# potamides/DeTikZify

Measured on AMD Instinct MI355X. Metric: tikz_tokens_per_sec, higher is better.
Workload: dtype bf16; 1 GPU; detikzify-ds-7b (synthetic weights, seed 1234), 1 image 224x224->384x384, 243-token prefix, greedy decode of 512 tokens per rollout, batch 1 per GPU, hipGraph per token; rollouts_per_gpu=5

## Files before the change

### detikzify_amd/_lib.py

```python
from __future__ import annotations

import ctypes as C
import os
from pathlib import Path

_HERE = Path(__file__).resolve().parent
LIB_PATH = _HERE / "lib" / "libdtk_hip.so"

DTK_ABI_VERSION = 7
DTK_VIT_BATCH = 8
DTK_F32, DTK_BF16, DTK_F16 = 0, 1, 2
DTK_ARCH_PROJ_NO_BIAS = 1
DTK_PREFILL_REUSE_PREFIX, DTK_PREFILL_REUSE_IMAGE = 1, 2
DTK_MAX_INFLIGHT = 4
DTK_MAX_BATCH = 64
DTK_MAX_TOP = 8
DTK_EPI_BIAS, DTK_EPI_GELU, DTK_EPI_RESIDUAL, DTK_GEMM_NAIVE = 1, 2, 4, 256
DTK_GEMM_WT = 512
DTK_GEMM_SL = 1024
DTK_GEMM_KSLICES_SHIFT = 12


class DtkConfig(C.Structure):
    _fields_ = [
# ... 163 lines not shown
    "dtk_decode_batch_launch": (C.c_int, [_P, C.POINTER(C.c_int32)]),
    "dtk_decode_batch_wait": (C.c_int, [_P, C.POINTER(C.c_int64)]),
    "dtk_kv_fork": (C.c_int, [_P, C.c_int, C.c_int, C.c_int]),
    "dtk_get_logits_slot": (C.c_int, [_P, C.c_int, _P]),
    "dtk_context_len_slot": (C.c_int, [_P, C.c_int]),
    "dtk_slot_lcp": (C.c_int, [_P, C.c_int, _P, C.c_int, C.c_uint64, C.POINTER(C.c_int)]),
    "dtk_slot_cached_ids": (C.c_int, [_P, C.c_int, _P, C.c_int]),
    "dtk_resume_slot": (C.c_int, [_P, C.c_int, _P, C.c_int, C.c_uint64]),
    "dtk_bench_gemv": (C.c_int, [_P, C.c_int, C.c_int, C.c_int, C.POINTER(C.c_float)]),
    "dtk_set_gemv_variant": (C.c_int, [_P, C.c_int, C.c_int]),
    "dtk_set_option": (C.c_int, [_P, C.c_char_p, C.c_int]),
    "dtk_op_gemm": (C.c_int, [_P, _P, _P, _P, _P, C.c_int, C.c_int, C.c_int, C.c_int, _P]),
    "dtk_adapter_create": (C.c_int, [_P, C.POINTER(DtkAdapterConfig)]),
    "dtk_adapter_destroy": (C.c_int, [_P]),
    "dtk_has_adapter": (C.c_int, [_P]),
    "dtk_vit_encode_text": (C.c_int, [_P, _P, C.c_int, _P, C.c_int, C.c_uint64, _P, _P]),
    "dtk_prefill_text": (C.c_int, [_P, _P, C.c_int, _P, C.c_uint64, _P, C.c_int, C.c_uint64, C.c_int, _P]),
    "dtk_prefill_slot_text": (C.c_int, [_P, C.c_int, _P, C.c_int, _P, C.c_uint64, _P, C.c_int, C.c_uint64, C.c_int, _P]),
    "dtk_adapter_embed": (C.c_int, [_P, _P, C.c_int, _P]),
    "dtk_text_image_key": (C.c_uint64, [C.c_uint64, C.c_uint64]),
    "dtk_op_gemm_gated": (C.c_int, [_P, _P, _P, _P, _P, _P, C.c_int, C.c_int, C.c_int, C.c_int, _P]),
    "dtk_score": (C.c_int, [_P, _P, C.c_int, _P, C.c_uint64, C.c_uint32, C.c_int, _P, _P, _P]),
    "dtk_score_text": (C.c_int, [_P, _P, C.c_int, _P, C.c_uint64, _P, C.c_int, C.c_uint64, C.c_uint32, C.c_int, _P, _P, _P]),
    "dtk_op_score": (C.c_int, [_P, _P, _P, _P, C.c_int, C.c_int, C.c_int, C.c_int, _P, _P, _P, _P]),
    "dtk_score_packed": (C.c_int, [_P, _P, C.c_int, _P, C.c_uint64, C.c_uint32, _P, _P, C.c_int, _P, _P, _P]),
    "dtk_score_packed_text": (C.c_int, [_P, _P, C.c_int, _P, C.c_uint64, _P, C.c_int, C.c_uint64, C.c_uint32, _P, _P, C.c_int, _P, _P, _P]),
    "dtk_op_attention_seg": (C.c_int, [_P, _P, _P, _P, C.c_int, C.c_int, C.c_int, C.c_int, C.c_int, _P, _P, _P]),
    "dtk_op_attn_decode": (C.c_int, [_P, _P, _P, _P, C.c_int, C.c_int, C.c_int, C.c_int, _P, C.c_int, C.c_int, C.c_int, C.c_int, C.c_int,
                                     _P, _P, _P, _P]),
    "dtk_op_attn_decode_b": (C.c_int, [_P, _P, _P, _P, C.c_int, C.c_int, C.c_int, C.c_int, _P, _P, _P, _P,
                                       C.c_int, C.c_int, C.c_int, C.c_int, C.c_int, _P]),
    "dtk_kv8_info": (C.c_int, [_P, C.c_int, C.POINTER(C.c_int)]),
    "dtk_read_kv8": (C.c_int, [_P, C.c_int, C.c_int, C.c_int, C.c_int, C.c_int, _P, _P, _P]),
    "dtk_op_attn_decode_b8": (C.c_int, [_P, _P, _P, _P, C.c_int, C.c_int, C.c_int, C.c_int, _P, _P, _P, _P, _P, _P, _P, _P, _P,
                                        C.c_int, C.c_int, C.c_int, C.c_int, C.c_int, _P]),
    "dtk_op_gemv_b": (C.c_int, [_P, C.c_int, _P, _P, _P, C.c_int, C.c_int, _P, _P, C.c_float, _P, _P, C.c_int,
                                C.c_int, C.c_int, C.c_int, C.c_int, C.c_int, _P, _P, _P, _P, _P, _P, _P, _P, _P, _P]),
    "dtk_op_gemv_bkp": (C.c_int, [_P, _P, _P, _P, C.c_int, C.c_int, _P, _P, C.c_int, _P, C.c_float, _P, _P, _P, _P]),
    "dtk_op_gemv_role": (C.c_int, [_P, C.c_int, C.c_int, C.c_int, _P, _P, _P, _P, _P] + [C.c_int] * 9 + [C.c_float, _P, _P, _P, _P,
                                   C.c_int, _P, _P, _P, C.c_int, _P, _P, _P, _P, _P]),
    "dtk_op_rope_scatter": (C.c_int, [_P, C.c_int, _P, _P] + [C.c_int] * 8 + [_P, C.c_int, _P, _P, C.c_int, _P, _P, _P]),
    "dtk_op_rows_norm": (C.c_int, [_P, C.c_int, _P, _P, C.c_int, C.c_int, _P, _P, _P, _P, _P] + [C.c_int] * 7 + [C.c_float, C.c_int, _P, _P]),
    "dtk_op_swiglu": (C.c_int, [_P, C.c_int, _P, _P, C.c_int, C.c_int, _P, _P, C.c_int, C.c_int, C.c_int, C.c_int, C.c_int, _P]),
    "dtk_op_attention_ex": (C.c_int, [_P, _P, C.c_int64, _P, C.c_int64, _P, C.c_int64, _P, C.c_int64, _P] + [C.c_int] * 9),
    "dtk_op_rows_move": (C.c_int, [_P, C.c_int, _P, _P, _P] + [C.c_int] * 8 + [_P]),
    "dtk_op_gemv_mv_role": (C.c_int, [_P] + [C.c_int] * 4 + [_P, _P, _P] + [C.c_int] * 7 + [_P, _P, C.c_int, C.c_int, _P, _P, C.c_float,
                                      _P, _P, C.c_int, _P, _P, _P, _P, _P]),
    "dtk_w13_row_bytes": (C.c_int, [C.c_int]),
    "dtk_w13_pack_host": (C.c_int, [_P, C.c_int, C.c_int, _P, _P, _P]),
    "dtk_w13_unpack_host": (C.c_int, [_P, _P, C.c_int, C.c_int, _P]),
    "dtk_w13_op_bad_rows": (C.c_int, [_P]),
    "dtk_w13_row_bytes_host": (C.c_int, [_P, C.c_int, C.c_int, _P]),
    "dtk_w13_flagged_rows": (C.c_int, [_P, C.c_int]),
    "dtk_op_gemv": (C.c_int, [_P, _P, _P, _P, C.c_int, C.c_int, C.c_int, C.c_float, _P]),
    "dtk_op_gemv_mv": (C.c_int, [_P, _P, _P, _P, C.c_int, C.c_int, C.c_int, C.c_float, C.c_int, _P]),
    "dtk_op_gemv_q4": (C.c_int, [_P, _P, _P, _P, C.c_int, C.c_int, C.c_int, C.c_float, _P, _P]),
    "dtk_mx_layout": (C.c_int, [C.c_int, C.c_int, C.c_int, _P, _P]),
    "dtk_op_gemv_mx": (C.c_int, [_P, _P, _P, _P, C.c_int, C.c_int, C.c_int, C.c_int, C.c_int, _P, _P, _P, _P, _P]),
    "dtk_op_attention": (C.c_int, [_P, _P, _P, _P, C.c_int, C.c_int, C.c_int, C.c_int, C.c_int, C.c_int, _P]),
    "dtk_op_layernorm": (C.c_int, [_P, _P, _P, _P, C.c_int, C.c_int, C.c_float, _P]),
    "dtk_op_sample": (C.c_int, [_P, _P, C.c_int, C.c_int, C.POINTER(C.c_int64), _P]),
    "dtk_decode_wait_lp": (C.c_int, [_P, C.POINTER(C.c_int64), C.POINTER(C.c_float)]),
    "dtk_decode_batch_wait_lp": (C.c_int, [_P, C.POINTER(C.c_int64), C.POINTER(C.c_float), C.POINTER(C.c_float)]),
    "dtk_engine_read_lp": (C.c_int, [_P, C.c_int, C.POINTER(C.c_int64), C.POINTER(C.c_float), C.POINTER(C.c_float), C.c_int,
                                     C.POINTER(C.c_int32), C.POINTER(C.c_int32), C.c_int]),
    "dtk_engine_set_wait_lp_op": (C.c_int, [_P, DtkEngineOps.WAIT_LP]),
    "dtk_op_sample_lp": (C.c_int, [_P, _P, C.c_int, C.c_int, C.POINTER(C.c_int64), _P, C.POINTER(C.c_float)]),
    "dtk_score_top": (C.c_int, [_P, _P, C.c_int, _P, C.c_uint64, C.c_uint32, C.c_int, _P, _P, _P, C.c_int, _P, _P]),
    "dtk_score_top_text": (C.c_int, [_P, _P, C.c_int, _P, C.c_uint64, _P, C.c_int, C.c_uint64, C.c_uint32, C.c_int, _P, _P, _P,
                                     C.c_int, _P, _P]),
    "dtk_score_packed_top": (C.c_int, [_P, _P, C.c_int, _P, C.c_uint64, C.c_uint32, _P, _P, C.c_int, _P, _P, _P, C.c_int, _P, _P]),
    "dtk_score_packed_top_text": (C.c_int, [_P, _P, C.c_int, _P, C.c_uint64, _P, C.c_int, C.c_uint64, C.c_uint32, _P, _P, C.c_int,
                                            _P, _P, _P, C.c_int, _P, _P]),
    "dtk_op_score_top": (C.c_int, [_P, _P, _P, _P, C.c_int, C.c_int, C.c_int, C.c_int, _P, _P, _P, _P, C.c_int, _P, _P, _P]),
    "dtk_decode_wait_top": (C.c_int, [_P, C.POINTER(C.c_int64), C.POINTER(C.c_float), C.POINTER(C.c_int32), C.POINTER(C.c_float)]),
    "dtk_decode_batch_wait_top": (C.c_int, [_P, C.POINTER(C.c_int64), C.POINTER(C.c_float), C.POINTER(C.c_float),
                                            C.POINTER(C.c_int32), C.POINTER(C.c_float)]),
    "dtk_set_sampling_ext": (C.c_int, [_P, C.POINTER(DtkSamplingExt)]),
    "dtk_set_sampling_slot_ext": (C.c_int, [_P, C.c_int, C.POINTER(DtkSamplingExt)]),
    "dtk_op_sample_ext": (C.c_int, [_P, _P, C.c_int, C.c_int, C.POINTER(C.c_int64), _P, C.POINTER(C.c_float), C.POINTER(DtkSamplingExt)]),
    "dtk_engine_submit_ext": (C.c_int, [_P, C.POINTER(DtkJoin), C.POINTER(DtkSamplingExt), C.POINTER(C.c_int64), C.c_int, C.c_uint64,
                                        C.POINTER(C.c_uint64)]),
    "dtk_engine_set_sampling_ext_op": (C.c_int, [_P, DtkEngineOps.SAMPLING_EXT]),
    "dtk_set_penalties": (C.c_int, [_P, C.c_float, C.c_float, C.c_int]),
    "dtk_set_penalties_slot": (C.c_int, [_P, C.c_int, C.c_float, C.c_float, C.c_int]),
    "dtk_op_sample_pen": (C.c_int, [_P, _P, C.c_int, C.c_int, C.POINTER(C.c_int64), _P, C.POINTER(C.c_float), C.POINTER(DtkSamplingExt),
                                    C.c_float, C.c_float, C.POINTER(C.c_int64), C.c_int]),
    "dtk_token_counts": (C.c_int, [_P, C.c_int, C.POINTER(C.c_uint16), C.c_int]),
    "dtk_engine_submit_pen": (C.c_int, [_P, C.POINTER(DtkJoin), C.POINTER(DtkSamplingExt), C.c_float, C.c_float, C.c_int,
                                        C.POINTER(C.c_int64), C.c_int, C.c_uint64, C.POINTER(C.c_uint64)]),
    "dtk_engine_set_penalties_op": (C.c_int, [_P, DtkEngineOps.PENALTIES]),
    "dtk_set_dry": (C.c_int, [_P, C.POINTER(DtkDry)]),
    "dtk_set_dry_slot": (C.c_int, [_P, C.c_int, C.POINTER(DtkDry)]),
    "dtk_dry_history": (C.c_int, [_P, C.c_int, C.POINTER(C.c_int32), C.c_int]),
    "dtk_dry_state_bytes": (C.c_int64, [_P]),
    "dtk_op_dry_scan": (C.c_int, [_P, C.c_int, C.POINTER(C.c_int64), C.c_int, C.POINTER(C.c_int64), C.c_int, C.POINTER(DtkDry),
                                  C.POINTER(C.c_int32), C.POINTER(C.c_uint8), C.c_int]),
    "dtk_op_sample_dry": (C.c_int, [_P, _P, C.c_int, C.c_int, C.POINTER(C.c_int64), _P, C.POINTER(C.c_float), C.POINTER(DtkSamplingExt),
                                    C.c_float, C.c_float, C.POINTER(C.c_int64), C.c_int, C.POINTER(C.c_int64), C.c_int, C.POINTER(DtkDry)]),
    "dtk_engine_submit_dry": (C.c_int, [_P, C.POINTER(DtkJoin), C.POINTER(DtkSamplingExt), C.c_float, C.c_float, C.c_int, C.POINTER(DtkDry),
                                        C.POINTER(C.c_int64), C.c_int, C.c_uint64, C.POINTER(C.c_uint64)]),
    "dtk_engine_set_dry_op": (C.c_int, [_P, DtkEngineOps.DRY]),
    "dtk_set_length_control": (C.c_int, [_P, C.POINTER(DtkLengthCtl)]),
    "dtk_set_length_control_slot": (C.c_int, [_P, C.c_int, C.POINTER(DtkLengthCtl)]),
    "dtk_set_logit_bias": (C.c_int, [_P, C.POINTER(C.c_int32), C.POINTER(C.c_float), C.c_int]),
    "dtk_set_logit_bias_slot": (C.c_int, [_P, C.c_int, C.POINTER(C.c_int32), C.POINTER(C.c_float), C.c_int]),
# ... 85 lines not shown
```

### detikzify_amd/csrc/dtk_api.hip

```cpp
#include <hip/hip_runtime.h>

#include <cfloat>
#include <cmath>
#include <cstdarg>
#include <cstdio>
#include <cstdlib>
#include <cstring>
#include <atomic>
#include <mutex>
#include <string>
#include <unordered_map>
#include <vector>

#include "dtk_ctx.h"
#include "w13.h"
#include "mx_quant.h"

int& dtk_lds_attr_error(int device) {
  static int e[65] = {};
  return e[(device >= 0 && device < 64) ? device : 64];
}

namespace {

// ... 497 lines not shown

static void pen_args(const dtk_ctx* c, SampleArgs& sa, DryScanArgs& ds, bool batch) {
  const bool dry = (batch ? c->dry_batch : c->dry_single) && c->dry_tab;
  const bool pen = (batch ? c->pen_batch : c->pen_single) && c->pen_tab;
  const bool len = (batch ? c->len_batch : c->len_single) && c->len_dev;
  if (!(pen || dry || len) || !c->pen_dev || !c->pen_tok) return;
  const int first = batch ? 1 : 0;
  if (len) {
    sa.len = c->len_dev + first; sa.len_m = c->len_m + (size_t)first * c->len_m_stride; sa.len_m_stride = c->len_m_stride;
    sa.bias = c->bias_tab + (size_t)first * c->bias_stride; sa.bias_stride = c->bias_stride;
  }
  sa.pen = c->pen_dev + first; sa.pen_cnt = c->pen_tab ? c->pen_tab + (size_t)first * c->pen_stride : nullptr; sa.pen_stride = c->pen_stride;
  sa.pen_tok = c->pen_tok + first;
  if (!dry) return;
  sa.dry = c->dry_dev + first; sa.dry_m = c->dry_tab + (size_t)first * c->dry_stride; sa.dry_stride = c->dry_stride;
  ds.dry = sa.dry; ds.hist = c->dry_hist + (size_t)first * c->Tmax; ds.len = c->dry_len + first; ds.hist_stride = c->Tmax;
  ds.m = c->dry_tab + (size_t)first * c->dry_stride; ds.m_stride = c->dry_stride;
  ds.touched = c->dry_touched + (size_t)first * c->Tmax; ds.n_touched = c->dry_ntouched + first;
  ds.V = sa.V; ds.bs = sa.bs; ds.nslots = sa.bs ? sa.nslots : 1;
}
static void sampler_launch(dtk_ctx* c, SampleArgs& sa, bool mb, bool batch) {
  DryScanArgs ds;
  pen_args(c, sa, ds, batch);
  if (sa.dry) launch_dry_scan(ds, c->stream);
  if (mb) launch_sample_mb(sa, c->stream); else launch_sample_b(sa, c->stream);
  if (sa.pen) launch_count_token(sa, ds, c->stream);
}

static void top_logits_launch(dtk_ctx* c, const SampleArgs& sa) {
  if (!c->top_logprobs || !c->logprobs) return;
  TopArgs t;
  t.logits = sa.logits; t.V = sa.V; t.logits_stride = sa.logits_stride; t.st = sa.st; t.bs = sa.bs; t.nslots = sa.nslots;
  t.ring = sa.ring; t.k = c->top_logprobs; t.top_ring = sa.bs ? c->topb_dev : c->top_ring_dev;
  launch_top_logits(t, c->stream);
}

static inline int cfg_grid(const dtk_ctx* c) { return c->cfg_res > c->cfg_n ? c->cfg_res : c->cfg_n; }
static void guidance_launch(dtk_ctx* c, const SampleArgs& sa) {
  if (!cfg_grid(c)) return;
  CfgArgs g;
  g.logits = const_cast<float*>(sa.logits); g.V = sa.V; g.stride = sa.logits_stride; g.pairs = c->cfg_dev; g.n_pairs = cfg_grid(c); g.bs = sa.bs;
  g.part = c->cfg_part; g.lse = c->cfg_lse; g.st = sa.st; g.forced = c->cfg_forced;
  launch_cfg_mix(g, c->stream);
}
static void follow_launch(dtk_ctx* c, const SampleArgs& sa) {
  if (!cfg_grid(c)) return;
  CfgFollowArgs f;
  f.pairs = c->cfg_dev; f.n_pairs = cfg_grid(c); f.bs = sa.bs; f.forced = c->cfg_forced; f.st = sa.st; f.x = sa.x; f.d = sa.d; f.tok_ring = sa.tok_ring; f.ring = sa.ring;
  f.lp_ring = sa.lp_ring; f.lse_ring = sa.lse_ring; f.top_ring = (c->logprobs && c->top_logprobs) ? c->topb_dev : nullptr;
  launch_cfg_follow(f, c->stream);
}

static inline bool w13_on(const dtk_ctx* c) { return c->wfmt == 0 && c->w13 != 0; }

void decode_step_launches(dtk_ctx* c, bool with_probe, bool short_ctx = false) {
  hipStream_t s = c->stream;
  SampleArgs sa;
  sa.logits = c->logits; sa.V = c->V; sa.sp = c->sp; sa.st = c->st; sa.embed = c->embed;
  sa.x = c->x; sa.d = c->d; sa.tok_ring = c->tok_ring_dev; sa.ring = DTK_MAX_INFLIGHT;
  sa.probs_out = nullptr; sa.advance = 1; sa.step_override = -1; sa.bs = nullptr; sa.logits_stride = 0; sa.nslots = 1; sa.mb = c->smb;
  sa.lp_ring = c->logprobs ? c->lp_ring_dev : nullptr;
  sa.trunc = c->trunc_single ? 1 : 0;
  sa.lse_ring = (c->logprobs && c->top_logprobs) ? c->lse_ring_dev : nullptr;
  top_logits_launch(c, sa);
  sampler_launch(c, sa, c->mb_single, false);
  const float scale = 1.0f / sqrtf((float)c->hd);
  for (int l = 0; l < c->L; ++l) {
    const LayerW& w = c->layers[l];
    GemvArgs g{};
    g.eps = c->cfg.rms_eps; g.st = c->st; g.T_max = c->Tmax; g.d = c->d; g.ff = c->ff; g.H = c->H; g.KVH = c->KVH; g.hd = c->hd;
    g.rope_cos = c->rope_cos; g.rope_sin = c->rope_sin;
    g.pm = c->pm; g.pl = c->pl; g.po = c->po; g.S = c->S;
    g.W = w.wqkv; g.W8 = w.q_wqkv; g.wscale = w.s_wqkv; g.N = c->d + 2 * c->KVH * c->hd; g.K = c->d; g.x = c->x; g.norm_w = w.ln1;
    g.W4 = w.f4_wqkv; g.S4 = w.e4_wqkv;
    const bool p13 = w13_on(c) && c->w13_ready;
    g.Wp = p13 ? w.p13_wqkv : nullptr; g.Wh = w.h13_wqkv;
    g.q_out = c->q; g.kcache = kcache(c, l); g.vcache = vcache(c, l);
    launch_gemv(PRO_RMSNORM, EPI_QKV, g, s);
    AttnDecArgs ad;
    ad.q = c->q; ad.kcache = kcache(c, l); ad.vcache = vcache(c, l); ad.st = c->st;
    ad.pm = c->pm; ad.pl = c->pl; ad.po = c->po; ad.H = c->H; ad.S = c->S; ad.T_max = c->Tmax; ad.G = c->H / c->KVH;
    ad.scale = scale; ad.hd = c->hd;
    ad.threads = c->attn_threads;
    ad.combine = (!ad.threads && short_ctx && c->attn_combine == 2) ? 3 : c->attn_combine; ad.out = c->attn_out; ad.counters = c->attn_ctr;
    if (ad.threads && ad.combine == 1) ad.combine = 2;
    launch_attn_decode(ad, s);
    g.W = w.wo; g.W8 = w.q_wo; g.wscale = w.s_wo; g.N = c->d; g.K = c->d; g.y = c->x;
    g.W4 = w.f4_wo; g.S4 = w.e4_wo;
    g.Wp = p13 ? w.p13_wo : nullptr; g.Wh = w.h13_wo;
    const bool partials = ad.combine == 0 && !(ad.threads && ad.S == 1);
    if (!partials) { g.x = c->attn_out; launch_gemv(PRO_COPY, EPI_RESID, g, s); }
    else launch_gemv(PRO_ATTN, EPI_RESID, g, s);
    g.W = w.wgu; g.W8 = w.q_wgu; g.wscale = w.s_wgu; g.N = 2 * c->ff; g.K = c->d; g.x = c->x; g.norm_w = w.ln2; g.y = c->act;
    g.W4 = w.f4_wgu; g.S4 = w.e4_wgu;
    g.Wp = p13 ? w.p13_wgu : nullptr; g.Wh = w.h13_wgu;
    const bool probe_here = with_probe && (l == c->L / 2);
    if (probe_here) (void)hipEventRecord(c->probe_a, s);
    launch_gemv(PRO_RMSNORM, EPI_SWIGLU, g, s);
    if (probe_here) (void)hipEventRecord(c->probe_b, s);
    g.W = w.wdown; g.W8 = w.q_wdown; g.wscale = w.s_wdown; g.N = c->d; g.K = c->ff; g.x = c->act; g.y = c->x;
    g.W4 = w.f4_wdown; g.S4 = w.e4_wdown;
    g.Wp = p13 ? w.p13_wdown : nullptr; g.Wh = w.h13_wdown;
    launch_gemv(PRO_COPY, EPI_RESID, g, s);
  }
  GemvArgs g{};
  if (w13_on(c) && c->w13_ready) { g.Wp = c->p13_lm_head; g.Wh = c->h13_lm_head; }
  g.W = c->lm_head; g.W8 = c->q_lm_head; g.wscale = c->s_lm_head; g.N = c->V; g.K = c->d; g.x = c->x; g.norm_w = c->final_norm;
  g.eps = c->cfg.rms_eps; g.logits = c->logits;
  launch_gemv(PRO_RMSNORM, EPI_LOGITS, g, s);
}

static inline bool mx_step(const dtk_ctx* c) { return c->wfmt == 1 && c->mx_ok && c->act_fp8 != 0; }
static inline void kv8_args(const dtk_ctx* c, int l, AttnDecBArgs& ad) {
  if (!c->kv8) return;
  const size_t head_rows = (size_t)c->KVH * c->Tmax, kv_layer = 2 * head_rows * 128;
  ad.k8 = c->kv8c + (size_t)l * kv_layer; ad.v8 = ad.k8 + head_rows * 128;
  ad.k8s = c->kv8s + (size_t)l * (kv_layer / 32); ad.v8s = ad.k8s + head_rows * 4;
  ad.kv8_slot_stride = c->kv_slot_stride;
}

void batch_step_launches_mx(dtk_ctx* c) {
  hipStream_t s = c->stream;
  const int d = c->d, ff = c->ff, nslots = 16 * c->nt_step;
  SampleArgs sa;
  sa.logits = c->logits_b; sa.V = c->V; sa.sp = c->sp_b; sa.st = c->st_b; sa.embed = c->embed;
  sa.x = c->xb; sa.d = d; sa.tok_ring = c->tokb_dev; sa.ring = DTK_MAX_INFLIGHT;
  sa.probs_out = nullptr; sa.advance = 1; sa.step_override = -1; sa.bs = c->bs_dev; sa.logits_stride = c->V; sa.nslots = nslots; sa.mb = c->smb_b;
  sa.lp_ring = c->logprobs ? c->lpb_dev : nullptr;
  sa.trunc = c->trunc_batch ? 1 : 0;
  sa.lse_ring = (c->logprobs && c->top_logprobs) ? c->lseb_dev : nullptr;
  guidance_launch(c, sa);
  top_logits_launch(c, sa);
  sampler_launch(c, sa, c->mb_batch, true);
  follow_launch(c, sa);
  const float scale = 1.0f / sqrtf(128.f);
  const size_t kv_layer = (size_t)2 * c->KVH * c->Tmax * 128;
  for (int l = 0; l < c->L; ++l) {
    const LayerW& w = c->layers[l];
    bf16_t* kc = c->kvb + (size_t)l * kv_layer;
    bf16_t* vc = kc + (size_t)c->KVH * c->Tmax * 128;
    GemvBArgs g{};
    g.bs = c->bs_dev; g.st = c->st_b; g.T_max = c->Tmax; g.d = d; g.ff = ff; g.H = c->H; g.KVH = c->KVH; g.nt = c->nt_step;
    g.rope_cos = c->rope_cos; g.rope_sin = c->rope_sin; g.kv_slot_stride = c->kv_slot_stride; g.kpart = c->kpart; g.err = batch_err_word(c);
    if (l == 0) launch_rmsnorm_b(c->xb, d, w.ln1, c->xnb, d, d, c->cfg.rms_eps, c->bs_dev, nslots, s, c->xn8, c->xns);
    g.Wm = w.m_wqkv; g.wscale = w.s_wqkv; g.N = d + 2 * c->KVH * 128; g.K = d; g.X8 = c->xn8; g.XS = c->xns; g.q_out = c->qb; g.kcache = kc; g.vcache = vc;
    launch_gemv_mxu(EPI_QKV, g, s);
    AttnDecBArgs ad;
    ad.q = c->qb; ad.kcache = kc; ad.vcache = vc; ad.kv_slot_stride = c->kv_slot_stride; ad.st = c->st_b; ad.bs = c->bs_dev;
    ad.out = c->aob; ad.H = c->H; ad.T_max = c->Tmax; ad.d = d; ad.G = c->H / c->KVH; ad.nslots = nslots;
    ad.scale = scale;
    ad.use_prefix = c->prefix_mfma; ad.pfx_splits = c->pfx_splits; ad.tail_threads = c->tail_threads; ad.gqa_fused = c->gqa_fused; ad.nt_private = c->attn_nt;
    ad.pfx_m = c->pfx_m; ad.pfx_l = c->pfx_l; ad.pfx_o = c->pfx_o;
    ad.out8 = c->ao8; ad.outs = c->aos;
    kv8_args(c, l, ad);
    launch_attn_decode_b(ad, s);
    g.Wm = w.m_wo; g.wscale = w.s_wo; g.N = d; g.K = d; g.X8 = c->ao8; g.XS = c->aos;
    if (!launch_gemv_mxk(g, 32, s)) c->launch_refused = true;
    launch_resid_norm_b(c->kpart, c->xb, d, w.ln2, c->xnb, d, c->cfg.rms_eps, c->bs_dev, nslots, s, c->xn8, c->xns);
    g.Wm = w.m_wgu; g.wscale = w.s_wgu; g.N = 2 * ff; g.K = d; g.X8 = c->xn8; g.XS = c->xns; g.Y8 = c->act8; g.YS = c->acts;
    launch_gemv_mxu(EPI_SWIGLU, g, s);
    g.Wm = w.m_wdown; g.wscale = w.s_wdown; g.N = d; g.K = ff; g.X8 = c->act8; g.XS = c->acts;
// ... 138 lines not shown
  }
  g.W = c->lm_head; g.W8 = c->q_lm_head; g.wscale = c->s_lm_head; g.N = c->V; g.K = d; g.X = c->xb; g.ldx = d; g.norm_w = c->final_norm;
  g.logits = c->logits_b;
  launch_gemv_mv(PRO_RMSNORM, EPI_LOGITS, NB, g, s);
}

void ensure_fp8_weights(dtk_ctx* c) {
  if (c->wfmt == 0 || c->fp8_ready) return;
  for (int l = 0; l < c->L && c->wfmt == 2; ++l) {
    LayerW& w = c->layers[l];
    launch_quant_mxfp4_rows(w.wqkv, w.f4_wqkv, w.e4_wqkv, c->d + 2 * c->KVH * c->hd, c->d, c->stream);
    launch_quant_mxfp4_rows(w.wo, w.f4_wo, w.e4_wo, c->d, c->d, c->stream);
    launch_quant_mxfp4_rows(w.wgu, w.f4_wgu, w.e4_wgu, 2 * c->ff, c->d, c->stream);
    launch_quant_mxfp4_rows(w.wdown, w.f4_wdown, w.e4_wdown, c->d, c->ff, c->stream);
  }
  for (int l = 0; l < c->L && c->wfmt == 1; ++l) {
    LayerW& w = c->layers[l];
    launch_quant_fp8_rows(w.wqkv, w.q_wqkv, w.s_wqkv, c->d + 2 * c->KVH * c->hd, c->d, c->stream);
    launch_quant_fp8_rows(w.wo, w.q_wo, w.s_wo, c->d, c->d, c->stream);
    launch_quant_fp8_rows(w.wgu, w.q_wgu, w.s_wgu, 2 * c->ff, c->d, c->stream);
    launch_quant_fp8_rows(w.wdown, w.q_wdown, w.s_wdown, c->d, c->ff, c->stream);
  }
  launch_quant_fp8_rows(c->lm_head, c->q_lm_head, c->s_lm_head, c->V, c->d, c->stream);
  c->fp8_ready = true;
  c->tiled_ready = false;
  c->ptiled_ready = false;
}

static void set_weight_bytes(dtk_ctx* c) {
  const uint64_t kvd = (uint64_t)c->KVH * c->hd;
  const uint64_t attn_lin = (uint64_t)2 * c->d * c->d + 2 * kvd * c->d;
  const uint64_t per_layer = attn_lin + (uint64_t)3 * c->d * c->ff + 2 * (uint64_t)c->d;
  c->stats.weight_bytes_per_token = 2 * (per_layer * c->L + (uint64_t)c->d + (uint64_t)c->V * c->d);
  if (c->wfmt == 1) {
    const uint64_t lin = attn_lin + (uint64_t)3 * c->d * c->ff;
    const uint64_t rows = (uint64_t)3 * c->d + 2 * kvd + (uint64_t)2 * c->ff;
    c->stats.weight_bytes_per_token = (lin + 4 * rows + 4 * (uint64_t)c->d) * c->L + 2 * (uint64_t)c->d + (uint64_t)c->V * c->d + 4 * (uint64_t)c->V;
  }
  if (c->wfmt == 2) {
    const uint64_t bd = mxfp4_row_scales(c->d), bf = mxfp4_row_scales(c->ff);
    const uint64_t blocks = ((uint64_t)2 * c->d + 2 * kvd + (uint64_t)2 * c->ff) * bd + (uint64_t)c->d * bf;
    c->stats.weight_bytes_per_token = (17 * blocks + 4 * (uint64_t)c->d) * c->L + 2 * (uint64_t)c->d + (uint64_t)c->V * c->d + 4 * (uint64_t)c->V;
  }
  c->stats.probe_kernel_bytes = (uint64_t)2 * c->ff * c->d * (c->wfmt == 1 ? 1 : 2);
  if (c->wfmt == 2) c->stats.probe_kernel_bytes = (uint64_t)2 * c->ff * 17 * mxfp4_row_scales(c->d);
  if (w13_on(c) && c->w13_ready) {
    auto mat = [](const uint8_t* planes, uint64_t N, int K) { return planes ? N * (w13_row_bytes(K) + 1) : 2 * N * (uint64_t)K; };
    uint64_t W = 2 * ((uint64_t)2 * c->d * c->L + (uint64_t)c->d) + mat(c->p13_lm_head, (uint64_t)c->V, c->d);
    for (int l = 0; l < c->L; ++l) {
      const LayerW& w = c->layers[l];
      W += mat(w.p13_wqkv, (uint64_t)c->d + 2 * kvd, c->d) + mat(w.p13_wo, (uint64_t)c->d, c->d) + mat(w.p13_wgu, (uint64_t)2 * c->ff, c->d) +
           mat(w.p13_wdown, (uint64_t)c->d, c->ff);
    }
    c->stats.weight_bytes_per_token = W;
    c->stats.probe_kernel_bytes = mat(c->layers[c->L / 2].p13_wgu, (uint64_t)2 * c->ff, c->d);
  }
}
static void w13_set_stats(dtk_ctx* c) {
  const uint32_t rows = c->w13_bad_rows > 4095u ? 4095u : c->w13_bad_rows;
  c->stats.w13_counts = (c->w13_packed & 1023u) | ((c->w13_unpacked & 1023u) << 10) | (rows << 20);
}
static int w13_pack_one(dtk_ctx* c, int role, int pro, int epi, const bf16_t* W, int N, int K, uint8_t** planes, uint8_t** hb) {
  GemvArgs g{};
  g.N = N; g.K = K; g.d = c->d; g.ff = c->ff; g.hd = c->hd;
  if (!gemv_w13_takes(pro, epi, g)) {
    if (*planes) { (void)hipFree(*planes); *planes = nullptr; }
    if (*hb) { (void)hipFree(*hb); *hb = nullptr; }
    return DTK_OK;
  }
  if (!*planes) HIPCHK(c, hipMalloc((void**)planes, (size_t)N * w13_row_bytes(K)));
  if (!*hb) HIPCHK(c, hipMalloc((void**)hb, (size_t)N));
  HIPCHK(c, hipMemsetAsync(c->w13_bad, 0, sizeof(unsigned), c->stream));
  launch_pack_w13_rows(W, *planes, *hb, c->w13_bad, N, K, !c->w13_nz, c->stream);
  unsigned bad = 0;
  HIPCHK(c, hipMemcpyAsync(&bad, c->w13_bad, sizeof(unsigned), hipMemcpyDeviceToHost, c->stream));
  HIPCHK(c, hipStreamSynchronize(c->stream));
  if (bad) {
    (void)hipFree(*planes); *planes = nullptr;
    (void)hipFree(*hb); *hb = nullptr;
    c->w13_unpacked++; c->w13_bad_rows += bad;
  } else {
    c->w13_packed++;
    std::vector<uint8_t> bytes((size_t)N);
    HIPCHK(c, hipMemcpy(bytes.data(), *hb, (size_t)N, hipMemcpyDeviceToHost));
    for (uint8_t b : bytes) c->w13_zrows[role] += (b & W13_ZROW) ? 1u : 0u;
  }
  return DTK_OK;
}
static void w13_free(dtk_ctx* c);
int ensure_w13(dtk_ctx* c) {
  if (!w13_on(c) || c->w13_ready) return DTK_OK;
  if (!c->w13_bad) HIPCHK(c, hipMalloc((void**)&c->w13_bad, sizeof(unsigned)));
  c->w13_packed = c->w13_unpacked = c->w13_bad_rows = 0;
  for (uint32_t& z : c->w13_zrows) z = 0;
  const int qkvn = c->d + 2 * c->KVH * c->hd;
  for (int l = 0; l < c->L; ++l) {
    LayerW& w = c->layers[l];
    int rc = w13_pack_one(c, 0, PRO_RMSNORM, EPI_QKV, w.wqkv, qkvn, c->d, &w.p13_wqkv, &w.h13_wqkv);
    if (!rc) rc = w13_pack_one(c, 1, PRO_ATTN, EPI_RESID, w.wo, c->d, c->d, &w.p13_wo, &w.h13_wo);
    if (!rc) rc = w13_pack_one(c, 2, PRO_RMSNORM, EPI_SWIGLU, w.wgu, 2 * c->ff, c->d, &w.p13_wgu, &w.h13_wgu);
    if (!rc) rc = w13_pack_one(c, 3, PRO_COPY, EPI_RESID, w.wdown, c->d, c->ff, &w.p13_wdown, &w.h13_wdown);
    if (rc) { w13_free(c); return rc; }
  }
  int rc = w13_pack_one(c, 4, PRO_RMSNORM, EPI_LOGITS, c->lm_head, c->V, c->d, &c->p13_lm_head, &c->h13_lm_head);
  if (rc) { w13_free(c); return rc; }
  c->w13_ready = true;
  w13_set_stats(c);
  set_weight_bytes(c);
  return DTK_OK;
}
static void w13_free(dtk_ctx* c) {
  for (auto& w : c->layers) {
    uint8_t** ps[8] = {&w.p13_wqkv, &w.h13_wqkv, &w.p13_wo, &w.h13_wo, &w.p13_wgu, &w.h13_wgu, &w.p13_wdown, &w.h13_wdown};
    for (uint8_t** p : ps) if (*p) { (void)hipFree(*p); *p = nullptr; }
  }
  if (c->p13_lm_head) { (void)hipFree(c->p13_lm_head); c->p13_lm_head = nullptr; }
  if (c->h13_lm_head) { (void)hipFree(c->h13_lm_head); c->h13_lm_head = nullptr; }
  c->w13_ready = false;
  c->w13_packed = c->w13_unpacked = c->w13_bad_rows = 0;
  for (uint32_t& z : c->w13_zrows) z = 0;
}

void ensure_tiled_weights(dtk_ctx* c);
void ensure_prefill_tiles(dtk_ctx* c) {
  ensure_fp8_weights(c);
  if (c->ptiled_ready) return;
  for (int l = 0; l < c->L; ++l)
    if (c->layers[l].p_wgui) launch_retile_pairs(c->layers[l].wgu, c->layers[l].p_wgui, c->ff, c->d, c->stream);
  if (c->nb > 0 && c->wfmt != 1) { ensure_tiled_weights(c); c->ptiled_ready = true; return; }
  for (int l = 0; l < c->L; ++l) {
    LayerW& w = c->layers[l];
    launch_retile(w.wqkv, w.p_wqkv, c->d + 2 * c->KVH * c->hd, c->d, c->stream);
    launch_retile(w.wo, w.p_wo, c->d, c->d, c->stream);
    launch_retile(w.wgu, w.p_wgu, 2 * c->ff, c->d, c->stream);
    launch_retile(w.wdown, w.p_wdown, c->d, c->ff, c->stream);
  }
  c->ptiled_ready = true;
}

void ensure_tiled_weights(dtk_ctx* c) {
  ensure_fp8_weights(c);
  if (c->tiled_ready || c->nb <= 0) return;
  if (c->wfmt == 1) {
    const int qkvn = c->d + 2 * c->KVH * 128;
    for (int l = 0; l < c->L; ++l) {
      LayerW& w = c->layers[l];
      launch_retile_f8(w.q_wqkv, w.t8_wqkv, qkvn, c->d, c->stream);
      launch_retile_f8(w.q_wo, w.t8_wo, c->d, c->d, c->stream);
      launch_retile_f8(w.q_wgu, w.t8_wgu, 2 * c->ff, c->d, c->stream);
      launch_retile_f8(w.q_wdown, w.t8_wdown, c->d, c->ff, c->stream);
    }
    launch_retile_f8(c->q_lm_head, c->t8_lm_head, c->V, c->d, c->stream);
    if (c->mx_ok) {
      for (int l = 0; l < c->L; ++l) {
        LayerW& w = c->layers[l];
        launch_retile_mx(w.q_wqkv, w.m_wqkv, qkvn, c->d, 32, c->stream);
        launch_retile_mx(w.q_wo, w.m_wo, c->d, c->d, 32, c->stream);
        launch_retile_mx(w.q_wgu, w.m_wgu, 2 * c->ff, c->d, 32, c->stream);
        launch_retile_mx(w.q_wdown, w.m_wdown, c->d, c->ff, 16, c->stream);
      }
      launch_retile_mx(c->q_lm_head, c->m_lm_head, c->V, c->d, 32, c->stream);
    }
    c->tiled_ready = true;
    return;
  }
  for (int l = 0; l < c->L; ++l) {
    LayerW& w = c->layers[l];
    launch_retile(w.wqkv, w.t_wqkv, c->d + 2 * c->KVH * 128, c->d, c->stream);
    launch_retile(w.wo, w.t_wo, c->d, c->d, c->stream);
    launch_retile(w.wgu, w.t_wgu, 2 * c->ff, c->d, c->stream);
    launch_retile(w.wdown, w.t_wdown, c->d, c->ff, c->stream);
  }
  launch_retile(c->lm_head, c->t_lm_head, c->V, c->d, c->stream);
// ... 2162 lines not shown
  return dtk_decode_wait(c, token_out);
}

int dtk_get_logits(dtk_ctx* c, float* out) {
  if (!c || !out) return fail(c, DTK_ERR_ARG, "dtk_get_logits: null argument");
  if (!c->seq0.have_logits) return fail(c, DTK_ERR_STATE, "no logits yet");
  HIPCHK(c, hipSetDevice(c->device));
  HIPCHK(c, hipStreamSynchronize(c->stream));
  HIPCHK(c, hipMemcpy(out, c->logits, (size_t)c->V * 4, hipMemcpyDeviceToHost));
  return DTK_OK;
}

int dtk_context_len(const dtk_ctx* c) { return c ? c->seq0.host_next_pos : -1; }

int dtk_synchronize(dtk_ctx* c) {
  if (!c) return DTK_ERR_ARG;
  HIPCHK(c, hipSetDevice(c->device));
  HIPCHK(c, hipStreamSynchronize(c->stream));
  HIPCHK(c, hipGetLastError());
  return DTK_OK;
}

int dtk_get_stats(dtk_ctx* c, dtk_stats* out) {
  if (!c || !out) return DTK_ERR_ARG;
  *out = c->stats;
  return DTK_OK;
}

int dtk_bench_gemv(dtk_ctx* c, int role, int variant, int reps, float* avg_us) {
  if (!c || !avg_us || reps < 1) return fail(c, DTK_ERR_ARG, "dtk_bench_gemv: bad argument");
  HIPCHK(c, hipSetDevice(c->device));
  hipStream_t s = c->stream;
  if (role < 0 || role > 4) return fail(c, DTK_ERR_ARG, "dtk_bench_gemv: role %d (0 qkv, 1 o_proj, 2 gate/up, 3 down, 4 lm_head)", role);
  const bool same_layer = (variant & 0x100) != 0;
  const int plain = (variant >> 9) & 3;
  const bool fmt = (variant & 0x800) != 0;
  const bool b13 = (variant & 0x1000) != 0, raw16 = (variant & 0x2000) != 0;
  if (b13 && (fmt || raw16 || plain || same_layer || c->wfmt != 0 || !c->w13 || (variant & 0xff) == 0xff))
    return fail(c, DTK_ERR_ARG, "dtk_bench_gemv: 0x1000 | shape (13-bit planes) needs a bf16 context with w13 = 1, a shape number and no other flag");
  if (raw16 && ((variant & 0xff) != 0xff || plain || fmt)) return fail(c, DTK_ERR_ARG, "dtk_bench_gemv: 0x2000 (bf16 rows) goes with variant 0xff only");
  const bool step13 = w13_on(c) && !raw16 && !plain && (variant & 0xff) == 0xff;
  struct Tmp13 { std::vector<uint8_t*> p, h; ~Tmp13() { for (auto x : p) if (x) (void)hipFree(x); for (auto x : h) if (x) (void)hipFree(x); } } tmp13;
  if (b13 || step13) { if (int rc = ensure_w13(c)) return rc; }
  if (b13) {
    for (int l = 0; l < c->L && role != 4; ++l) {
      const LayerW& w = c->layers[l];
      const uint8_t* p = role == 0 ? w.p13_wqkv : (role == 1 ? w.p13_wo : (role == 2 ? w.p13_wgu : w.p13_wdown));
      if (p) continue;
      if (role != 1) return fail(c, DTK_ERR_STATE, "dtk_bench_gemv: role %d has no 13-bit planes in layer %d (an unpackable row, or a bf16 fold no 13-bit shape has)", role, l);
      if (!c->w13_bad) HIPCHK(c, hipMalloc((void**)&c->w13_bad, sizeof(unsigned)));
      uint8_t *pp = nullptr, *hh = nullptr;
      HIPCHK(c, hipMalloc((void**)&pp, (size_t)c->d * w13_row_bytes(c->d)));
      tmp13.p.push_back(pp);
      HIPCHK(c, hipMalloc((void**)&hh, (size_t)c->d));
      tmp13.h.push_back(hh);
      unsigned bad = 0;
      HIPCHK(c, hipMemsetAsync(c->w13_bad, 0, sizeof(unsigned), s));
      launch_pack_w13_rows(w.wo, pp, hh, c->w13_bad, c->d, c->d, !c->w13_nz, s);
      HIPCHK(c, hipMemcpyAsync(&bad, c->w13_bad, sizeof(unsigned), hipMemcpyDeviceToHost, s));
      HIPCHK(c, hipStreamSynchronize(s));
      if (bad) return fail(c, DTK_ERR_STATE, "dtk_bench_gemv: o_proj of layer %d has %u unpackable row(s)", l, bad);
    }
    if (role == 4 && !c->p13_lm_head) return fail(c, DTK_ERR_STATE, "dtk_bench_gemv: lm_head has no 13-bit planes");
  }
  if (fmt && ((variant & 0xff) != 0xff || plain))
    return fail(c, DTK_ERR_ARG, "dtk_bench_gemv: 0x800 (the context's weight format) goes with variant 0xff only");
  if (fmt) ensure_fp8_weights(c);
  variant &= 0xff;
  const bool shipped = variant == 0xff;
  if (b13) {
    const int pro = (role == 1 || role == 3) ? PRO_COPY : PRO_RMSNORM;
    const int epi = role == 0 ? EPI_QKV : (role == 2 ? EPI_SWIGLU : (role == 4 ? EPI_LOGITS : EPI_RESID));
    if (!gemv_w13_has(pro, epi, variant)) return fail(c, DTK_ERR_ARG, "dtk_bench_gemv: no 13-bit shape %d for role %d", variant, role);
  }
  auto launch = [&](int pro, int epi, const GemvArgs& g) {
    if (b13) launch_gemv_w13_variant(pro, epi, variant, g, s);
    else if (shipped) launch_gemv(pro, epi, g, s);
    else launch_gemv_variant(pro, epi, variant, g, s);
  };
  auto one_pass = [&]() {
    for (int l = 0; l < c->L; ++l) {
      const LayerW& w = c->layers[same_layer ? 0 : l];
      GemvArgs g{};
      if (plain) {
        g.eps = c->cfg.rms_eps; g.y = c->GU;
        if (role == 0) { g.W = w.wqkv; g.N = c->d + 2 * c->KVH * c->hd; g.K = c->d; g.x = c->x; g.norm_w = w.ln1; }
        else if (role == 1) { g.W = w.wo; g.N = c->d; g.K = c->d; g.x = c->attn_out; g.norm_w = w.ln1; }
        else if (role == 2) { g.W = w.wgu; g.N = 2 * c->ff; g.K = c->d; g.x = c->x; g.norm_w = w.ln2; }
        else if (role == 3) { g.W = w.wdown; g.N = c->d; g.K = c->ff; g.x = c->act; g.norm_w = w.ln2; }
        else { g.W = c->lm_head; g.N = c->V; g.K = c->d; g.x = c->x; g.norm_w = c->final_norm; }
        launch_gemv_variant(plain == 2 ? PRO_RMSNORM : PRO_COPY, EPI_STORE, variant, g, s);
        continue;
      }
      g.eps = c->cfg.rms_eps; g.st = c->st; g.T_max = c->Tmax; g.d = c->d; g.ff = c->ff; g.H = c->H; g.KVH = c->KVH; g.hd = c->hd;
      g.rope_cos = c->rope_cos; g.rope_sin = c->rope_sin; g.pm = c->pm; g.pl = c->pl; g.po = c->po; g.S = c->S;
      if (fmt) {
        if (role == 0) { g.W8 = w.q_wqkv; g.wscale = w.s_wqkv; g.W4 = w.f4_wqkv; g.S4 = w.e4_wqkv; }
        else if (role == 1) { g.W8 = w.q_wo; g.wscale = w.s_wo; g.W4 = w.f4_wo; g.S4 = w.e4_wo; }
        else if (role == 2) { g.W8 = w.q_wgu; g.wscale = w.s_wgu; g.W4 = w.f4_wgu; g.S4 = w.e4_wgu; }
        else if (role == 3) { g.W8 = w.q_wdown; g.wscale = w.s_wdown; g.W4 = w.f4_wdown; g.S4 = w.e4_wdown; }
        else { g.W8 = c->q_lm_head; g.wscale = c->s_lm_head; }
      }
      if (b13 || step13) {
        if (role == 0) { g.Wp = w.p13_wqkv; g.Wh = w.h13_wqkv; }
        else if (role == 1) { g.Wp = w.p13_wo; g.Wh = w.h13_wo; if (!g.Wp && b13) { g.Wp = tmp13.p[(size_t)l]; g.Wh = tmp13.h[(size_t)l]; } }
        else if (role == 2) { g.Wp = w.p13_wgu; g.Wh = w.h13_wgu; }
        else if (role == 3) { g.Wp = w.p13_wdown; g.Wh = w.h13_wdown; }
        else { g.Wp = c->p13_lm_head; g.Wh = c->h13_lm_head; }
      }
      if (role == 0) { g.W = w.wqkv; g.N = c->d + 2 * c->KVH * c->hd; g.K = c->d; g.x = c->x; g.norm_w = w.ln1; g.q_out = c->q; g.kcache = kcache(c, l); g.vcache = vcache(c, l); launch(PRO_RMSNORM, EPI_QKV, g); }
      else if (role == 1) { g.W = w.wo; g.N = c->d; g.K = c->d; g.x = c->attn_out; g.y = c->q; launch(PRO_COPY, EPI_RESID, g); }
      else if (role == 2) { g.W = w.wgu; g.N = 2 * c->ff; g.K = c->d; g.x = c->x; g.norm_w = w.ln2; g.y = c->act; launch(PRO_RMSNORM, EPI_SWIGLU, g); }
      else if (role == 3) { g.W = w.wdown; g.N = c->d; g.K = c->ff; g.x = c->act; g.y = c->q; launch(PRO_COPY, EPI_RESID, g); }
      else { g.W = c->lm_head; g.N = c->V; g.K = c->d; g.x = c->x; g.norm_w = c->final_norm; g.logits = c->logits; launch(PRO_RMSNORM, EPI_LOGITS, g); }
    }
  };
  one_pass();
  HIPCHK(c, hipEventRecord(c->ev_a, s));
  for (int r = 0; r < reps; ++r) one_pass();
  HIPCHK(c, hipEventRecord(c->ev_b, s));
  HIPCHK(c, hipStreamSynchronize(s));
  HIPCHK(c, hipGetLastError());
  float ms = 0.f;
  HIPCHK(c, hipEventElapsedTime(&ms, c->ev_a, c->ev_b));
  *avg_us = ms * 1e3f / (float)(reps * c->L);
  c->seq0.have_logits = false;
  return DTK_OK;
}
// ... 4 lines not shown
  if (c->blaunched != c->bwaited) return fail(c, DTK_ERR_STATE, "dtk_bench_cfg: a batch step is in flight");
  HIPCHK(c, hipSetDevice(c->device));
  SampleArgs sa;
  sa.logits = c->logits_b; sa.V = c->V; sa.logits_stride = c->V; sa.bs = c->bs_dev; sa.st = c->st_b; sa.x = c->xb; sa.d = c->d;
  sa.tok_ring = c->tokb_dev; sa.ring = DTK_MAX_INFLIGHT;
  sa.lp_ring = c->logprobs ? c->lpb_dev : nullptr; sa.lse_ring = (c->logprobs && c->top_logprobs) ? c->lseb_dev : nullptr;
  for (int which = 0; which < 2; ++which) {
    for (int i = 0; i < 3; ++i) { if (which) follow_launch(c, sa); else guidance_launch(c, sa); }
    HIPCHK(c, hipEventRecord(c->probe_a, c->stream));
    for (int i = 0; i < reps; ++i) { if (which) follow_launch(c, sa); else guidance_launch(c, sa); }
    HIPCHK(c, hipEventRecord(c->probe_b, c->stream));
    HIPCHK(c, hipEventSynchronize(c->probe_b));
    float ms = 0.f;
    HIPCHK(c, hipEventElapsedTime(&ms, c->probe_a, c->probe_b));
    avg_us[which] = ms * 1000.f / (float)reps;
  }
  return DTK_OK;
}

int dtk_bench_spec(dtk_ctx* c, int reps, float* avg_us) {
  if (!c || !avg_us || reps < 1 || reps > 64) return fail(c, DTK_ERR_ARG, "dtk_bench_spec: bad argument (1 <= reps <= 64)");
  if (!c->spec_on) return fail(c, DTK_ERR_STATE, "dtk_bench_spec: slot 0 is not speculating (dtk_spec_begin)");
  if (c->blaunched != c->bwaited) return fail(c, DTK_ERR_STATE, "dtk_bench_spec: a step is in flight");
  HIPCHK(c, hipSetDevice(c->device));
  SpecArgs sv;
  sv.sd = c->spec_sd; sv.hist = c->spec_hist; sv.table = c->spec_table; sv.K = 0; sv.max_ngram = 0; sv.NV = 0; sv.T_max = c->Tmax; sv.V = c->V;
  sv.st_true = c->st_b; sv.st_vec = c->spec_st; sv.bs = c->spec_bs; sv.tok_ring = c->tokb_dev; sv.ring = DTK_MAX_INFLIGHT;
  sv.embed = c->embed; sv.x = c->xb; sv.d = c->d;
  for (int i = 0; i < 3; ++i) { launch_spec_accept(sv, c->stream); launch_spec_draft(sv, c->stream); }
  HIPCHK(c, hipEventRecord(c->probe_a, c->stream));
  for (int i = 0; i < reps; ++i) { launch_spec_accept(sv, c->stream); launch_spec_draft(sv, c->stream); }
  HIPCHK(c, hipEventRecord(c->probe_b, c->stream));
  HIPCHK(c, hipEventSynchronize(c->probe_b));
  float ms = 0.f;
  HIPCHK(c, hipEventElapsedTime(&ms, c->probe_a, c->probe_b));
  *avg_us = ms * 1000.f / (float)reps;
  const uint32_t ring_was = (uint32_t)(c->blaunched % DTK_MAX_INFLIGHT);
  HIPCHK(c, hipMemcpy(&c->spec_bs->step, &ring_was, sizeof ring_was, hipMemcpyHostToDevice));
  return DTK_OK;
}

int dtk_set_option(dtk_ctx* c, const char* name, int value) {
  if (!c || !name) return DTK_ERR_ARG;
  HIPCHK(c, hipSetDevice(c->device));
  HIPCHK(c, hipStreamSynchronize(c->stream));
  if (!strcmp(name, "attn_full_max")) c->attn_full_max = value;
  else if (!strcmp(name, "w13")) {
    if (value != 0 && value != 1) return fail(c, DTK_ERR_ARG, "w13 must be 0 or 1");
    if (value != c->w13) {
      if (c->launched != c->waited) return fail(c, DTK_ERR_STATE, "w13: %d single-sequence decode step(s) are unread", (int)(c->launched - c->waited));
      c->w13 = value; drop_graph(c);
      if (!value) { w13_free(c); w13_set_stats(c); }
      set_weight_bytes(c);
    }
  }
  else if (!strcmp(name, "w13_nz")) {
    if (value != 0 && value != 1) return fail(c, DTK_ERR_ARG, "w13_nz must be 0 or 1");
    if (value != c->w13_nz) {
      if (c->launched != c->waited) return fail(c, DTK_ERR_STATE, "w13_nz: %d single-sequence decode step(s) are unread", (int)(c->launched - c->waited));
      c->w13_nz = value;
      if (c->w13_ready) { c->w13_ready = false; drop_graph(c); }
    }
  }
  else if (!strcmp(name, "logprobs")) {
    if (value != 0 && value != 1) return fail(c, DTK_ERR_ARG, "logprobs must be 0 or 1");
    if (value == 0 && c->top_logprobs) return fail(c, DTK_ERR_STATE, "logprobs: top_logprobs = %d needs it (set \"top_logprobs\" to 0 first)", c->top_logprobs);
    if ((value != 0) != (c->logprobs != 0)) {
      if (c->blaunched != c->bwaited) return fail(c, DTK_ERR_STATE, "logprobs: a batch step is in flight");
      if (c->engine_holds.load() > 0) return fail(c, DTK_ERR_STATE, "logprobs: an engine holds %d sequence(s) in this context's slots", c->engine_holds.load());
      if (c->launched != c->waited) return fail(c, DTK_ERR_STATE, "logprobs: %d single-sequence decode step(s) are unread", (int)(c->launched - c->waited));
      c->logprobs = value; drop_graph(c); drop_batch_graphs(c);
    }
  }
  else if (!strcmp(name, "top_logprobs")) {
    if (value < 0 || value > DTK_MAX_TOP) return fail(c, DTK_ERR_ARG, "top_logprobs must be 0 .. %d", DTK_MAX_TOP);
    if (value > c->V) return fail(c, DTK_ERR_ARG, "top_logprobs = %d exceeds the vocabulary (%d)", value, c->V);
    if (value != 0 && !c->logprobs) return fail(c, DTK_ERR_STATE, "top_logprobs needs logprobs = 1 (dtk_set_option \"logprobs\", 1 first)");
    if (value != c->top_logprobs) {
      if (c->blaunched != c->bwaited) return fail(c, DTK_ERR_STATE, "top_logprobs: a batch step is in flight");
      if (c->engine_holds.load() > 0) return fail(c, DTK_ERR_STATE, "top_logprobs: an engine holds %d sequence(s) in this context's slots", c->engine_holds.load());
      if (c->launched != c->waited) return fail(c, DTK_ERR_STATE, "top_logprobs: %d single-sequence decode step(s) are unread", (int)(c->launched - c->waited));
      if (value) {
        const size_t n1 = DTK_MAX_INFLIGHT, nb = c->nb > 0 ? (size_t)DTK_MAX_INFLIGHT * DTK_MAX_BATCH : 0;
        if (!c->top_ring_dev) { HIPCHK(c, hipMalloc(&c->top_ring_dev, sizeof(TopRec) * n1)); HIPCHK(c, hipMemset(c->top_ring_dev, 0, sizeof(TopRec) * n1)); }
        if (!c->lse_ring_dev) { HIPCHK(c, hipMalloc(&c->lse_ring_dev, sizeof(float) * n1)); HIPCHK(c, hipMemset(c->lse_ring_dev, 0, sizeof(float) * n1)); }
        if (!c->top_ring_host) HIPCHK(c, hipHostMalloc((void**)&c->top_ring_host, sizeof(TopRec) * n1, hipHostMallocDefault));
        if (!c->lse_ring_host) HIPCHK(c, hipHostMalloc((void**)&c->lse_ring_host, sizeof(float) * n1, hipHostMallocDefault));
        if (nb && !c->topb_dev) { HIPCHK(c, hipMalloc(&c->topb_dev, sizeof(TopRec) * nb)); HIPCHK(c, hipMemset(c->topb_dev, 0, sizeof(TopRec) * nb)); }
        if (nb && !c->lseb_dev) { HIPCHK(c, hipMalloc(&c->lseb_dev, sizeof(float) * nb)); HIPCHK(c, hipMemset(c->lseb_dev, 0, sizeof(float) * nb)); }
        if (nb && !c->topb_host) HIPCHK(c, hipHostMalloc((void**)&c->topb_host, sizeof(TopRec) * nb, hipHostMallocDefault));
        if (nb && !c->lseb_host) HIPCHK(c, hipHostMalloc((void**)&c->lseb_host, sizeof(float) * nb, hipHostMallocDefault));
      }
      c->top_logprobs = value; drop_graph(c); drop_batch_graphs(c);
    }
  }
  else if (!strcmp(name, "gemm_tile")) {
    if (value < 0 || value > 5) return fail(c, DTK_ERR_ARG, "gemm_tile must be 0..5");
    set_gemm_tile(value);
  }
  else if (!strcmp(name, "share_prefix_reads")) c->share_reads = value != 0;
  else if (!strcmp(name, "prefix_mfma") || !strcmp(name, "pfx_splits") || !strcmp(name, "gemv_b_wide") ||
           !strcmp(name, "tail_threads")) {
    if (!strcmp(name, "prefix_mfma")) c->prefix_mfma = value != 0;
    else if (!strcmp(name, "tail_threads")) { if (value != 64 && value != 128 && value != 256 && value != 512) return fail(c, DTK_ERR_ARG, "tail_threads must be 64, 128, 256 or 512"); c->tail_threads = value; }
    else if (!strcmp(name, "pfx_splits")) { if (value < 1 || value > 4) return fail(c, DTK_ERR_ARG, "pfx_splits must be 1..4"); c->pfx_splits = value; }
    else { if (value < 0 || value > 6) return fail(c, DTK_ERR_ARG, "gemv_b_wide must be 0..6"); set_gemv_b_wide(value); }
// ... 383 lines not shown
```

### detikzify_amd/csrc/dtk_ctx.h

```cpp
#pragma once
#include <hip/hip_runtime.h>

#include <atomic>
#include <cstddef>
#include <cstdint>
#include <mutex>
#include <string>
#include <unordered_map>
#include <vector>

#include "../../include/dtk.h"
#include "kernels.h"
#ifndef W13_DEFAULT
#define W13_DEFAULT 1
#endif

struct TensorEntry {
  std::string name;
  bf16_t* ptr = nullptr;
  int64_t rows = 1;
  int64_t cols = 0;
  int64_t stride = 0;
  float synth_scale = 0.02f;
  float synth_offset = 0.f;
// ... 75 lines not shown

  bf16_t *X, *Xn, *QKV, *Qh, *AO, *GU, *ACT;
  int sk_sl_min_rows = SK_SL_MIN_ROWS;
  float* skpart = nullptr;
  size_t skpart_floats = 0;
  int swiglu_fused = 1;
  int qkv_rope_fused = 1;
  int prefill_sk = 1;
  int32_t* ids_dev = nullptr;
  float* score_rec = nullptr;
  float* score_out = nullptr;
  float* score_top = nullptr;
  int32_t* packed_rows = nullptr;
  bf16_t *x, *q, *act;
  float *logits, *pm, *pl, *po;
  bf16_t* attn_out = nullptr;
  unsigned* attn_ctr = nullptr;
  int attn_combine = 0;
  DecState* st = nullptr;
  SamplingDev* sp = nullptr;
  int64_t* tok_ring_dev = nullptr;
  int64_t* tok_ring_host = nullptr;
  float* probs_dev = nullptr;
  int logprobs = 0;
  std::atomic<int> engine_holds{0};
  float2* lp_ring_dev = nullptr;
  float2* lp_ring_host = nullptr;
  float2* lpb_dev = nullptr;
  float2* lpb_host = nullptr;
  int top_logprobs = 0;
  TopRec* top_ring_dev = nullptr;
  TopRec* top_ring_host = nullptr;
  float* lse_ring_dev = nullptr;
  float* lse_ring_host = nullptr;
  TopRec* topb_dev = nullptr;
  TopRec* topb_host = nullptr;
  float* lseb_dev = nullptr;
  float* lseb_host = nullptr;
  float* pixels_dev = nullptr;
  bf16_t *patches, *VX, *VN, *VQKV, *VAO, *VH, *feats, *last_hidden;
  bf16_t *pq, *pkv, *pao, *px, *pn, *ph, *pooled;
  bf16_t* IMG;
  Adapter* ad = nullptr;
  unsigned char* scratch = nullptr;
  size_t scratch_bytes = 0;

  SeqHost seq0;
  int wfmt = 0;
  bool fp8_ready = false;
  uint8_t* q_lm_head = nullptr;
  float* s_lm_head = nullptr;
  int w13 = W13_DEFAULT;
  int w13_nz = 1;
  bool w13_ready = false;
  uint8_t *p13_lm_head = nullptr, *h13_lm_head = nullptr;
  unsigned* w13_bad = nullptr;
  int w13_op_bad_rows = -1;
  uint32_t w13_packed = 0, w13_unpacked = 0, w13_bad_rows = 0;
  uint32_t w13_zrows[5] = {0, 0, 0, 0, 0};
  uint64_t cached_image_key = 0;
  bool have_image = false;
  int KVH = 0;
  int hd = 128;
  bool proj_bias = true;
  int nb = 0;
  bool share_reads = true;
  int nt = 1;
  std::vector<SeqHost> bseq;
  bf16_t* kvb = nullptr;
  size_t kv_slot_stride = 0;
  int kv8 = 0; int kv8_slots = 0;
  uint8_t* kv8c = nullptr; uint8_t* kv8s = nullptr;
  bf16_t *xb = nullptr, *xnb = nullptr, *qb = nullptr, *aob = nullptr, *actb = nullptr;
  float* logits_b = nullptr;
  float* kpart = nullptr; unsigned* kctr = nullptr;
  int attn_nt = 1;
  bool resid_kparts = true;
  float *pfx_m = nullptr, *pfx_l = nullptr, *pfx_o = nullptr;
  int prefix_mfma = 0;
  int pfx_splits = 4;
  int gqa_fused = 1;
  int tail_threads = 256;
  DecState* st_b = nullptr;
  SamplingDev* sp_b = nullptr;
  BatchState* bs_dev = nullptr;
  bf16_t* t_lm_head = nullptr;
  uint8_t* t8_lm_head = nullptr;
  uint8_t* m_lm_head = nullptr;
  uint8_t *xn8 = nullptr, *xns = nullptr, *ao8 = nullptr, *aos = nullptr, *act8 = nullptr, *acts = nullptr;
  bool mx_ok = false;
  int act_fp8 = 0;
  bool launch_refused = false;
  bool tiled_ready = false;
  bool ptiled_ready = false;
  BatchState* bs_host = nullptr;
  SamplingDev* sp_stage = nullptr; uint32_t* draw_stage = nullptr;
  DecState* st_stage = nullptr;
  int64_t* tokb_dev = nullptr;
  int64_t* tokb_host = nullptr;
  uint64_t blaunched = 0, bwaited = 0;
  hipEvent_t bstep_done[DTK_MAX_INFLIGHT] = {};
  bool bgraph_ready[6] = {false, false, false, false, false, false};
  hipGraph_t bgraph[6] = {nullptr, nullptr, nullptr, nullptr, nullptr, nullptr};
  hipGraphExec_t bgraph_exec[6] = {nullptr, nullptr, nullptr, nullptr, nullptr, nullptr};
  int nt_step = 1;
  int mv_slots = 4;
  int mv_step = 0;
  int mv_tail_threads = 512;
  dtk_sampling sampling{};
  SampleMB* smb = nullptr;
  SampleMB* smb_b = nullptr;
  bool mb_single = false;
// ... 120 lines not shown
```

### detikzify_amd/csrc/dtk_ops.hip

```cpp
#include <hip/hip_runtime.h>

#include <cmath>
#include <cstdio>
#include <cstdlib>
#include <cstring>
#include <optional>
#include <vector>

#include "dtk_ctx.h"
#include "w13.h"
#include "mx_quant.h"

#pragma GCC visibility push(default)
extern "C" {

extern "C++" {
namespace {
struct OpRun {
  static constexpr size_t GUARD = 256;
  dtk_ctx* c; const char* who; int fill; size_t off = 0, need = 0; bool full = false;
  struct In { void* dev; const void* host; size_t bytes; };
  struct Res { void* dev; void* host; size_t bytes; const char* name; bool up; };
  std::vector<In> ins; std::vector<Res> res;
  OpRun(dtk_ctx* c_, const char* who_, int fill_ = -1) : c(c_), who(who_), fill(fill_) {}
// ... 480 lines not shown
int dtk_op_gemv_role(dtk_ctx* c, int pro, int epi, int variant, const uint16_t* W, const uint8_t* W8, const float* wscale,
                     const uint8_t* W4, const uint8_t* S4, int N, int K, int d, int ff, int H, int KVH, int hd, int T_max, int pos, float eps,
                     const uint16_t* x, const uint16_t* norm_w, const uint16_t* rope_cos, const uint16_t* rope_sin,
                     int S, const float* pm, const float* pl, const float* po, int scratch_fill,
                     uint16_t* q_io, uint16_t* k_io, uint16_t* v_io, uint16_t* y_io, float* logits_io) {
  if (!c) return DTK_ERR_ARG;
  if ((W != nullptr) + (W8 != nullptr) + (W4 != nullptr) != 1 || (W8 && !wscale) || (!W8 && wscale) || (!W4 != !S4))
    return fail(c, DTK_ERR_ARG, "dtk_op_gemv_role: exactly one of W | W8 + wscale | W4 + S4");
  const int fmt = W4 ? 2 : (W8 ? 1 : 0);
  const bool f13 = variant >= 0x1000;
  const int v13 = variant - 0x1000;
  if (f13) {
    if (fmt != 0) return fail(c, DTK_ERR_ARG, "dtk_op_gemv_role: the 13-bit planes are packed from bf16 operands (W)");
    if (v13 != 0xff && !gemv_w13_has(pro, epi, v13)) return fail(c, DTK_ERR_ARG, "dtk_op_gemv_role: no 13-bit kernel for prologue %d, epilogue %d, shape %d", pro, epi, v13);
    if (v13 == 0xff && !gemv_w13_has(pro, epi, 0)) return fail(c, DTK_ERR_ARG, "dtk_op_gemv_role: no 13-bit kernel for prologue %d, epilogue %d", pro, epi);
    variant = -1;
  }
  if (N < 1 || K < 8 || (K & 7) || (fmt == 1 && (K & 15))) return fail(c, DTK_ERR_ARG, "dtk_op_gemv_role: N >= 1, K a multiple of 8 (16 for fp8 weights)");
  if (pro < PRO_COPY || pro > PRO_ATTN || epi < EPI_STORE || epi > EPI_LOGITS) return fail(c, DTK_ERR_ARG, "dtk_op_gemv_role: unknown prologue %d or epilogue %d", pro, epi);
  if (!gemv_role_variant_ok(fmt, pro, epi, variant))
    return fail(c, DTK_ERR_ARG, "dtk_op_gemv_role: no %s kernel for prologue %d, epilogue %d, variant %d", fmt == 2 ? "MXFP4" : (fmt == 1 ? "fp8" : "bf16"), pro, epi, variant);
  if (hd != 128 && hd != 64) return fail(c, DTK_ERR_ARG, "dtk_op_gemv_role: head dim %d (128 or 64)", hd);
  if (scratch_fill < 0 || scratch_fill > 255 || d < 0) return fail(c, DTK_ERR_ARG, "dtk_op_gemv_role: scratch_fill is a byte, d >= 0");
  if (pro == PRO_ATTN) {
    if (S < 1 || S > 16) return fail(c, DTK_ERR_ARG, "dtk_op_gemv_role: S must be 1..16");
    if (H < 1 || K != H * hd || !pm || !pl || !po) return fail(c, DTK_ERR_ARG, "dtk_op_gemv_role: PRO_ATTN needs K = H * hd and the partials pm / pl / po");
  } else if (!x || (pro == PRO_RMSNORM && !norm_w)) return fail(c, DTK_ERR_ARG, "dtk_op_gemv_role: x (and norm_w for PRO_RMSNORM) required");
  if (epi == EPI_QKV) {
    if (H < 1 || KVH < 1 || H % KVH) return fail(c, DTK_ERR_ARG, "dtk_op_gemv_role: H %d query heads over KVH %d key / value heads", H, KVH);
    if (N != (H + 2 * KVH) * hd || d != H * hd) return fail(c, DTK_ERR_ARG, "dtk_op_gemv_role: QKV needs N = (H + 2 KVH) * hd and d = H * hd");
    if (T_max < 1 || pos < 0 || pos >= T_max) return fail(c, DTK_ERR_ARG, "dtk_op_gemv_role: position %d of %d rows", pos, T_max);
    if (!rope_cos || !rope_sin || !q_io || !k_io || !v_io) return fail(c, DTK_ERR_ARG, "dtk_op_gemv_role: QKV needs the rope tables and q / k / v buffers");
  } else if (epi == EPI_SWIGLU) {
    if (ff < 8 || (ff & 7) || N != 2 * ff || !y_io) return fail(c, DTK_ERR_ARG, "dtk_op_gemv_role: SWIGLU needs ff a multiple of 8 (as dtk_create), N = 2 ff and y");
  } else if (epi == EPI_LOGITS) {
    if (!logits_io) return fail(c, DTK_ERR_ARG, "dtk_op_gemv_role: LOGITS needs the logits buffer");
  } else if (!y_io) return fail(c, DTK_ERR_ARG, "dtk_op_gemv_role: RESID / STORE need y");
  HIPCHK(c, hipSetDevice(c->device));
  hipStream_t s = c->stream;
  const int KC4 = (K + 31) >> 5, hd2 = hd / 2;
  const size_t w_bytes = fmt == 2 ? (size_t)N * KC4 * 16 : (fmt == 1 ? (size_t)N * K : (size_t)N * K * 2);
  const size_t kv = epi == EPI_QKV ? (size_t)KVH * T_max * hd : 0, qn = epi == EPI_QKV ? (size_t)H * hd : 0, rope = epi == EPI_QKV ? (size_t)T_max * hd2 : 0;
  const size_t ny = epi == EPI_SWIGLU ? (size_t)ff : ((epi == EPI_STORE || epi == EPI_RESID) ? (size_t)N : 0), nl = epi == EPI_LOGITS ? (size_t)N : 0;
  const size_t hs = pro == PRO_ATTN ? (size_t)H * S : 0;
  DecState hst; memset(&hst, 0, sizeof hst);
  hst.pos = pos; hst.next_pos = pos + 1;
  OpRun r(c, "dtk_op_gemv_role", scratch_fill);
  GemvArgs g{};
  const uint8_t* dW = r.in<uint8_t>(fmt == 2 ? (const void*)W4 : (fmt == 1 ? (const void*)W8 : (const void*)W), w_bytes);
  const float* dws = r.in<float>(wscale, fmt == 1 ? N : 0); const uint8_t* dS4 = r.in<uint8_t>(S4, fmt == 2 ? (size_t)N * KC4 : 0);
  if (fmt == 0) g.W = reinterpret_cast<const bf16_t*>(dW);
  else if (fmt == 1) { g.W8 = dW; g.wscale = dws; }
  else { g.W4 = dW; g.S4 = dS4; }
  uint8_t* dWp = (uint8_t*)r.take(f13 ? (size_t)N * w13_row_bytes(K) : 0); uint8_t* dWh = (uint8_t*)r.take(f13 ? (size_t)N : 0);
  unsigned* dbad = (unsigned*)r.take(f13 ? sizeof(unsigned) : 0);
  g.x = r.in<bf16_t>(pro != PRO_ATTN ? x : nullptr, K); g.norm_w = r.in<bf16_t>(pro == PRO_RMSNORM ? norm_w : nullptr, K);
  g.rope_cos = r.in<bf16_t>(rope_cos, rope); g.rope_sin = r.in<bf16_t>(rope_sin, rope); g.st = r.in<DecState>(&hst, 1);
  g.pm = r.in<float>(pm, hs); g.pl = r.in<float>(pl, hs); g.po = r.in<float>(po, hs * hd);
  g.q_out = r.io<bf16_t>(qn ? q_io : nullptr, qn, "q"); g.kcache = r.io<bf16_t>(kv ? k_io : nullptr, kv, "k"); g.vcache = r.io<bf16_t>(kv ? v_io : nullptr, kv, "v");
  g.y = r.io<bf16_t>(ny ? y_io : nullptr, ny, "y"); g.logits = r.io<float>(nl ? logits_io : nullptr, nl, "logits");
  g.N = N; g.K = K; g.eps = eps; g.S = S; g.T_max = T_max; g.d = d; g.ff = ff; g.H = H; g.KVH = KVH; g.hd = hd;
  if (const int rc = r.upload(s)) return rc;
  if (f13) {
    unsigned bad = 0;
    HIPCHK(c, hipMemsetAsync(dbad, 0, sizeof(unsigned), s));
    launch_pack_w13_rows(g.W, dWp, dWh, dbad, N, K, !c->w13_nz, s);
    HIPCHK(c, hipMemcpyAsync(&bad, dbad, sizeof(unsigned), hipMemcpyDeviceToHost, s));
    HIPCHK(c, hipStreamSynchronize(s));
    HIPCHK(c, hipMemsetAsync(dbad, scratch_fill, sizeof(unsigned), s));
    c->w13_op_bad_rows = (int)bad;
    if (!bad) { g.Wp = dWp; g.Wh = dWh; }
  }
  if (f13 && g.Wp && v13 != 0xff) launch_gemv_w13_variant(pro, epi, v13, g, s);
  else if (variant < 0) launch_gemv(pro, epi, g, s);
  else if (fmt == 1) launch_gemv_f8_variant(pro, epi, variant, g, s);
  else launch_gemv_variant(pro, epi, variant, g, s);
  return r.finish(s);
}


int dtk_op_rope_scatter(dtk_ctx* c, int form, const uint16_t* QKV, const float* part, int S, int part_rows, int T, int H, int KVH, int hd,
                        int T_max, int start_pos, const int32_t* rows, int max_pos, const uint16_t* rope_cos, const uint16_t* rope_sin,
                        int scratch_fill, uint16_t* q_io, uint16_t* k_io, uint16_t* v_io) {
  const char* who = "dtk_op_rope_scatter";
  if (!c || !rope_cos || !rope_sin || !q_io || !k_io || !v_io) return fail(c, DTK_ERR_ARG, "%s: null argument", who);
  if (form != 0 && form != 1) return fail(c, DTK_ERR_ARG, "%s: form %d (0 bf16 rows, 1 fp32 K-slice partials)", who, form);
  if (hd != 128 && hd != 64) return fail(c, DTK_ERR_ARG, "%s: head dim %d (128 or 64)", who, hd);
  if (T < 1 || H < 1 || KVH < 1 || H % KVH || T_max < 1 || max_pos < 1) return fail(c, DTK_ERR_ARG, "%s: T %d, H %d query heads over KVH %d key / value heads, T_max %d", who, T, H, KVH, T_max);
  if (scratch_fill < 0 || scratch_fill > 255) return fail(c, DTK_ERR_ARG, "%s: scratch_fill is a byte", who);
  if (form == 0 && !QKV) return fail(c, DTK_ERR_ARG, "%s: form 0 needs QKV", who);
  if (form == 1 && (!part || S < 1 || S > 8 || part_rows < T)) return fail(c, DTK_ERR_ARG, "%s: form 1 needs partials of S = 1..8 slices and part_rows >= T", who);
  for (int t = 0; t < T; ++t) {
    const int pos = rows ? rows[2 * t] : start_pos + t, row = rows ? rows[2 * t + 1] : start_pos + t;
    if (pos < 0 || pos >= max_pos || row < 0 || row >= T_max)
      return fail(c, DTK_ERR_ARG, "%s: row %d: position %d of %d, cache row %d of %d", who, t, pos, max_pos, row, T_max);
  }
  HIPCHK(c, hipSetDevice(c->device));
  hipStream_t s = c->stream;
  const size_t qkvn = (size_t)(H + 2 * KVH) * hd, kv = (size_t)KVH * T_max * hd;
  OpRun r(c, who, scratch_fill);
  const bf16_t* dQKV = r.in<bf16_t>(form == 0 ? QKV : nullptr, form == 0 ? (size_t)T * qkvn : 0);
  const float* dP = r.in<float>(form == 1 ? part : nullptr, form == 1 ? (size_t)S * part_rows * qkvn : 0);
  const bf16_t* dcos = r.in<bf16_t>(rope_cos, (size_t)max_pos * (hd / 2));
  const bf16_t* dsin = r.in<bf16_t>(rope_sin, (size_t)max_pos * (hd / 2));
  const int2* dR = r.in<int2>(rows, rows ? (size_t)T : 0);
  bf16_t* dq = r.io<bf16_t>(q_io, (size_t)H * T * hd, "q"); bf16_t* dk = r.io<bf16_t>(k_io, kv, "k"); bf16_t* dv = r.io<bf16_t>(v_io, kv, "v");
  if (const int rc = r.upload(s)) return rc;
  const long ps = (long)part_rows * (long)qkvn;
  if (form == 0 && rows) launch_rope_scatter_rows(dQKV, dq, dk, dv, dcos, dsin, T, dR, H, KVH, T_max, s, hd);
  else if (form == 0) launch_rope_scatter(dQKV, dq, dk, dv, dcos, dsin, T, start_pos, H, KVH, T_max, s, hd);
  else if (rows) launch_sk_rope_scatter_rows(dP, ps, S, dq, dk, dv, dcos, dsin, T, dR, H, KVH, T_max, s, hd);
  else launch_sk_rope_scatter(dP, ps, S, dq, dk, dv, dcos, dsin, T, start_pos, H, KVH, T_max, s, hd);
  return r.finish(s);
}

int dtk_op_rows_norm(dtk_ctx* c, int form, const uint16_t* X, const float* part, int S, int part_rows, const uint16_t* norm_w,
                     const uint16_t* ln_b, const uint16_t* bias, const uint16_t* residual, const uint16_t* gate, int flags, int M, int N,
                     int ldx, int ldc, int ldr, int ldy, float eps, int scratch_fill, uint16_t* c_io, uint16_t* y_io) {
  const char* who = "dtk_op_rows_norm";
  if (!c) return DTK_ERR_ARG;
  if (form < 0 || form > 3) return fail(c, DTK_ERR_ARG, "%s: form %d (0 rmsnorm_rows, 1 rmsnorm_rows_sk, 2 sk_reduce, 3 layernorm_rows)", who, form);
  if (M < 1 || N < 1 || scratch_fill < 0 || scratch_fill > 255) return fail(c, DTK_ERR_ARG, "%s: M, N >= 1, scratch_fill a byte", who);
  const bool in_place = form == 3 && !X;
  if (form != 2) {
// ... 199 lines not shown
  } else if (epi == EPI_SWIGLU) {
    if (ff < 8 || (ff & 7) || N != 2 * ff || !y_io) return fail(c, DTK_ERR_ARG, "%s: SWIGLU needs ff a multiple of 8 (as dtk_create), N = 2 ff and y", who);
  } else if (epi == EPI_LOGITS) {
    if (!logits_io) return fail(c, DTK_ERR_ARG, "%s: LOGITS needs the logits buffer", who);
  } else if (!y_io) return fail(c, DTK_ERR_ARG, "%s: RESID / STORE need y", who);
  HIPCHK(c, hipSetDevice(c->device));
  hipStream_t s = c->stream;
  const bool qkv = epi == EPI_QKV;
  const size_t kv_slot = qkv ? (size_t)KVH * T_max * 128 : 0;
  const size_t ny = epi == EPI_SWIGLU ? (size_t)((ff + 31) >> 5) * 512 : ((epi == EPI_STORE || epi == EPI_RESID) ? (size_t)nb * N : 0);
  BatchState hbs; memset(&hbs, 0, sizeof hbs);
  DecState hst[4]; memset(hst, 0, sizeof hst);
  for (int j = 0; j < DTK_MAX_BATCH; ++j) hbs.share_src[j] = -1;
  for (int b = 0; b < nb; ++b) { hbs.active[b] = active[b] ? 1 : 0; hst[b].pos = pos[b]; hst[b].next_pos = pos[b] + 1; }
  OpRun r(c, who, scratch_fill);
  GemvMvArgs g{};
  if (W8) { g.W8 = r.in<uint8_t>(W8, (size_t)N * K); g.wscale = r.in<float>(wscale, N); }
  else g.W = r.in<bf16_t>(W, (size_t)N * K);
  g.X = r.in<bf16_t>(X, x_layout ? (size_t)((K + 31) >> 5) * 512 : (size_t)nb * K);
  g.norm_w = r.in<bf16_t>(pro == PRO_RMSNORM ? norm_w : nullptr, pro == PRO_RMSNORM ? K : 0);
  g.rope_cos = r.in<bf16_t>(qkv ? rope_cos : nullptr, qkv ? (size_t)T_max * 64 : 0);
  g.rope_sin = r.in<bf16_t>(qkv ? rope_sin : nullptr, qkv ? (size_t)T_max * 64 : 0);
  g.st = r.in<DecState>(hst, 4);
  const BatchState* dbs = r.in<BatchState>(&hbs, 1);
  g.bs = bs_null ? nullptr : dbs;
  g.q_out = r.io<bf16_t>(qkv ? q_io : nullptr, qkv ? (size_t)nb * d : 0, "q");
  g.kcache = r.io<bf16_t>(qkv ? k_io : nullptr, (size_t)nb * kv_slot, "k");
  g.vcache = r.io<bf16_t>(qkv ? v_io : nullptr, (size_t)nb * kv_slot, "v");
  g.Y = r.io<bf16_t>(ny ? y_io : nullptr, ny, "y");
  g.logits = r.io<float>(epi == EPI_LOGITS ? logits_io : nullptr, epi == EPI_LOGITS ? (size_t)nb * N : 0, "logits");
  g.N = N; g.K = K; g.ldx = K; g.x_rowmajor = x_layout == 0; g.eps = eps; g.ldy = N; g.kv_slot_stride = kv_slot;
  g.T_max = T_max; g.d = d; g.ff = ff; g.H = H; g.KVH = KVH;
  if (const int rc = r.upload(s)) return rc;
  {
    MvShapeScope scope(epi, shape);
    launch_gemv_mv(pro, epi, nb, g, s);
  }
  return r.finish(s);
}

int dtk_w13_row_bytes(int K) { return (K < 8 || (K & 7)) ? -1 : (int)w13_row_bytes(K); }
int dtk_w13_pack_host(const uint16_t* W, int N, int K, uint8_t* planes, uint8_t* hb, int32_t* bad) {
  if (!W || !planes || !hb || !bad || N < 1 || K < 8 || (K & 7)) return DTK_ERR_ARG;
  for (int r = 0; r < N; ++r) bad[r] = w13_pack_row(W + (size_t)r * K, K, planes + (size_t)r * w13_row_bytes(K), hb + r);
  return DTK_OK;
}
int dtk_w13_unpack_host(const uint8_t* planes, const uint8_t* hb, int N, int K, uint16_t* W) {
  if (!W || !planes || !hb || N < 1 || K < 8 || (K & 7)) return DTK_ERR_ARG;
  for (int r = 0; r < N; ++r) w13_unpack_row(planes + (size_t)r * w13_row_bytes(K), hb[r], K, W + (size_t)r * K);
  return DTK_OK;
}
int dtk_w13_op_bad_rows(dtk_ctx* c) { return c ? c->w13_op_bad_rows : -1; }
int dtk_w13_flagged_rows(dtk_ctx* c, int role) { return (c && role >= 0 && role < 5 && c->w13_ready) ? (int)c->w13_zrows[role] : -1; }
int dtk_w13_row_bytes_host(const uint16_t* W, int N, int K, uint8_t* bytes) {
  if (!W || !bytes || N < 0 || K < 8 || (K & 7)) return DTK_ERR_ARG;
  for (int r = 0; r < N; ++r) bytes[r] = (uint8_t)w13_row_byte(W + (size_t)r * K, K);
  return DTK_OK;
}

extern "C++" {
namespace {
inline int op_nt_of(int nslots) { const int hi = nslots - 1; return hi < 16 ? 1 : (hi < 32 ? 2 : 4); }
const void* op_tiled_weights(OpRun& r, const uint16_t* W, const uint8_t* W8, const float* wscale, int N, int K, GemvBArgs& g) {
  g.N = N; g.K = K;
  if (W8) {
    const uint8_t* dW = r.in<uint8_t>(W8, (size_t)N * K);
    g.W8 = (uint8_t*)r.take(tiled_bytes_f8(N, K)); g.wscale = r.in<float>(wscale, N);
    return dW;
  }
  const bf16_t* dW = r.in<bf16_t>(W, (size_t)N * K);
  g.W = (bf16_t*)r.take(tiled_elems(N, K) * sizeof(bf16_t));
  return dW;
}
void op_retile(const void* rows, const GemvBArgs& g, hipStream_t s) {
  if (g.W8) launch_retile_f8((const uint8_t*)rows, const_cast<uint8_t*>(g.W8), g.N, g.K, s);
  else launch_retile((const bf16_t*)rows, const_cast<bf16_t*>(g.W), g.N, g.K, s);
}
struct OpBatchState {
  BatchState hbs; DecState hst[DTK_MAX_BATCH];
  OpBatchState(OpRun& r, const int32_t* active, const int32_t* pos, int nslots, GemvBArgs& g) {
    memset(&hbs, 0, sizeof hbs); memset(hst, 0, sizeof hst);
    for (int j = 0; j < DTK_MAX_BATCH; ++j) hbs.share_src[j] = -1;
    for (int j = 0; j < nslots; ++j) {
      hbs.active[j] = active[j] ? 1 : 0;
      if (pos) { hst[j].pos = pos[j]; hst[j].next_pos = pos[j] + 1; }
    }
    g.bs = r.in<BatchState>(&hbs, 1); g.st = r.in<DecState>(hst, DTK_MAX_BATCH); g.nt = op_nt_of(nslots);
  }
  OpBatchState(const OpBatchState&) = delete;
};
std::vector<bf16_t> op_x_fragments(const uint16_t* X, int nslots, int K) {
  const int nsteps = (K + 31) >> 5;
  std::vector<bf16_t> h((size_t)4 * nsteps * 512, (bf16_t)0);
  for (int j = 0; j < nslots; ++j)
    for (int k = 0; k < K; ++k) h[host_xtile_off(j, k, nsteps)] = X[(size_t)j * K + k];
  return h;
}
void op_x_rows(const bf16_t* frag, int nslots, int K, uint16_t* X) {
  const int nsteps = (K + 31) >> 5;
  for (int j = 0; j < nslots; ++j)
    for (int k = 0; k < K; ++k) X[(size_t)j * K + k] = frag[host_xtile_off(j, k, nsteps)];
}
}
}

int dtk_op_gemv_b(dtk_ctx* c, int epi, const uint16_t* W, const uint8_t* W8, const float* wscale, int N, int K,
// ... 364 lines not shown
```

### detikzify_amd/csrc/gemv_inl.h

```cpp
#pragma once
#include "common.h"
#include "w13.h"

template <int NR, int U>
__device__ __forceinline__ void gemv_load(u32x4 (&w)[NR][U], const u32x4* (&rows)[NR],
                                          int g, int lane, int K8) {
  if (64 * (g * U + U) <= K8) {
#pragma unroll
    for (int u = 0; u < U; ++u) {
      const int c = lane + 64 * (g * U + u);
#pragma unroll
      for (int r = 0; r < NR; ++r) w[r][u] = ld_nt(rows[r] + c);
    }
    return;
  }
#pragma unroll
  for (int u = 0; u < U; ++u) {
    const int c = lane + 64 * (g * U + u);
    const bool ok = c < K8;
#pragma unroll
    for (int r = 0; r < NR; ++r) {
      u32x4 z = {0u, 0u, 0u, 0u};
      w[r][u] = ok ? ld_nt(rows[r] + c) : z;
    }
// ... 55 lines not shown
#undef F4_WORD
  return c;
}

template <int NR, int U>
__device__ __forceinline__ void gemv_load_f4(u32x4 (&w)[NR][U], unsigned (&sc)[NR][U], const u32x4* (&rows)[NR], const uint8_t* (&srows)[NR],
                                             int g, int lane, int KC) {
  gemv_load<NR, U>(w, rows, g, lane, KC);
  const bool full = 64 * (g * U + U) <= KC;
#pragma unroll
  for (int u = 0; u < U; ++u) {
    const int c = lane + 64 * (g * U + u);
#pragma unroll
    for (int r = 0; r < NR; ++r) sc[r][u] = (full || c < KC) ? (unsigned)srows[r][c] : 127u;
  }
}

template <int NR, int U>
__device__ __forceinline__ void gemv_fma_f4(float (&acc)[NR], const u32x4 (&w)[NR][U], const unsigned (&sc)[NR][U],
                                            const u32x4* xs, int g, int lane, int KC) {
#pragma unroll
  for (int u = 0; u < U; ++u) {
    const int c = lane + 64 * (g * U + u);
    u32x4 x0 = {0u, 0u, 0u, 0u}, x1 = x0, x2 = x0, x3 = x0;
    if (64 * (g * U + U) <= KC || c < KC) {
      const int b = ((c >> 4) << 6) | (c & 15);
      x0 = xs[b]; x1 = xs[(b + 16) ^ 2]; x2 = xs[(b + 32) ^ 4]; x3 = xs[(b + 48) ^ 6];
    }
#pragma unroll
    for (int r = 0; r < NR; ++r) acc[r] = dot32_f4(w[r][u], f4_scale(sc[r][u]), x0, x1, x2, x3, acc[r]);
  }
}

typedef __attribute__((ext_vector_type(2))) unsigned short u16x2_t;

__device__ __forceinline__ uint32_t w13_high4(uint32_t codes, uint32_t lo2) {
  const uint32_t nz = ((codes + 0x0f0f0f0fu) >> 4) & 0x01010101u;
  const u16x2_t r = __builtin_bit_cast(u16x2_t, nz) * __builtin_bit_cast(u16x2_t, lo2) + __builtin_bit_cast(u16x2_t, codes);
  return __builtin_bit_cast(uint32_t, r);
}

template <bool NZ>
__device__ __forceinline__ float dot8_w13(uint32_t la, uint32_t lb, uint32_t n, uint32_t s, int i, uint32_t lo4, const u32x4& x, float c) {
  const uint32_t ce = n & 0x0f0f0f0fu, co = (n >> 4) & 0x0f0f0f0fu;
  const uint32_t he = (NZ ? ce + lo4 : w13_high4(ce, lo4 & 0x00ff00ffu)) | ((s << (7 - 2 * i)) & 0x80808080u);
  const uint32_t ho = (NZ ? co + lo4 : w13_high4(co, lo4 & 0x00ff00ffu)) | ((s << (6 - 2 * i)) & 0x80808080u);
  c = dot2(__builtin_amdgcn_perm(he, la, 0x05010400u), x[0], c);
  c = dot2(__builtin_amdgcn_perm(he, la, 0x07030602u), x[1], c);
  c = dot2(__builtin_amdgcn_perm(ho, lb, 0x05010400u), x[2], c);
  c = dot2(__builtin_amdgcn_perm(ho, lb, 0x07030602u), x[3], c);
  return c;
}

template <int NR, int U>
__device__ __forceinline__ void gemv_load_w13(u32x4 (&wl)[NR][U / 2], u32x2 (&wn)[NR][U / 2], uint32_t (&ws)[NR][U / 4],
                                              const u32x4* (&rows)[NR], int g, int lane, int J2, int n_off, int s_off) {
  static_assert(U % 4 == 0, "a stage is whole sign blocks");
  if (2 * (g * (U / 4) + U / 4) <= J2) {
#pragma unroll
    for (int ub = 0; ub < U / 4; ++ub) {
      const int b = g * (U / 4) + ub;
#pragma unroll
      for (int r = 0; r < NR; ++r) {
        const unsigned char* p = reinterpret_cast<const unsigned char*>(rows[r]);
#pragma unroll
        for (int h = 0; h < 2; ++h) {
          wl[r][2 * ub + h] = ld_nt(rows[r] + ((2 * b + h) * 64 + lane));
          wn[r][2 * ub + h] = __builtin_nontemporal_load(reinterpret_cast<const u32x2*>(p + n_off) + ((2 * b + h) * 64 + lane));
        }
        ws[r][ub] = __builtin_nontemporal_load(reinterpret_cast<const uint32_t*>(p + s_off) + (b * 64 + lane));
      }
    }
    return;
  }
#pragma unroll
  for (int ub = 0; ub < U / 4; ++ub) {
    const int b = g * (U / 4) + ub;
#pragma unroll
    for (int r = 0; r < NR; ++r) {
      const unsigned char* p = reinterpret_cast<const unsigned char*>(rows[r]);
#pragma unroll
      for (int h = 0; h < 2; ++h) {
        const bool ok = 2 * b + h < J2;
        const u32x4 zl = {0u, 0u, 0u, 0u};
        const u32x2 zn = {0u, 0u};
        wl[r][2 * ub + h] = ok ? ld_nt(rows[r] + ((2 * b + h) * 64 + lane)) : zl;
        wn[r][2 * ub + h] = ok ? __builtin_nontemporal_load(reinterpret_cast<const u32x2*>(p + n_off) + ((2 * b + h) * 64 + lane)) : zn;
      }
      ws[r][ub] = (2 * b < J2) ? __builtin_nontemporal_load(reinterpret_cast<const uint32_t*>(p + s_off) + (b * 64 + lane)) : 0u;
    }
  }
}

template <int NR, int U, bool NZ>
__device__ __forceinline__ void gemv_fma_w13(float (&acc)[NR], const u32x4 (&wl)[NR][U / 2], const u32x2 (&wn)[NR][U / 2],
                                             const uint32_t (&ws)[NR][U / 4], const uint32_t (&lo4)[NR],
                                             const u32x4* xs, int g, int lane, int K8) {
  const bool full = 64 * (g * U + U) <= K8;
#pragma unroll
  for (int u = 0; u < U; ++u) {
    const int c = lane + 64 * (g * U + u);
    u32x4 xv = {0u, 0u, 0u, 0u};
    if (full || c < K8) xv = xs[c];
#pragma unroll
    for (int r = 0; r < NR; ++r) {
      const u32x4& l = wl[r][u >> 1];
      acc[r] = dot8_w13<NZ>((u & 1) ? l[2] : l[0], (u & 1) ? l[3] : l[1], wn[r][u >> 1][u & 1], ws[r][u >> 2], u & 3, lo4[r], xv, acc[r]);
    }
  }
}
```

### detikzify_amd/csrc/kernels.h

```cpp
#pragma once
#include "common.h"
#include <stdlib.h>
#include <string.h>

enum { PRO_COPY = 0, PRO_RMSNORM = 1, PRO_ATTN = 2 };
enum { EPI_STORE = 0, EPI_RESID = 1, EPI_QKV = 2, EPI_SWIGLU = 3, EPI_LOGITS = 4 };

struct GemvArgs {
  const bf16_t* W;
  const uint8_t* W8;
  const float* wscale;
  int N;
  int K;
  const bf16_t* x;
  const bf16_t* norm_w;
  float eps;
  const float* pm;
  const float* pl;
  const float* po;
  int S;
  bf16_t* y;
  float* logits;
  bf16_t* q_out;
  bf16_t* kcache;
  bf16_t* vcache;
  const bf16_t* rope_cos;
  const bf16_t* rope_sin;
  const DecState* st;
  int T_max;
  int d;
  int ff;
  int H;
  int KVH;
  int hd = 128;
  const uint8_t* W4 = nullptr;
  const uint8_t* S4 = nullptr;
  const uint8_t* Wp = nullptr;
  const uint8_t* Wh = nullptr;
};

void launch_gemv(int pro, int epi, const GemvArgs& a, hipStream_t s);
void launch_gemv_q4(int pro, int epi, const GemvArgs& a, hipStream_t s);
void launch_gemv_variant(int pro, int epi, int variant, const GemvArgs& a, hipStream_t s);
void launch_gemv_w13_variant(int pro, int epi, int variant, const GemvArgs& a, hipStream_t s);
bool gemv_w13_has(int pro, int epi, int variant);
bool gemv_w13_takes(int pro, int epi, const GemvArgs& a);
void launch_pack_w13_rows(const bf16_t* W, uint8_t* Wp, uint8_t* Wh, unsigned* bad_rows, int N, int K, bool zflag_all, hipStream_t s);
void launch_gemv_f8(int pro, int epi, const GemvArgs& a, hipStream_t s);
void launch_gemv_f8_variant(int pro, int epi, int variant, const GemvArgs& a, hipStream_t s);
void set_gemv_default_variant(int epi, int variant);

struct AttnDecArgs {
  const bf16_t* q;
  const bf16_t* kcache;
  const bf16_t* vcache;
  const DecState* st;
  float* pm; float* pl; float* po;
  int H; int S; int T_max; float scale;
  int combine;
  bf16_t* out;
  unsigned* counters;
  int G;
  int threads;
  int hd = 128;
};
void launch_attn_decode(const AttnDecArgs& a, hipStream_t s);

struct SampleArgs {
  const float* logits; int V;
  const SamplingDev* sp;
  DecState* st;
  const bf16_t* embed;
  bf16_t* x;
  int d;
  int64_t* tok_ring;
  int ring;
  float* probs_out;
  int advance;
  int step_override;
  const BatchState* bs;
  int logits_stride;
  int nslots;
  SampleMB* mb;
  float2* lp_ring = nullptr;
  int trunc = 0;
  float* lse_ring = nullptr;
  const PenDev* pen = nullptr;
  const uint16_t* pen_cnt = nullptr;
  int pen_stride = 0;
  int32_t* pen_tok = nullptr;
  const DryDev* dry = nullptr;
  const uint8_t* dry_m = nullptr;
  int dry_stride = 0;
  const LenDev* len = nullptr;
  const float* len_m = nullptr;
  int len_m_stride = 0;
  const float* bias = nullptr;
  int bias_stride = 0;
  int len_cur = -1;
};
// ... 287 lines not shown
```

### detikzify_amd/csrc/kernels_decode.hip

```cpp
#include <cstdlib>
#include <cstring>
#include "kernels.h"
#include "gemv_inl.h"

template <int EPI, bool F8, int HD = 128>
__device__ __forceinline__ void gemv_epilogue(const GemvArgs& a, int u, float a0, float a1, float pre0, float pre1, int pos) {
    constexpr int HD2 = HD / 2, HSH = HD == 128 ? 6 : 5;
    static_assert(HD == 128 || HD == 64, "head dim 128 or 64");
    if (F8) {
      if (EPI == EPI_QKV) {
        const int r0 = (u >> HSH) * HD + (u & (HD2 - 1));
        a0 *= a.wscale[r0];
        a1 *= a.wscale[r0 + HD2];
      } else if (EPI == EPI_SWIGLU) {
        a0 *= a.wscale[u];
        a1 *= a.wscale[a.ff + u];
      } else {
        a0 *= a.wscale[u];
      }
    }
    if (EPI == EPI_STORE) {
      a.y[u] = f2bf(a0);
    } else if (EPI == EPI_RESID) {
      a.y[u] = f2bf(pre0 + rbf(a0));
// ... 18 lines not shown
        const float c = pre0, s = pre1;
        const float o1 = rbf(rbf(x1 * c) + rbf(-x2 * s));
        const float o2 = rbf(rbf(x2 * c) + rbf(x1 * s));
        bf16_t* dst = (sec == 0) ? (a.q_out + head * HD)
                                 : (a.kcache + ((size_t)head * a.T_max + pos) * HD);
        dst[i] = f2bf(o1);
        dst[i + HD2] = f2bf(o2);
      }
    }
}

template <int PRO, int EPI, int R, int U, int WAVES, bool PERSIST, bool F8 = false, int KS = 1, int HD = 128, bool F4 = false, bool W13 = false, int FW = WAVES>
__global__ __launch_bounds__(WAVES * 64) void k_gemv(GemvArgs a) {
  static_assert(!(F4 && F8) && !(W13 && (F4 || F8)), "one weight format");
  static_assert(FW >= 1 && FW <= WAVES, "the folding threads are the block's first");
  constexpr int FT = FW * 64;
  constexpr bool FALL = FW == WAVES;
  constexpr bool PAIRED = (EPI == EPI_QKV) || (EPI == EPI_SWIGLU);
  constexpr int NR = PAIRED ? 2 * R : R;
  constexpr int THREADS = WAVES * 64;
  constexpr int RW = WAVES / KS;
  constexpr int HD2 = HD / 2, HC = HD / 8;
  constexpr int HSH = HD == 128 ? 6 : 5, CSH = HSH - 2;
  static_assert(HD == 128 || HD == 64, "head dim 128 or 64");
  static_assert(WAVES % KS == 0 && (KS == 1 || !PERSIST), "split-K variants are not persistent");
  extern __shared__ __attribute__((aligned(16))) unsigned char smem[];
  u32x4* xs = reinterpret_cast<u32x4*>(smem);
  const int K8 = a.K >> 3;
  const int KC = F4 ? ((a.K + 31) >> 5) : (F8 ? (a.K >> 4) : K8);
  const size_t row_bytes = W13 ? w13_row_bytes(a.K) : (F4 ? (size_t)KC * 16 : (F8 ? (size_t)a.K : (size_t)a.K * 2));
  const unsigned char* Wb = reinterpret_cast<const unsigned char*>(W13 ? (const void*)a.Wp : (F4 ? (const void*)a.W4 : (F8 ? (const void*)a.W8 : (const void*)a.W)));
  const int J2 = W13 ? w13_units(a.K) : 0, n13 = W13 ? (int)w13_n_off(a.K) : 0, s13 = W13 ? (int)w13_s_off(a.K) : 0;
  float* red = reinterpret_cast<float*>(smem + (size_t)(F4 ? f4_xrows(KC) : K8) * 16);
#define XI(c) (F4 ? f4_xswz(c) : (c))

  const int tid = threadIdx.x;
  const int lane = tid & 63;
  const int wave = tid >> 6;
  const int rw = KS > 1 ? wave / KS : wave;
  const int ks = KS > 1 ? wave % KS : 0;

  int n_units;
  if (EPI == EPI_QKV) n_units = (a.N >> 1);
  else if (EPI == EPI_SWIGLU) n_units = a.ff;
  else n_units = a.N;
  const int chunk_stride = PERSIST ? (int)gridDim.x * WAVES : 0;
  int chunk = PERSIST ? (int)blockIdx.x + (int)gridDim.x * wave : (int)blockIdx.x * RW + rw;
  int unit0 = chunk * R;

  const u32x4* rows[NR];
  const uint8_t* srows[NR];
  uint32_t lo4[NR];
  bool zrow = false;
  auto set_rows = [&](int u0) {
    unsigned zb = 0;
#pragma unroll
    for (int j = 0; j < R; ++j) {
      int u = u0 + j;
      if (u >= n_units) u = n_units - 1;
      int r0, r1 = 0;
      if (EPI == EPI_QKV) {
        r0 = (u >> HSH) * HD + (u & (HD2 - 1));
        r1 = r0 + HD2;
      } else if (EPI == EPI_SWIGLU) {
        r0 = u;
        r1 = a.ff + u;
      } else {
        r0 = u;
      }
      if (PAIRED) {
        rows[2 * j] = reinterpret_cast<const u32x4*>(Wb + (size_t)r0 * row_bytes);
        rows[2 * j + 1] = reinterpret_cast<const u32x4*>(Wb + (size_t)r1 * row_bytes);
      } else {
        rows[j] = reinterpret_cast<const u32x4*>(Wb + (size_t)r0 * row_bytes);
      }
      if (F4) {
        if (PAIRED) { srows[2 * j] = a.S4 + (size_t)r0 * KC; srows[2 * j + 1] = a.S4 + (size_t)r1 * KC; }
        else srows[j] = a.S4 + (size_t)r0 * KC;
      }
      if (W13) {
        const unsigned b0 = a.Wh[r0], b1 = PAIRED ? a.Wh[r1] : 0u;
        if (PAIRED) { lo4[2 * j] = (uint32_t)w13_lo(b0) * 0x01010101u; lo4[2 * j + 1] = (uint32_t)w13_lo(b1) * 0x01010101u; }
        else lo4[j] = (uint32_t)w13_lo(b0) * 0x01010101u;
        zb |= b0 | b1;
      }
    }
    if (W13 && PRO == PRO_RMSNORM) zrow = (__builtin_amdgcn_readfirstlane((int)zb) & W13_ZROW) != 0;
  };
  set_rows(unit0);

  const int iters = (KC + 63) >> 6;
  const int Gall = (iters + U - 1) / U;
  const int G = KS > 1 ? (Gall - ks + KS - 1) / KS : Gall;
#define GIDX(g) (KS > 1 ? ks + KS * (g) : (g))
  u32x4 wa[NR][U], wb[NR][U];
  unsigned sa[NR][U], sb[NR][U];
  constexpr int UW = W13 ? U : 4;
  u32x4 lwa[NR][UW / 2], lwb[NR][UW / 2];
  u32x2 nwa[NR][UW / 2], nwb[NR][UW / 2];
  uint32_t zwa[NR][UW / 4], zwb[NR][UW / 4];
  float acc[NR];
#define GLOAD(w, sc, g) do { if (W13) gemv_load_w13<NR, UW>(l##w, n##w, z##w, rows, (g), lane, J2, n13, s13); else if (F4) gemv_load_f4<NR, U>(w, sc, rows, srows, (g), lane, KC); else gemv_load<NR, U>(w, rows, (g), lane, KC); } while (0)
#define GFMA(w, sc, g) do { if (W13) gemv_fma_w13<NR, UW, NZ>(acc, l##w, n##w, z##w, lo4, xs, (g), lane, K8); else if (F4) gemv_fma_f4<NR, U>(acc, w, sc, xs, (g), lane, KC); else if (F8) gemv_fma_f8<NR, U>(acc, w, xs, (g), lane, KC); else gemv_fma<NR, U>(acc, w, xs, (g), lane, KC); } while (0)

  if (G > 0) GLOAD(wa, sa, GIDX(0));

  float pre0[R], pre1[R];
  int pos = 0;
  if (EPI == EPI_QKV) pos = a.st->pos;
  auto prefetch_epilogue = [&](int u0) {
#pragma unroll
    for (int j = 0; j < R; ++j) {
      pre0[j] = 0.f; pre1[j] = 0.f;
      if (lane == 0 && ks == 0) {
        int u = u0 + j;
        if (u >= n_units) u = n_units - 1;
        if (EPI == EPI_RESID) pre0[j] = bf2f(a.y[u]);
        if (EPI == EPI_QKV) {
          pre0[j] = bf2f(a.rope_cos[(size_t)pos * HD2 + (u & (HD2 - 1))]);
          pre1[j] = bf2f(a.rope_sin[(size_t)pos * HD2 + (u & (HD2 - 1))]);
        }
      }
    }
  };
  if (EPI == EPI_RESID || EPI == EPI_QKV) prefetch_epilogue(unit0);

  if (PRO == PRO_COPY) {
    const u32x4* x4 = reinterpret_cast<const u32x4*>(a.x);
    for (int c = tid; c < K8; c += THREADS) xs[XI(c)] = x4[c];
  } else if (PRO == PRO_RMSNORM) {
    const u32x4* x4 = reinterpret_cast<const u32x4*>(a.x);
    const u32x4* w4 = reinterpret_cast<const u32x4*>(a.norm_w);
    if (K8 <= 2 * FT) {
      const int c0 = tid, c1 = tid + FT;
      const bool h0 = (FALL || tid < FT) && c0 < K8, h1 = (FALL || tid < FT) && c1 < K8;
      const u32x4 zz = {0u, 0u, 0u, 0u};
      const u32x4 v0 = h0 ? x4[c0] : zz, v1 = h1 ? x4[c1] : zz;
      const u32x4 g0 = h0 ? w4[c0] : zz, g1 = h1 ? w4[c1] : zz;
      float ss = 0.f;
#pragma unroll
      for (int e = 0; e < 4; ++e) {
        const float lo = pk_lo(v0[e]), hi = pk_hi(v0[e]);
        ss += lo * lo;
        ss += hi * hi;
      }
#pragma unroll
      for (int e = 0; e < 4; ++e) {
        const float lo = pk_lo(v1[e]), hi = pk_hi(v1[e]);
        ss += lo * lo;
        ss += hi * hi;
      }
      ss = wave_sum(ss);
      if (lane == 0) red[wave] = ss;
      __syncthreads();
      float tot = 0.f;
#pragma unroll
      for (int w = 0; w < FW; ++w) tot += red[w];
      const float inv = rsqrtf(tot / (float)a.K + a.eps);
// ... 47 lines not shown
        float m4[4];
#pragma unroll
        for (int j = 0; j < 4; ++j) m4[j] = (s0 + j < S) ? pmh[s0 + j] : -1e30f;
#pragma unroll
        for (int j = 0; j < 4; ++j) M = fmaxf(M, m4[j]);
      }
      float L = 0.f;
      float o[8];
#pragma unroll
      for (int e = 0; e < 8; ++e) o[e] = 0.f;
      for (int s0 = 0; s0 < S; s0 += 4) {
        float m4[4], l4[4];
        f32x4 p0[4], p1[4];
#pragma unroll
        for (int j = 0; j < 4; ++j) {
          const bool ok = s0 + j < S;
          const int sj = ok ? s0 + j : s0;
          m4[j] = ok ? pmh[sj] : -1e30f;
          l4[j] = ok ? plh[sj] : 0.f;
          const f32x4* po4 = reinterpret_cast<const f32x4*>(a.po + ((size_t)(head * S + sj)) * HD + d0);
          p0[j] = po4[0];
          p1[j] = po4[1];
        }
#pragma unroll
        for (int j = 0; j < 4; ++j) {
          if (s0 + j < S) {
            const float w = __expf(m4[j] - M);
            L += w * l4[j];
#pragma unroll
            for (int e = 0; e < 4; ++e) {
              o[e] += w * p0[j][e];
              o[4 + e] += w * p1[j][e];
            }
          }
        }
      }
      const float invL = 1.f / L;
      u32x4 ov;
#pragma unroll
      for (int e = 0; e < 4; ++e) ov[e] = pack2(o[2 * e] * invL, o[2 * e + 1] * invL);
      xs[XI(c)] = ov;
    }
  }
  if (F4) {
    const u32x4 zz = {0u, 0u, 0u, 0u};
    for (int c = K8 + tid; c < 4 * KC; c += THREADS) xs[XI(c)] = zz;
  }
  __syncthreads();

  for (;;) {
    const bool active = unit0 < n_units;
#pragma unroll
    for (int r = 0; r < NR; ++r) acc[r] = 0.f;
#define MAIN_LOOP(NZV) do {                                   \
      constexpr bool NZ = NZV;                                 \
      for (int g = 0; g < G; g += 2) {                         \
        if (g + 1 < G) GLOAD(wb, sb, GIDX(g + 1));             \
        GFMA(wa, sa, GIDX(g));                                 \
        if (g + 1 < G) {                                       \
          if (g + 2 < G) GLOAD(wa, sa, GIDX(g + 2));           \
          GFMA(wb, sb, GIDX(g + 1));                           \
        }                                                      \
      }                                                        \
    } while (0)
    if constexpr (W13 && PRO == PRO_RMSNORM) {
      if (zrow) MAIN_LOOP(false);
      else MAIN_LOOP(true);
    } else {
      MAIN_LOOP(false);
    }
#undef MAIN_LOOP
    const int cur = unit0;
    float q0[R], q1[R];
#pragma unroll
    for (int j = 0; j < R; ++j) { q0[j] = pre0[j]; q1[j] = pre1[j]; }
    if (PERSIST) {
      chunk += chunk_stride;
      unit0 = chunk * R;
      if (unit0 < n_units) {
        set_rows(unit0);
        GLOAD(wa, sa, 0);
        if (EPI == EPI_RESID || EPI == EPI_QKV) prefetch_epilogue(unit0);
      }
    }
#pragma unroll
    for (int r = 0; r < NR; ++r) acc[r] = wave_sum(acc[r]);
    if (KS > 1) {
      float* part = red + WAVES;
      if (lane == 0) {
#pragma unroll
        for (int r = 0; r < NR; ++r) part[(rw * NR + r) * KS + ks] = acc[r];
      }
      __syncthreads();
      if (ks == 0 && lane == 0) {
#pragma unroll
        for (int r = 0; r < NR; ++r) {
          float t = part[(rw * NR + r) * KS];
#pragma unroll
          for (int k = 1; k < KS; ++k) t += part[(rw * NR + r) * KS + k];
          acc[r] = t;
        }
      }
    }

    if (active && lane == 0 && ks == 0) {
#pragma unroll
      for (int j = 0; j < R; ++j) {
        const int u = cur + j;
        if (u >= n_units) break;
        gemv_epilogue<EPI, F8, HD>(a, u, PAIRED ? acc[2 * j] : acc[j], PAIRED ? acc[2 * j + 1] : 0.f, q0[j], q1[j], pos);
      }
    }
    if (!PERSIST || unit0 >= n_units) break;
  }
#undef GIDX
#undef GLOAD
#undef GFMA
#undef XI
}

static int num_cus() {
  static int n = 0;
  if (!n) {
    int dev = 0;
    hipDeviceProp_t p;
    if (hipGetDevice(&dev) == hipSuccess && hipGetDeviceProperties(&p, dev) == hipSuccess) n = p.multiProcessorCount;
    if (n <= 0) n = 256;
  }
  return n;
}

template <int PRO, int EPI, int R, int U, int WAVES, bool PERSIST, int KS = 1>
static void launch_gemv_t(const GemvArgs& a, hipStream_t s, int blocks_per_cu) {
  int n_units = (EPI == EPI_QKV) ? (a.N >> 1) : (EPI == EPI_SWIGLU ? a.ff : a.N);
  const int per_block = (WAVES / KS) * R;
  int grid = (n_units + per_block - 1) / per_block;
  if (PERSIST) {
    const int cap = num_cus() * (blocks_per_cu > 0 ? blocks_per_cu : 2);
    if (grid > cap) grid = cap;
  }
  const size_t lds = (size_t)(a.K >> 3) * 16 + 64 + 1024;
  if constexpr (EPI == EPI_QKV || PRO == PRO_ATTN) {
    if (a.hd == 64) { hipLaunchKernelGGL((k_gemv<PRO, EPI, R, U, WAVES, PERSIST, false, KS, 64>), dim3(grid), dim3(WAVES * 64), lds, s, a); return; }
  }
  hipLaunchKernelGGL((k_gemv<PRO, EPI, R, U, WAVES, PERSIST, false, KS>), dim3(grid), dim3(WAVES * 64), lds, s, a);
}

struct GemvShape { int R, U, waves, ks; bool persist; };
#define GV(PRO, EPI, R, U, W, P, BPC) do { if (q) { *q = GemvShape{R, U, W, 1, P}; return; } return launch_gemv_t<PRO, EPI, R, U, W, P>(a, s, BPC); } while (0)
#define GVK(PRO, EPI, R, U, W, KS) do { if (q) { *q = GemvShape{R, U, W, KS, false}; return; } return launch_gemv_t<PRO, EPI, R, U, W, false, KS>(a, s, 0); } while (0)
static void gemv_variant_row(int pro, int epi, int variant, const GemvArgs& a, hipStream_t s, GemvShape* q) {
  if (pro == PRO_RMSNORM && epi == EPI_QKV) {
    switch (variant) {
      default: GV(PRO_RMSNORM, EPI_QKV, 1, 2, 4, false, 0);
      case 8: GV(PRO_RMSNORM, EPI_QKV, 2, 2, 4, false, 0);
      case 9: GV(PRO_RMSNORM, EPI_QKV, 1, 1, 4, false, 0);
      case 10: GV(PRO_RMSNORM, EPI_QKV, 1, 2, 8, false, 0);
      case 11: GV(PRO_RMSNORM, EPI_QKV, 1, 2, 2, false, 0);
      case 1: GV(PRO_RMSNORM, EPI_QKV, 1, 4, 4, false, 0);
      case 2: GV(PRO_RMSNORM, EPI_QKV, 2, 2, 8, false, 0);
      case 3: GV(PRO_RMSNORM, EPI_QKV, 2, 2, 4, true, 4);
      case 4: GV(PRO_RMSNORM, EPI_QKV, 2, 2, 8, true, 2);
      case 5: GV(PRO_RMSNORM, EPI_QKV, 1, 4, 8, true, 2);
      case 6: GV(PRO_RMSNORM, EPI_QKV, 4, 1, 4, false, 0);
      case 7: GV(PRO_RMSNORM, EPI_QKV, 1, 2, 4, false, 0);
    }
  }
  if (pro == PRO_RMSNORM && epi == EPI_SWIGLU) {
    switch (variant) {
// ... 117 lines not shown
                 case 2: F8(PRO_RMSNORM, EPI_LOGITS, 4, 4, 4); case 3: F8(PRO_RMSNORM, EPI_LOGITS, 8, 2, 4); }
  }
  if (pro == PRO_ATTN && epi == EPI_RESID) F8(PRO_ATTN, EPI_RESID, 2, 2, 4);
  switch (v) { default: F8(PRO_COPY, EPI_RESID, 2, 4, 4); case 0: F8(PRO_COPY, EPI_RESID, 1, 4, 4);
               case 2: F8(PRO_COPY, EPI_RESID, 2, 8, 4); case 3: F8(PRO_COPY, EPI_RESID, 4, 4, 4);
               case 4: F8(PRO_COPY, EPI_RESID, 2, 4, 8); case 5: F8(PRO_COPY, EPI_RESID, 1, 8, 4);
               case 6: F8P(PRO_COPY, EPI_RESID, 1, 4, 4, 4); case 7: F8P(PRO_COPY, EPI_RESID, 2, 4, 4, 4);
               case 8: F8P(PRO_COPY, EPI_RESID, 1, 4, 8, 2); case 9: F8P(PRO_COPY, EPI_RESID, 1, 8, 4, 4); }
}
#undef F8
#undef F8P

template <int PRO, int EPI, int R, int U, int WAVES, bool PERSIST = false, int BPC = 2>
static void launch_gemv_q4_t(const GemvArgs& a, hipStream_t s) {
  int n_units = (EPI == EPI_QKV) ? (a.N >> 1) : (EPI == EPI_SWIGLU ? a.ff : a.N);
  const int per_block = WAVES * R;
  int grid = (n_units + per_block - 1) / per_block;
  if (PERSIST && grid > num_cus() * BPC) grid = num_cus() * BPC;
  const int KC = (a.K + 31) >> 5;
  const size_t lds = (size_t)((4 * KC + 63) & ~63) * 16 + 64 + 1024;
  if constexpr (EPI == EPI_QKV || PRO == PRO_ATTN) {
    if (a.hd == 64) { hipLaunchKernelGGL((k_gemv<PRO, EPI, R, U, WAVES, PERSIST, false, 1, 64, true>), dim3(grid), dim3(WAVES * 64), lds, s, a); return; }
  }
  hipLaunchKernelGGL((k_gemv<PRO, EPI, R, U, WAVES, PERSIST, false, 1, 128, true>), dim3(grid), dim3(WAVES * 64), lds, s, a);
}
#define Q4(PRO, EPI, R, U, W) return launch_gemv_q4_t<PRO, EPI, R, U, W>(a, s)
#define Q4P(PRO, EPI, R, U, W, BPC) return launch_gemv_q4_t<PRO, EPI, R, U, W, true, BPC>(a, s)
void launch_gemv_q4(int pro, int epi, const GemvArgs& a, hipStream_t s) {
  if (pro == PRO_RMSNORM && epi == EPI_QKV) Q4P(PRO_RMSNORM, EPI_QKV, 1, 2, 8, 2);
  if (pro == PRO_RMSNORM && epi == EPI_SWIGLU) Q4P(PRO_RMSNORM, EPI_SWIGLU, 1, 2, 8, 2);
  if (pro == PRO_ATTN && epi == EPI_RESID) Q4(PRO_ATTN, EPI_RESID, 2, 2, 4);
  if (pro == PRO_COPY && epi == EPI_RESID) Q4(PRO_COPY, EPI_RESID, 2, 2, 4);
  if (pro == PRO_RMSNORM && epi == EPI_STORE) Q4(PRO_RMSNORM, EPI_STORE, 2, 2, 4);
  if (pro == PRO_COPY && epi == EPI_STORE) Q4(PRO_COPY, EPI_STORE, 2, 2, 4);
  fprintf(stderr, "launch_gemv_q4: no MXFP4 kernel for prologue %d, epilogue %d\n", pro, epi);
  abort();
}
#undef Q4
#undef Q4P

template <int PRO, int EPI, int R, int U, int WAVES, bool PERSIST = false, int KS = 1, int BPC = 2, int FW0 = 0>
static void launch_gemv_w13_t(const GemvArgs& a, hipStream_t s) {
  int n_units = (EPI == EPI_QKV) ? (a.N >> 1) : (EPI == EPI_SWIGLU ? a.ff : a.N);
  const int per_block = (WAVES / KS) * R;
  int grid = (n_units + per_block - 1) / per_block;
  if (PERSIST && grid > num_cus() * BPC) grid = num_cus() * BPC;
  const size_t lds = (size_t)(a.K >> 3) * 16 + 64 + 1024;
  constexpr int FW = FW0 ? FW0 : WAVES;
  if constexpr (EPI == EPI_QKV || PRO == PRO_ATTN) {
    if (a.hd == 64) { hipLaunchKernelGGL((k_gemv<PRO, EPI, R, U, WAVES, PERSIST, false, KS, 64, false, true, FW>), dim3(grid), dim3(WAVES * 64), lds, s, a); return; }
  }
  hipLaunchKernelGGL((k_gemv<PRO, EPI, R, U, WAVES, PERSIST, false, KS, 128, false, true, FW>), dim3(grid), dim3(WAVES * 64), lds, s, a);
}
#define WV(PRO, EPI, R, U, W) return launch_gemv_w13_t<PRO, EPI, R, U, W>(a, s)
#define WVP(PRO, EPI, R, U, W, BPC) return launch_gemv_w13_t<PRO, EPI, R, U, W, true, 1, BPC>(a, s)
#define WVK(PRO, EPI, R, U, W, KS) return launch_gemv_w13_t<PRO, EPI, R, U, W, false, KS>(a, s)
#define WVF(PRO, EPI, R, U, W, BPC, FW) return launch_gemv_w13_t<PRO, EPI, R, U, W, true, 1, BPC, FW>(a, s)
bool gemv_w13_has(int pro, int epi, int v) {
  if (pro == PRO_RMSNORM && (epi == EPI_QKV || epi == EPI_SWIGLU)) return v >= 0 && v <= 7;
  if (pro == PRO_COPY && epi == EPI_RESID) return v >= 0 && v <= 6;
  if (pro == PRO_ATTN && epi == EPI_RESID) return v >= 0 && v <= 2;
  if (pro == PRO_RMSNORM && epi == EPI_LOGITS) return v >= 0 && v <= 7;
  if (pro == PRO_RMSNORM && epi == EPI_STORE) return v >= 0 && v <= 1;
  if (pro == PRO_COPY && epi == EPI_STORE) return v == 0;
  return false;
}
void launch_gemv_w13_variant(int pro, int epi, int v, const GemvArgs& a, hipStream_t s) {
  if (pro == PRO_RMSNORM && epi == EPI_QKV) {
    switch (v) { default: WV(PRO_RMSNORM, EPI_QKV, 1, 4, 4); case 1: WV(PRO_RMSNORM, EPI_QKV, 2, 4, 4); case 2: WV(PRO_RMSNORM, EPI_QKV, 1, 4, 8);
                 case 3: WVP(PRO_RMSNORM, EPI_QKV, 1, 4, 8, 2); case 4: WV(PRO_RMSNORM, EPI_QKV, 1, 8, 4);
                 case 5: WVP(PRO_RMSNORM, EPI_QKV, 1, 4, 4, 4);
                 case 6: WVF(PRO_RMSNORM, EPI_QKV, 1, 4, 8, 2, 4); case 7: WVF(PRO_RMSNORM, EPI_QKV, 1, 4, 16, 1, 4); }
  }
  if (pro == PRO_RMSNORM && epi == EPI_SWIGLU) {
    switch (v) { default: WV(PRO_RMSNORM, EPI_SWIGLU, 1, 4, 4); case 1: WV(PRO_RMSNORM, EPI_SWIGLU, 2, 4, 4); case 2: WV(PRO_RMSNORM, EPI_SWIGLU, 1, 4, 8);
                 case 3: WVP(PRO_RMSNORM, EPI_SWIGLU, 1, 4, 8, 2); case 4: WV(PRO_RMSNORM, EPI_SWIGLU, 1, 8, 4);
                 case 5: WVP(PRO_RMSNORM, EPI_SWIGLU, 1, 4, 4, 4);
                 case 6: WVF(PRO_RMSNORM, EPI_SWIGLU, 1, 4, 8, 2, 4); case 7: WVF(PRO_RMSNORM, EPI_SWIGLU, 1, 4, 16, 1, 4); }
  }
  if (pro == PRO_COPY && epi == EPI_RESID) {
    switch (v) { default: WV(PRO_COPY, EPI_RESID, 1, 8, 8); case 1: WV(PRO_COPY, EPI_RESID, 1, 4, 8); case 2: WV(PRO_COPY, EPI_RESID, 2, 4, 4);
                 case 3: WVK(PRO_COPY, EPI_RESID, 1, 4, 8, 2); case 4: WVK(PRO_COPY, EPI_RESID, 2, 4, 8, 2);
                 case 5: WV(PRO_COPY, EPI_RESID, 1, 4, 4); case 6: WV(PRO_COPY, EPI_RESID, 1, 4, 16); }
  }
  if (pro == PRO_ATTN && epi == EPI_RESID) {
    switch (v) { default: WVK(PRO_ATTN, EPI_RESID, 2, 4, 16, 2); case 1: WV(PRO_ATTN, EPI_RESID, 2, 4, 8); case 2: WV(PRO_ATTN, EPI_RESID, 2, 4, 4); }
  }
  if (pro == PRO_RMSNORM && epi == EPI_LOGITS) {
    switch (v) { default: WV(PRO_RMSNORM, EPI_LOGITS, 1, 4, 4); case 1: WV(PRO_RMSNORM, EPI_LOGITS, 2, 4, 4); case 2: WVP(PRO_RMSNORM, EPI_LOGITS, 1, 4, 8, 2);
                 case 3: WVP(PRO_RMSNORM, EPI_LOGITS, 2, 4, 8, 2); case 4: WV(PRO_RMSNORM, EPI_LOGITS, 2, 4, 8);
                 case 5: WVF(PRO_RMSNORM, EPI_LOGITS, 2, 4, 8, 2, 4); case 6: WVF(PRO_RMSNORM, EPI_LOGITS, 1, 4, 8, 2, 4);
                 case 7: WVF(PRO_RMSNORM, EPI_LOGITS, 2, 4, 16, 1, 4); }
  }
  if (pro == PRO_RMSNORM && epi == EPI_STORE) { if (v == 1) WVF(PRO_RMSNORM, EPI_STORE, 2, 4, 8, 2, 4); WV(PRO_RMSNORM, EPI_STORE, 2, 4, 4); }
  if (pro == PRO_COPY && epi == EPI_STORE) WV(PRO_COPY, EPI_STORE, 2, 4, 4);
  fprintf(stderr, "launch_gemv_w13: no 13-bit kernel for prologue %d, epilogue %d\n", pro, epi);
  abort();
}
#undef WV
#undef WVP
#undef WVK
#undef WVF
static int w13_shape_for(int pro, int epi, int v, const GemvArgs& a) {
  const GemvShape sh = gemv_variant_shape(pro, epi, v);
  if (pro == PRO_ATTN) return -1;
  if (pro == PRO_COPY && epi == EPI_RESID) {
    if (a.K == a.d) return -1;
    if (sh.ks == 1) return 1;
    return (sh.ks == 2 && sh.U == 4) ? 3 : -1;
  }
  const bool big = a.K >= 4096;
  if (pro == PRO_RMSNORM && epi == EPI_QKV) return sh.waves == 4 ? (big ? 6 : 5) : (sh.waves == 8 ? 3 : -1);
  if (pro == PRO_RMSNORM && epi == EPI_SWIGLU) return sh.waves == 4 ? 5 : (sh.waves == 8 ? 3 : -1);
  if (pro == PRO_RMSNORM && epi == EPI_LOGITS) return sh.waves == 4 ? (big ? 5 : 1) : (sh.waves == 8 ? 4 : -1);
  if (pro == PRO_RMSNORM && epi == EPI_STORE) return sh.waves == 4 ? 0 : -1;
  if (pro == PRO_COPY && epi == EPI_STORE) return 0;
  return -1;
}

__global__ __launch_bounds__(256) void k_pack_w13_rows(const bf16_t* W, uint8_t* Wp, uint8_t* Wh, unsigned* bad_rows, int N, int K, int zflag_all) {
  const int row = blockIdx.x, tid = threadIdx.x;
  const u32x4* w4 = reinterpret_cast<const u32x4*>(W + (size_t)row * K);
  unsigned char* out = Wp + (size_t)row * w13_row_bytes(K);
  __shared__ int red[4], redq[4];
  __shared__ int any_bad;
  const int K8 = K >> 3, J2 = w13_units(K), J4 = w13_blocks(K);
  int hb = 0, qmin = 127;
  for (int c = tid; c < K8; c += 256) {
    const u32x4 v = w4[c];
#pragma unroll
    for (int e = 0; e < 4; ++e) {
      const int q0 = (int)((v[e] >> 8) & 0x7fu), q1 = (int)((v[e] >> 24) & 0x7fu);
      hb = max(hb, max(q0, q1));
      qmin = min(qmin, min(q0, q1));
    }
  }
#pragma unroll
  for (int off = 32; off >= 1; off >>= 1) { hb = max(hb, __shfl_xor(hb, off)); qmin = min(qmin, __shfl_xor(qmin, off)); }
  if ((tid & 63) == 0) { red[tid >> 6] = hb; redq[tid >> 6] = qmin; }
  if (tid == 0) any_bad = 0;
  __syncthreads();
  hb = max(max(red[0], red[1]), max(red[2], red[3]));
  qmin = min(min(redq[0], redq[1]), min(redq[2], redq[3]));
  if (tid == 0) Wh[row] = (uint8_t)(hb | ((qmin == 0 || zflag_all) ? W13_ZROW : 0));
  const int lo = w13_lo(hb);
  int bad = 0;
  for (int t = tid; t < J4 * 64; t += 256) {
    const int b = t >> 6, l = t & 63;
    uint32_t sg = 0;
#pragma unroll
    for (int h = 0; h < 2; ++h) {
      const int j = 2 * b + h;
      if (j >= J2) break;
      u32x4 lv;
      u32x2 nv;
#pragma unroll
      for (int i2 = 0; i2 < 2; ++i2) {
        const int i = 2 * h + i2, c = 256 * b + 64 * i + l;
        u32x4 v = {0u, 0u, 0u, 0u};
        if (c < K8) v = w4[c];
        uint32_t la = 0, lb = 0, n = 0;
#pragma unroll
        for (int k = 0; k < 8; ++k) {
          unsigned wk = (v[k >> 1] >> (16 * (k & 1))) & 0xffffu;
          int code = w13_code(wk, lo);
          if (code < 0) { ++bad; code = 0; wk = 0; }
          const int kb = 8 * (k & 3);
          if (k < 4) la |= (wk & 0xffu) << kb; else lb |= (wk & 0xffu) << kb;
          n |= (uint32_t)code << (kb + 4 * (k >> 2));
          sg |= (wk >> 15) << (kb + 2 * i + (k >> 2));
        }
        lv[2 * i2] = la; lv[2 * i2 + 1] = lb; nv[i2] = n;
      }
      reinterpret_cast<u32x4*>(out)[j * 64 + l] = lv;
      reinterpret_cast<u32x2*>(out + w13_n_off(K))[j * 64 + l] = nv;
    }
    reinterpret_cast<uint32_t*>(out + w13_s_off(K))[b * 64 + l] = sg;
  }
  if (bad) atomicOr(&any_bad, 1);
  __syncthreads();
  if (tid == 0 && any_bad) atomicAdd(bad_rows, 1u);
}
void launch_pack_w13_rows(const bf16_t* W, uint8_t* Wp, uint8_t* Wh, unsigned* bad_rows, int N, int K, bool zflag_all, hipStream_t s) {
  hipLaunchKernelGGL(k_pack_w13_rows, dim3(N), dim3(256), 0, s, W, Wp, Wh, bad_rows, N, K, zflag_all ? 1 : 0);
}

static int g_variant[8] = {0, 0, 0, 0, 0, -1, 0, 0};
void set_gemv_default_variant(int epi, int variant) { if (epi >= 0 && epi < 8) g_variant[epi] = variant; }

static int gemv_chosen_variant(int pro, int epi, const GemvArgs& a) {
  if (pro == PRO_ATTN) return g_variant[6] ? g_variant[6] : (a.d > 2048 ? 8 : 1);
  int v = g_variant[epi & 7];
  const bool o_proj = epi == EPI_RESID && a.K == a.d;
  if (o_proj && g_variant[5] >= 0) v = g_variant[5];
  if (v == 0 && a.d > 0 && a.d <= 2048) {
    if (epi == EPI_SWIGLU) v = 5;
    else if (epi == EPI_RESID) v = o_proj ? 1 : 15;
    else if (epi == EPI_LOGITS) v = 3;
  } else if (v == 0 && a.d > 2048) {
    if (epi == EPI_RESID) v = 10;
    else if (epi == EPI_LOGITS) v = 3;
  }
  return v;
}

void launch_gemv(int pro, int epi, const GemvArgs& a, hipStream_t s) {
  if (a.W4) return launch_gemv_q4(pro, epi, a, s);
  if (a.W8) return launch_gemv_f8(pro, epi, a, s);
  const int v = gemv_chosen_variant(pro, epi, a);
  const int v13 = a.Wp ? w13_shape_for(pro, epi, v, a) : -1;
  if (v13 >= 0) return launch_gemv_w13_variant(pro, epi, v13, a, s);
  launch_gemv_variant(pro, epi, v, a, s);
}
bool gemv_w13_takes(int pro, int epi, const GemvArgs& a) { return w13_shape_for(pro, epi, gemv_chosen_variant(pro, epi, a), a) >= 0; }

__global__ __launch_bounds__(256) void k_attn_decode(AttnDecArgs a) {
  const int h = blockIdx.x, sp = blockIdx.y;
  const int tid = threadIdx.x, lane = tid & 63, wave = tid >> 6;
  const int sub = lane & 15;
  const int grp = lane >> 4;
  const int n = a.st->pos + 1;
  int chunk = (n + a.S - 1) / a.S;
  chunk = (chunk + 15) & ~15;
  const int j_begin = sp * chunk;
  const int j_end = min(n, j_begin + chunk);

  const u32x4 qv = reinterpret_cast<const u32x4*>(a.q + h * 128)[sub];
  const int kvh = h / a.G;
  const bf16_t* kbase = a.kcache + (size_t)kvh * a.T_max * 128;
  const bf16_t* vbase = a.vcache + (size_t)kvh * a.T_max * 128;

  float m = -1e30f, l = 0.f;
  float o[8];
#pragma unroll
  for (int e = 0; e < 8; ++e) o[e] = 0.f;

  for (int j0 = j_begin; j0 < j_end; j0 += 64) {
    u32x4 kv[4], vv[4];
    bool ok[4];
#pragma unroll
    for (int i = 0; i < 4; ++i) {
      const int j = j0 + i * 16 + wave * 4 + grp;
      ok[i] = j < j_end;
      const int jj = ok[i] ? j : j_begin;
      kv[i] = reinterpret_cast<const u32x4*>(kbase + (size_t)jj * 128)[sub];
      vv[i] = reinterpret_cast<const u32x4*>(vbase + (size_t)jj * 128)[sub];
    }
#pragma unroll
    for (int i = 0; i < 4; ++i) {
      float s = dot8(qv, kv[i], 0.f);
      s += __shfl_xor(s, 1, 64);
      s += __shfl_xor(s, 2, 64);
      s += __shfl_xor(s, 4, 64);
      s += __shfl_xor(s, 8, 64);
      s *= a.scale;
      if (ok[i]) {
        const float mn = fmaxf(m, s);
        const float corr = __expf(m - mn);
        const float p = __expf(s - mn);
        l = l * corr + p;
#pragma unroll
        for (int e = 0; e < 4; ++e) {
          o[2 * e] = o[2 * e] * corr + p * pk_lo(vv[i][e]);
          o[2 * e + 1] = o[2 * e + 1] * corr + p * pk_hi(vv[i][e]);
        }
        m = mn;
      }
// ... 1244 lines not shown
```

### detikzify_amd/csrc/w13.h

```cpp
#pragma once
#include <stddef.h>
#include <stdint.h>

#if defined(__HIPCC__) || defined(__CUDACC__)
#define W13_HD __host__ __device__
#else
#define W13_HD
#endif

W13_HD static inline int w13_units(int K) { return ((K >> 3) + 127) >> 7; }
W13_HD static inline int w13_blocks(int K) { return (w13_units(K) + 1) >> 1; }
W13_HD static inline size_t w13_n_off(int K) { return (size_t)w13_units(K) * 1024; }
W13_HD static inline size_t w13_s_off(int K) { return (size_t)w13_units(K) * 1536; }
W13_HD static inline size_t w13_row_bytes(int K) { return (size_t)w13_units(K) * 1536 + (size_t)w13_blocks(K) * 256; }
#define W13_ZROW 0x80
W13_HD static inline int w13_lo(int hb) { hb &= 0x7f; return hb > 15 ? hb - 15 : 0; }
W13_HD static inline int w13_high(int code, int lo) { return code ? lo + code : 0; }
W13_HD static inline int w13_high_nz(int code, int lo) { return lo + code; }

struct W13Pos { size_t l, n, s; int nshift, sbit; };
W13_HD static inline W13Pos w13_pos(int K, int k) {
  const int c = k >> 3, e = k & 7, lane = c & 63;
  W13Pos p;
  p.l = (size_t)((c >> 7) * 64 + lane) * 16 + (size_t)(((c >> 6) & 1) * 8 + e);
  p.n = w13_n_off(K) + (size_t)((c >> 7) * 64 + lane) * 8 + (size_t)(((c >> 6) & 1) * 4 + (e & 3));
  p.nshift = (e >> 2) * 4;
  p.s = w13_s_off(K) + (size_t)((c >> 8) * 64 + lane) * 4 + (size_t)(e & 3);
  p.sbit = 2 * ((c >> 6) & 3) + (e >> 2);
  return p;
}

static inline int w13_row_hb(const uint16_t* w, int K) {
  int hb = 0;
  for (int k = 0; k < K; ++k) { const int q = (w[k] >> 8) & 0x7f; if (q > hb) hb = q; }
  return hb;
}
static inline int w13_row_byte(const uint16_t* w, int K) {
  int z = 0;
  for (int k = 0; k < K; ++k) if (((w[k] >> 8) & 0x7f) == 0) z = W13_ZROW;
  return w13_row_hb(w, K) | z;
}
W13_HD static inline int w13_code(unsigned w, int lo) {
  const int q = (int)((w >> 8) & 0x7fu);
  if (q == 0) return 0;
  return q > lo ? q - lo : -1;
}
static inline int w13_pack_row(const uint16_t* w, int K, uint8_t* row, uint8_t* hb_out) {
  const int hb = w13_row_hb(w, K), lo = w13_lo(hb);
  int bad = 0;
  const size_t nb = w13_row_bytes(K);
  for (size_t i = 0; i < nb; ++i) row[i] = 0;
  for (int k = 0; k < K; ++k) {
    const int code = w13_code(w[k], lo);
    if (code < 0) { ++bad; continue; }
    const W13Pos p = w13_pos(K, k);
    row[p.l] = (uint8_t)(w[k] & 0xff);
    row[p.n] = (uint8_t)(row[p.n] | (code << p.nshift));
    row[p.s] = (uint8_t)(row[p.s] | (((w[k] >> 15) & 1) << p.sbit));
  }
  *hb_out = (uint8_t)hb;
  return bad;
}
static inline void w13_unpack_row(const uint8_t* row, int hb, int K, uint16_t* w) {
  const int lo = w13_lo(hb);
  for (int k = 0; k < K; ++k) {
    const W13Pos p = w13_pos(K, k);
    const int code = (row[p.n] >> p.nshift) & 15, sign = (row[p.s] >> p.sbit) & 1;
    w[k] = (uint16_t)((sign << 15) | (w13_high(code, lo) << 8) | row[p.l]);
  }
}
static inline void w13_unpack_row_nz(const uint8_t* row, int hb, int K, uint16_t* w) {
  const int lo = w13_lo(hb);
  for (int k = 0; k < K; ++k) {
    const W13Pos p = w13_pos(K, k);
    const int code = (row[p.n] >> p.nshift) & 15, sign = (row[p.s] >> p.sbit) & 1;
    w[k] = (uint16_t)((sign << 15) | (w13_high_nz(code, lo) << 8) | row[p.l]);
  }
}
```

### include/dtk.h

```cpp
#ifndef DTK_H
#define DTK_H

#include <stdint.h>

#ifdef __cplusplus
extern "C" {
#endif

#define DTK_ABI_VERSION 7

typedef struct dtk_ctx dtk_ctx;

enum { DTK_F32 = 0, DTK_BF16 = 1, DTK_F16 = 2 };

enum {
  DTK_OK = 0,
  DTK_ERR_ARG = -1,
  DTK_ERR_HIP = -2,
  DTK_ERR_STATE = -3,
  DTK_ERR_RANGE = -4
};

typedef struct dtk_config {
  int32_t hidden;
// ... 258 lines not shown
                    float* Y, uint8_t* x8_out, uint8_t* xs_out, uint8_t* y8_out, uint8_t* ys_out);
int  dtk_op_attention(dtk_ctx* ctx, const uint16_t* Q, const uint16_t* K, const uint16_t* V,
                      int H, int Tq, int Tk, int hd, int causal, int q_offset, uint16_t* O);
int  dtk_op_attention_seg(dtk_ctx* ctx, const uint16_t* Q, const uint16_t* K, const uint16_t* V,
                          int H, int Tq, int Tk, int hd, int shared_len, const int32_t* seg_begin, const int32_t* kv_row, uint16_t* O);
int  dtk_op_attn_decode(dtk_ctx* ctx, const uint16_t* q, const uint16_t* K, const uint16_t* V, int H, int KVH, int hd, int T_max,
                        const int32_t* pos, int npos, int threads, int splits, int mode, int variant, uint16_t* out,
                        float* pm_out, float* pl_out, float* po_out);
int  dtk_op_attn_decode_b(dtk_ctx* ctx, const uint16_t* q, const uint16_t* K, const uint16_t* V, int nslots, int H, int KVH, int T_max,
                          const int32_t* pos, const int32_t* active, const int32_t* share_src, const int32_t* share_len,
                          int use_prefix, int pfx_splits, int tail_threads, int gqa_fused, int attn_nt, uint16_t* out);
int  dtk_op_attn_decode_b8(dtk_ctx* ctx, const uint16_t* q, const uint16_t* K, const uint16_t* V, int nslots, int H, int KVH, int T_max,
                           const int32_t* pos, const int32_t* active, const int32_t* share_src, const int32_t* share_len,
                           const int32_t* kv8_from, uint8_t* k8_codes, uint8_t* k8_scales, uint8_t* v8_codes, uint8_t* v8_scales,
                           int use_prefix, int pfx_splits, int tail_threads, int gqa_fused, int attn_nt, uint16_t* out);
int  dtk_op_gemv_b(dtk_ctx* ctx, int epi, const uint16_t* W, const uint8_t* W8, const float* wscale, int N, int K,
                   const uint16_t* X, const uint16_t* norm_w, float eps, const int32_t* active, const int32_t* pos, int nslots,
                   int d, int ff, int H, int KVH, int T_max, const uint16_t* rope_cos, const uint16_t* rope_sin,
                   uint16_t* q_io, uint16_t* k_io, uint16_t* v_io, uint16_t* y_io, uint16_t* frag_io, float* logits_io,
                   uint16_t* xn_out, uint32_t* err_out);
int  dtk_op_gemv_bkp(dtk_ctx* ctx, const uint16_t* W, const uint8_t* W8, const float* wscale, int N, int K, const uint16_t* X,
                     const int32_t* active, int nslots, const uint16_t* norm_w, float eps, uint16_t* resid_io, uint16_t* xn_io,
                     float* part_out, uint32_t* err_out);
int  dtk_op_gemv_role(dtk_ctx* ctx, int pro, int epi, int variant, const uint16_t* W, const uint8_t* W8, const float* wscale,
                      const uint8_t* W4, const uint8_t* S4, int N, int K, int d, int ff, int H, int KVH, int hd, int T_max, int pos, float eps,
                      const uint16_t* x, const uint16_t* norm_w, const uint16_t* rope_cos, const uint16_t* rope_sin,
                      int S, const float* pm, const float* pl, const float* po, int scratch_fill,
                      uint16_t* q_io, uint16_t* k_io, uint16_t* v_io, uint16_t* y_io, float* logits_io);
#define DTK_EPI_GATED_RESIDUAL 8
int  dtk_op_rope_scatter(dtk_ctx* ctx, int form, const uint16_t* QKV, const float* part, int S, int part_rows, int T, int H, int KVH, int hd,
                         int T_max, int start_pos, const int32_t* rows, int max_pos, const uint16_t* rope_cos, const uint16_t* rope_sin,
                         int scratch_fill, uint16_t* q_io, uint16_t* k_io, uint16_t* v_io);
int  dtk_op_rows_norm(dtk_ctx* ctx, int form, const uint16_t* X, const float* part, int S, int part_rows, const uint16_t* norm_w,
                      const uint16_t* ln_b, const uint16_t* bias, const uint16_t* residual, const uint16_t* gate, int flags, int M, int N,
                      int ldx, int ldc, int ldr, int ldy, float eps, int scratch_fill, uint16_t* c_io, uint16_t* y_io);
int  dtk_op_swiglu(dtk_ctx* ctx, int form, const uint16_t* GU, const float* part, int S, int part_rows, const uint16_t* A, const uint16_t* W,
                   int M, int ff, int K, int ldact, int scratch_fill, uint16_t* act_io);
int  dtk_op_attention_ex(dtk_ctx* ctx, const uint16_t* Q, int64_t nq, const uint16_t* K, int64_t nk, const uint16_t* V, int64_t nv,
                         uint16_t* o_io, int64_t no, const int64_t* strides, int H, int kv_group, int Tq, int Tk, int hd, int causal,
                         int q_offset, int nbatch, int scratch_fill);
int  dtk_op_rows_move(dtk_ctx* ctx, int form, const int32_t* ids, const uint16_t* src, const float* pixels, int M, int D, int V, int lds,
                      int ldd, int image, int patch, int scratch_fill, uint16_t* dst_io);
int  dtk_op_gemv_mv_role(dtk_ctx* ctx, int pro, int epi, int nb, int shape, const uint16_t* W, const uint8_t* W8, const float* wscale,
                         int N, int K, int d, int ff, int H, int KVH, int T_max, const int32_t* pos, const int32_t* active, int bs_null,
                         int x_layout, const uint16_t* X, const uint16_t* norm_w, float eps, const uint16_t* rope_cos,
                         const uint16_t* rope_sin, int scratch_fill, uint16_t* q_io, uint16_t* k_io, uint16_t* v_io, uint16_t* y_io,
                         float* logits_io);
int  dtk_w13_row_bytes(int K);
int  dtk_w13_pack_host(const uint16_t* W, int N, int K, uint8_t* planes, uint8_t* hb, int32_t* bad);
int  dtk_w13_unpack_host(const uint8_t* planes, const uint8_t* hb, int N, int K, uint16_t* W);
int  dtk_w13_op_bad_rows(dtk_ctx* ctx);
int  dtk_w13_row_bytes_host(const uint16_t* W, int N, int K, uint8_t* bytes);
int  dtk_w13_flagged_rows(dtk_ctx* ctx, int role);
int  dtk_op_layernorm(dtk_ctx* ctx, const uint16_t* X, const uint16_t* w, const uint16_t* b,
                      int M, int D, float eps, uint16_t* Y);
int  dtk_op_sample(dtk_ctx* ctx, const float* logits, int V, int step, int64_t* token_out,
                   float* filtered_probs_out);

int  dtk_decode_wait_lp(dtk_ctx* ctx, int64_t* token_out, float* lp_out );
int  dtk_decode_batch_wait_lp(dtk_ctx* ctx, int64_t* tokens_out , float* logprob_out ,
                              float* sample_logprob_out );
int  dtk_engine_read_lp(dtk_engine* e, int slot, int64_t* tokens_out, float* logprob_out, float* sample_logprob_out, int cap,
                        int32_t* n_out, int32_t* state_out, int timeout_ms);
int  dtk_engine_set_wait_lp_op(dtk_engine* e, int (*wait_lp)(void* dev, int64_t* tokens_out, float* logprob_out, float* sample_logprob_out));
int  dtk_op_sample_lp(dtk_ctx* ctx, const float* logits, int V, int step, int64_t* token_out, float* filtered_probs_out,
                      float* lp_out );

#define DTK_MAX_TOP 8
int  dtk_score_top(dtk_ctx* ctx, const int64_t* ids, int T, const float* pixels, uint64_t image_key, uint32_t flags, int first,
                   float* logprob_out, int32_t* argmax_out, float* lse_out, int k, int32_t* top_ids_out, float* top_logprob_out);
int  dtk_score_top_text(dtk_ctx* ctx, const int64_t* ids, int T, const float* pixels, uint64_t image_key, const int64_t* text_ids, int T_text,
                        uint64_t text_key, uint32_t flags, int first, float* logprob_out, int32_t* argmax_out, float* lse_out,
                        int k, int32_t* top_ids_out, float* top_logprob_out);
int  dtk_score_packed_top(dtk_ctx* ctx, const int64_t* prefix_ids, int P, const float* pixels, uint64_t image_key, uint32_t flags,
                          const int64_t* cand_ids, const int32_t* cand_len, int N, float* logprob_out, int32_t* argmax_out, float* lse_out,
                          int k, int32_t* top_ids_out, float* top_logprob_out);
int  dtk_score_packed_top_text(dtk_ctx* ctx, const int64_t* prefix_ids, int P, const float* pixels, uint64_t image_key, const int64_t* text_ids,
                               int T_text, uint64_t text_key, uint32_t flags, const int64_t* cand_ids, const int32_t* cand_len, int N,
                               float* logprob_out, int32_t* argmax_out, float* lse_out, int k, int32_t* top_ids_out, float* top_logprob_out);
int  dtk_op_score_top(dtk_ctx* ctx, const uint16_t* Xn, const uint16_t* W, const int32_t* targets, int M, int N, int K, int flags,
                      float* logprob_out, float* lse_out, int32_t* argmax_out, float* zmax_out, int k, int32_t* top_ids_out,
                      float* top_logprob_out, float* top_z_out);
int  dtk_decode_wait_top(dtk_ctx* ctx, int64_t* token_out, float* lp_out , int32_t* top_ids_out ,
                         float* top_logprob_out );
int  dtk_decode_batch_wait_top(dtk_ctx* ctx, int64_t* tokens_out , float* logprob_out ,
                               float* sample_logprob_out , int32_t* top_ids_out ,
                               float* top_logprob_out );

int  dtk_set_sampling_ext(dtk_ctx* ctx, const dtk_sampling_ext* x);
int  dtk_set_sampling_slot_ext(dtk_ctx* ctx, int slot, const dtk_sampling_ext* x);
int  dtk_op_sample_ext(dtk_ctx* ctx, const float* logits, int V, int step, int64_t* token_out, float* filtered_probs_out,
                       float* lp_out , const dtk_sampling_ext* x);
int  dtk_engine_submit_ext(dtk_engine* e, dtk_join* j, const dtk_sampling_ext* x, const int64_t* text_ids, int n_text, uint64_t text_key,
                           uint64_t* ticket_out);
int  dtk_engine_set_sampling_ext_op(dtk_engine* e, int (*set_sampling_slot_ext)(void* dev, int slot, const dtk_sampling_ext* x));

int  dtk_set_penalties(dtk_ctx* ctx, float presence, float frequency, int start);
int  dtk_set_penalties_slot(dtk_ctx* ctx, int slot, float presence, float frequency, int start);
int  dtk_op_sample_pen(dtk_ctx* ctx, const float* logits, int V, int step, int64_t* token_out, float* filtered_probs_out,
                       float* lp_out , const dtk_sampling_ext* x , float presence, float frequency,
                       const int64_t* counted_ids, int n_counted);
int  dtk_token_counts(dtk_ctx* ctx, int slot, uint16_t* out, int V);
int  dtk_engine_submit_pen(dtk_engine* e, dtk_join* j, const dtk_sampling_ext* x , float presence, float frequency, int start,
                           const int64_t* text_ids, int n_text, uint64_t text_key, uint64_t* ticket_out);
int  dtk_engine_set_penalties_op(dtk_engine* e, int (*set_penalties_slot)(void* dev, int slot, float presence, float frequency, int start));

// ... 84 lines not shown
```

Before: 416.5 tokens/s.

## Add narrow 12-bit w13 row encoding that skips the sign plane for eligible row groups

Rows whose exponent codes all stay at least 8 above the row's low exponent are flagged as narrow at pack time. For those rows the sign bit is folded into the 4-bit nibble, so the GEMV kernels can skip loading the separate sign plane. Flags are computed per kernel row-group so a whole group shares one load path, with a per-row flag byte stored after the high-byte array. The aim is fewer weight bytes streamed per decode token. The cost is extra pack-time work, a flag read per row, and new kernel template paths.

```diff
diff --git a/detikzify_amd/_lib.py b/detikzify_amd/_lib.py
--- a/detikzify_amd/_lib.py
+++ b/detikzify_amd/_lib.py
@@ -239,6 +239,10 @@
     "dtk_w13_op_bad_rows": (C.c_int, [_P]),
     "dtk_w13_row_bytes_host": (C.c_int, [_P, C.c_int, C.c_int, _P]),
     "dtk_w13_flagged_rows": (C.c_int, [_P, C.c_int]),
+    "dtk_w13_narrow_rows": (C.c_int, [_P, C.c_int]),
+    "dtk_w13_op_narrow_rows": (C.c_int, [_P]),
+    "dtk_w13_pack_narrow_host": (C.c_int, [_P, C.c_int, C.c_int, _P, _P, _P, _P]),
+    "dtk_w13_unpack_narrow_host": (C.c_int, [_P, _P, _P, C.c_int, C.c_int, _P]),
     "dtk_op_gemv": (C.c_int, [_P, _P, _P, _P, C.c_int, C.c_int, C.c_int, C.c_float, _P]),
     "dtk_op_gemv_mv": (C.c_int, [_P, _P, _P, _P, C.c_int, C.c_int, C.c_int, C.c_float, C.c_int, _P]),
     "dtk_op_gemv_q4": (C.c_int, [_P, _P, _P, _P, C.c_int, C.c_int, C.c_int, C.c_float, _P, _P]),
diff --git a/detikzify_amd/csrc/dtk_api.hip b/detikzify_amd/csrc/dtk_api.hip
--- a/detikzify_amd/csrc/dtk_api.hip
+++ b/detikzify_amd/csrc/dtk_api.hip
@@ -573,6 +573,9 @@
 }
 
 static inline bool w13_on(const dtk_ctx* c) { return c->wfmt == 0 && c->w13 != 0; }
+static const uint8_t* w13_flags(const dtk_ctx* c, int pro, int epi, const GemvArgs& g, int v13 = -1) {
+  return (g.Wp && g.Wh && c->w13_narrow && gemv_w13_group(pro, epi, v13, g, c->w13_narrow == 2).mode) ? g.Wh + g.N : nullptr;
+}
 
 void decode_step_launches(dtk_ctx* c, bool with_probe, bool short_ctx = false) {
   hipStream_t s = c->stream;
@@ -617,17 +620,20 @@
     g.Wp = p13 ? w.p13_wgu : nullptr; g.Wh = w.h13_wgu;
     const bool probe_here = with_probe && (l == c->L / 2);
     if (probe_here) (void)hipEventRecord(c->probe_a, s);
+    if (g.Wp) g.Wn = w13_flags(c, PRO_RMSNORM, EPI_SWIGLU, g);
     launch_gemv(PRO_RMSNORM, EPI_SWIGLU, g, s);
     if (probe_here) (void)hipEventRecord(c->probe_b, s);
     g.W = w.wdown; g.W8 = w.q_wdown; g.wscale = w.s_wdown; g.N = c->d; g.K = c->ff; g.x = c->act; g.y = c->x;
     g.W4 = w.f4_wdown; g.S4 = w.e4_wdown;
     g.Wp = p13 ? w.p13_wdown : nullptr; g.Wh = w.h13_wdown;
+    if (g.Wp) g.Wn = w13_flags(c, PRO_COPY, EPI_RESID, g);
     launch_gemv(PRO_COPY, EPI_RESID, g, s);
   }
   GemvArgs g{};
   if (w13_on(c) && c->w13_ready) { g.Wp = c->p13_lm_head; g.Wh = c->h13_lm_head; }
   g.W = c->lm_head; g.W8 = c->q_lm_head; g.wscale = c->s_lm_head; g.N = c->V; g.K = c->d; g.x = c->x; g.norm_w = c->final_norm;
-  g.eps = c->cfg.rms_eps; g.logits = c->logits;
+  g.eps = c->cfg.rms_eps; g.logits = c->logits; g.d = c->d; g.ff = c->ff; g.hd = c->hd;
+  if (g.Wp) g.Wn = w13_flags(c, PRO_RMSNORM, EPI_LOGITS, g);
   launch_gemv(PRO_RMSNORM, EPI_LOGITS, g, s);
 }
 
@@ -872,26 +878,29 @@
       W += mat(w.p13_wqkv, (uint64_t)c->d + 2 * kvd, c->d) + mat(w.p13_wo, (uint64_t)c->d, c->d) + mat(w.p13_wgu, (uint64_t)2 * c->ff, c->d) +
            mat(w.p13_wdown, (uint64_t)c->d, c->ff);
     }
+    for (uint64_t sk : c->w13_sskip) W -= sk;
+    W += c->w13_flag_bytes;
     c->stats.weight_bytes_per_token = W;
-    c->stats.probe_kernel_bytes = mat(c->layers[c->L / 2].p13_wgu, (uint64_t)2 * c->ff, c->d);
+    c->stats.probe_kernel_bytes = mat(c->layers[c->L / 2].p13_wgu, (uint64_t)2 * c->ff, c->d) + c->w13_flag_bytes_probe - c->w13_sskip_probe;
   }
 }
 static void w13_set_stats(dtk_ctx* c) {
   const uint32_t rows = c->w13_bad_rows > 4095u ? 4095u : c->w13_bad_rows;
   c->stats.w13_counts = (c->w13_packed & 1023u) | ((c->w13_unpacked & 1023u) << 10) | (rows << 20);
 }
-static int w13_pack_one(dtk_ctx* c, int role, int pro, int epi, const bf16_t* W, int N, int K, uint8_t** planes, uint8_t** hb) {
+static int w13_pack_one(dtk_ctx* c, int role, int pro, int epi, const bf16_t* W, int N, int K, uint8_t** planes, uint8_t** hb, bool probe = false) {
   GemvArgs g{};
-  g.N = N; g.K = K; g.d = c->d; g.ff = c->ff; g.hd = c->hd;
+  g.N = N; g.K = K; g.d = c->d; g.ff = c->ff; g.hd = c->hd; g.H = c->H; g.KVH = c->KVH;
   if (!gemv_w13_takes(pro, epi, g)) {
     if (*planes) { (void)hipFree(*planes); *planes = nullptr; }
     if (*hb) { (void)hipFree(*hb); *hb = nullptr; }
     return DTK_OK;
   }
   if (!*planes) HIPCHK(c, hipMalloc((void**)planes, (size_t)N * w13_row_bytes(K)));
-  if (!*hb) HIPCHK(c, hipMalloc((void**)hb, (size_t)N));
+  if (!*hb) HIPCHK(c, hipMalloc((void**)hb, (size_t)2 * N));
   HIPCHK(c, hipMemsetAsync(c->w13_bad, 0, sizeof(unsigned), c->stream));
-  launch_pack_w13_rows(W, *planes, *hb, c->w13_bad, N, K, !c->w13_nz, c->stream);
+  const W13Group grp = c->w13_narrow ? gemv_w13_group(pro, epi, -1, g, c->w13_narrow == 2) : W13Group{};
+  launch_pack_w13_rows(W, *planes, *hb, c->w13_bad, N, K, !c->w13_nz, grp, c->stream);
   unsigned bad = 0;
   HIPCHK(c, hipMemcpyAsync(&bad, c->w13_bad, sizeof(unsigned), hipMemcpyDeviceToHost, c->stream));
   HIPCHK(c, hipStreamSynchronize(c->stream));
@@ -901,9 +910,14 @@
     c->w13_unpacked++; c->w13_bad_rows += bad;
   } else {
     c->w13_packed++;
-    std::vector<uint8_t> bytes((size_t)N);
-    HIPCHK(c, hipMemcpy(bytes.data(), *hb, (size_t)N, hipMemcpyDeviceToHost));
-    for (uint8_t b : bytes) c->w13_zrows[role] += (b & W13_ZROW) ? 1u : 0u;
+    std::vector<uint8_t> bytes((size_t)2 * N);
+    HIPCHK(c, hipMemcpy(bytes.data(), *hb, (size_t)2 * N, hipMemcpyDeviceToHost));
+    for (int r = 0; r < N; ++r) { c->w13_zrows[role] += (bytes[(size_t)r] & W13_ZROW) ? 1u : 0u; c->w13_nrows[role] += bytes[(size_t)N + r] ? 1u : 0u; }
+    uint64_t skip = 0;
+    for (int r = 0; r < N; ++r) if (bytes[(size_t)N + r]) skip += w13_row_bytes(K) - w13_row_bytes_streamed(K, 1);
+    c->w13_sskip[role] += skip;
+    if (grp.mode) c->w13_flag_bytes += (uint64_t)N;
+    if (probe) { c->w13_sskip_probe = skip; c->w13_flag_bytes_probe = grp.mode ? (uint64_t)N : 0; }
   }
   return DTK_OK;
 }
@@ -913,12 +927,15 @@
   if (!c->w13_bad) HIPCHK(c, hipMalloc((void**)&c->w13_bad, sizeof(unsigned)));
   c->w13_packed = c->w13_unpacked = c->w13_bad_rows = 0;
   for (uint32_t& z : c->w13_zrows) z = 0;
+  for (uint32_t& z : c->w13_nrows) z = 0;
+  for (uint64_t& z : c->w13_sskip) z = 0;
+  c->w13_sskip_probe = 0; c->w13_flag_bytes = c->w13_flag_bytes_probe = 0;
   const int qkvn = c->d + 2 * c->KVH * c->hd;
   for (int l = 0; l < c->L; ++l) {
     LayerW& w = c->layers[l];
     int rc = w13_pack_one(c, 0, PRO_RMSNORM, EPI_QKV, w.wqkv, qkvn, c->d, &w.p13_wqkv, &w.h13_wqkv);
     if (!rc) rc = w13_pack_one(c, 1, PRO_ATTN, EPI_RESID, w.wo, c->d, c->d, &w.p13_wo, &w.h13_wo);
-    if (!rc) rc = w13_pack_one(c, 2, PRO_RMSNORM, EPI_SWIGLU, w.wgu, 2 * c->ff, c->d, &w.p13_wgu, &w.h13_wgu);
+    if (!rc) rc = w13_pack_one(c, 2, PRO_RMSNORM, EPI_SWIGLU, w.wgu, 2 * c->ff, c->d, &w.p13_wgu, &w.h13_wgu, l == c->L / 2);
     if (!rc) rc = w13_pack_one(c, 3, PRO_COPY, EPI_RESID, w.wdown, c->d, c->ff, &w.p13_wdown, &w.h13_wdown);
     if (rc) { w13_free(c); return rc; }
   }
@@ -939,6 +956,9 @@
   c->w13_ready = false;
   c->w13_packed = c->w13_unpacked = c->w13_bad_rows = 0;
   for (uint32_t& z : c->w13_zrows) z = 0;
+  for (uint32_t& z : c->w13_nrows) z = 0;
+  for (uint64_t& z : c->w13_sskip) z = 0;
+  c->w13_sskip_probe = 0; c->w13_flag_bytes = c->w13_flag_bytes_probe = 0;
 }
 
 void ensure_tiled_weights(dtk_ctx* c);
@@ -3207,11 +3227,13 @@
       uint8_t *pp = nullptr, *hh = nullptr;
       HIPCHK(c, hipMalloc((void**)&pp, (size_t)c->d * w13_row_bytes(c->d)));
       tmp13.p.push_back(pp);
-      HIPCHK(c, hipMalloc((void**)&hh, (size_t)c->d));
+      HIPCHK(c, hipMalloc((void**)&hh, (size_t)2 * c->d));
       tmp13.h.push_back(hh);
       unsigned bad = 0;
       HIPCHK(c, hipMemsetAsync(c->w13_bad, 0, sizeof(unsigned), s));
-      launch_pack_w13_rows(w.wo, pp, hh, c->w13_bad, c->d, c->d, !c->w13_nz, s);
+      GemvArgs go{};
+      go.N = c->d; go.K = c->d; go.d = c->d; go.ff = c->ff; go.hd = c->hd;
+      launch_pack_w13_rows(w.wo, pp, hh, c->w13_bad, c->d, c->d, !c->w13_nz, c->w13_narrow ? gemv_w13_group(PRO_COPY, EPI_RESID, variant & 0xff, go, c->w13_narrow == 2) : W13Group{}, s);
       HIPCHK(c, hipMemcpyAsync(&bad, c->w13_bad, sizeof(unsigned), hipMemcpyDeviceToHost, s));
       HIPCHK(c, hipStreamSynchronize(s));
       if (bad) return fail(c, DTK_ERR_STATE, "dtk_bench_gemv: o_proj of layer %d has %u unpackable row(s)", l, bad);
@@ -3227,8 +3249,18 @@
     const int pro = (role == 1 || role == 3) ? PRO_COPY : PRO_RMSNORM;
     const int epi = role == 0 ? EPI_QKV : (role == 2 ? EPI_SWIGLU : (role == 4 ? EPI_LOGITS : EPI_RESID));
     if (!gemv_w13_has(pro, epi, variant)) return fail(c, DTK_ERR_ARG, "dtk_bench_gemv: no 13-bit shape %d for role %d", variant, role);
-  }
-  auto launch = [&](int pro, int epi, const GemvArgs& g) {
+    if (c->w13_narrow && role != 1) {
+      GemvArgs gq{};
+      gq.K = role == 3 ? c->ff : c->d; gq.d = c->d; gq.ff = c->ff; gq.hd = c->hd;
+      gq.N = role == 0 ? c->d + 2 * c->KVH * c->hd : (role == 2 ? 2 * c->ff : (role == 3 ? c->d : c->V));
+      const W13Group ga = gemv_w13_group(pro, epi, variant, gq, c->w13_narrow == 2), gb = gemv_w13_group(pro, epi, -1, gq, c->w13_narrow == 2);
+      if (gb.mode && (ga.mode != gb.mode || ga.R != gb.R))
+        return fail(c, DTK_ERR_STATE, "dtk_bench_gemv: 13-bit shape %d of role %d groups rows otherwise than the step's shape, by whose groups the narrow rows are flagged: set w13_narrow = 0", variant, role);
+    }
+  }
+  auto launch = [&](int pro, int epi, const GemvArgs& g0) {
+    GemvArgs g = g0;
+    if ((b13 || step13) && g.Wp) g.Wn = w13_flags(c, pro, epi, g, b13 ? variant : -1);
     if (b13) launch_gemv_w13_variant(pro, epi, variant, g, s);
     else if (shipped) launch_gemv(pro, epi, g, s);
     else launch_gemv_variant(pro, epi, variant, g, s);
@@ -3339,6 +3371,14 @@
       c->w13 = value; drop_graph(c);
       if (!value) { w13_free(c); w13_set_stats(c); }
       set_weight_bytes(c);
+    }
+  }
+  else if (!strcmp(name, "w13_narrow")) {
+    if (value < 0 || value > 2) return fail(c, DTK_ERR_ARG, "w13_narrow must be 0, 1 or 2");
+    if (value != c->w13_narrow) {
+      if (c->launched != c->waited) return fail(c, DTK_ERR_STATE, "w13_narrow: %d single-sequence decode step(s) are unread", (int)(c->launched - c->waited));
+      c->w13_narrow = value;
+      if (c->w13_ready) { c->w13_ready = false; drop_graph(c); set_weight_bytes(c); }
     }
   }
   else if (!strcmp(name, "w13_nz")) {
diff --git a/detikzify_amd/csrc/dtk_ctx.h b/detikzify_amd/csrc/dtk_ctx.h
--- a/detikzify_amd/csrc/dtk_ctx.h
+++ b/detikzify_amd/csrc/dtk_ctx.h
@@ -151,12 +151,18 @@
   float* s_lm_head = nullptr;
   int w13 = W13_DEFAULT;
   int w13_nz = 1;
+  int w13_narrow = 1;
   bool w13_ready = false;
   uint8_t *p13_lm_head = nullptr, *h13_lm_head = nullptr;
   unsigned* w13_bad = nullptr;
   int w13_op_bad_rows = -1;
+  int w13_op_narrow_rows = -1;
   uint32_t w13_packed = 0, w13_unpacked = 0, w13_bad_rows = 0;
   uint32_t w13_zrows[5] = {0, 0, 0, 0, 0};
+  uint32_t w13_nrows[5] = {0, 0, 0, 0, 0};
+  uint64_t w13_sskip[5] = {0, 0, 0, 0, 0};
+  uint64_t w13_flag_bytes = 0, w13_flag_bytes_probe = 0;
+  uint64_t w13_sskip_probe = 0;
   uint64_t cached_image_key = 0;
   bool have_image = false;
   int KVH = 0;
diff --git a/detikzify_amd/csrc/dtk_ops.hip b/detikzify_amd/csrc/dtk_ops.hip
--- a/detikzify_amd/csrc/dtk_ops.hip
+++ b/detikzify_amd/csrc/dtk_ops.hip
@@ -556,7 +556,7 @@
   if (fmt == 0) g.W = reinterpret_cast<const bf16_t*>(dW);
   else if (fmt == 1) { g.W8 = dW; g.wscale = dws; }
   else { g.W4 = dW; g.S4 = dS4; }
-  uint8_t* dWp = (uint8_t*)r.take(f13 ? (size_t)N * w13_row_bytes(K) : 0); uint8_t* dWh = (uint8_t*)r.take(f13 ? (size_t)N : 0);
+  uint8_t* dWp = (uint8_t*)r.take(f13 ? (size_t)N * w13_row_bytes(K) : 0); uint8_t* dWh = (uint8_t*)r.take(f13 ? (size_t)2 * N : 0);
   unsigned* dbad = (unsigned*)r.take(f13 ? sizeof(unsigned) : 0);
   g.x = r.in<bf16_t>(pro != PRO_ATTN ? x : nullptr, K); g.norm_w = r.in<bf16_t>(pro == PRO_RMSNORM ? norm_w : nullptr, K);
   g.rope_cos = r.in<bf16_t>(rope_cos, rope); g.rope_sin = r.in<bf16_t>(rope_sin, rope); g.st = r.in<DecState>(&hst, 1);
@@ -567,13 +567,18 @@
   if (const int rc = r.upload(s)) return rc;
   if (f13) {
     unsigned bad = 0;
+    const W13Group grp = !c->w13_narrow ? W13Group{} : (v13 == 0xff ? gemv_w13_group(pro, epi, -1, g, c->w13_narrow == 2) : gemv_w13_group(pro, epi, v13, g, true));
     HIPCHK(c, hipMemsetAsync(dbad, 0, sizeof(unsigned), s));
-    launch_pack_w13_rows(g.W, dWp, dWh, dbad, N, K, !c->w13_nz, s);
+    launch_pack_w13_rows(g.W, dWp, dWh, dbad, N, K, !c->w13_nz, grp, s);
     HIPCHK(c, hipMemcpyAsync(&bad, dbad, sizeof(unsigned), hipMemcpyDeviceToHost, s));
     HIPCHK(c, hipStreamSynchronize(s));
     HIPCHK(c, hipMemsetAsync(dbad, scratch_fill, sizeof(unsigned), s));
     c->w13_op_bad_rows = (int)bad;
-    if (!bad) { g.Wp = dWp; g.Wh = dWh; }
+    std::vector<uint8_t> flags((size_t)N);
+    HIPCHK(c, hipMemcpy(flags.data(), dWh + N, (size_t)N, hipMemcpyDeviceToHost));
+    c->w13_op_narrow_rows = 0;
+    for (uint8_t f : flags) c->w13_op_narrow_rows += f ? 1 : 0;
+    if (!bad) { g.Wp = dWp; g.Wh = dWh; g.Wn = grp.mode ? dWh + N : nullptr; }
   }
   if (f13 && g.Wp && v13 != 0xff) launch_gemv_w13_variant(pro, epi, v13, g, s);
   else if (variant < 0) launch_gemv(pro, epi, g, s);
@@ -879,6 +884,18 @@
 }
 int dtk_w13_op_bad_rows(dtk_ctx* c) { return c ? c->w13_op_bad_rows : -1; }
 int dtk_w13_flagged_rows(dtk_ctx* c, int role) { return (c && role >= 0 && role < 5 && c->w13_ready) ? (int)c->w13_zrows[role] : -1; }
+int dtk_w13_op_narrow_rows(dtk_ctx* c) { return c ? c->w13_op_narrow_rows : -1; }
+int dtk_w13_narrow_rows(dtk_ctx* c, int role) { return (c && role >= 0 && role < 5 && c->w13_ready) ? (int)c->w13_nrows[role] : -1; }
+int dtk_w13_pack_narrow_host(const uint16_t* W, int N, int K, uint8_t* planes, uint8_t* hb, uint8_t* narrow, int32_t* bad) {
+  if (!W || !planes || !hb || !narrow || !bad || N < 1 || K < 8 || (K & 7)) return DTK_ERR_ARG;
+  for (int r = 0; r < N; ++r) bad[r] = w13_pack_row_n(W + (size_t)r * K, K, planes + (size_t)r * w13_row_bytes(K), hb + r, narrow + r);
+  return DTK_OK;
+}
+int dtk_w13_unpack_narrow_host(const uint8_t* planes, const uint8_t* hb, const uint8_t* narrow, int N, int K, uint16_t* W) {
+  if (!W || !planes || !hb || !narrow || N < 1 || K < 8 || (K & 7)) return DTK_ERR_ARG;
+  for (int r = 0; r < N; ++r) w13_unpack_row_n(planes + (size_t)r * w13_row_bytes(K), hb[r], narrow[r], K, W + (size_t)r * K);
+  return DTK_OK;
+}
 int dtk_w13_row_bytes_host(const uint16_t* W, int N, int K, uint8_t* bytes) {
   if (!W || !bytes || N < 0 || K < 8 || (K & 7)) return DTK_ERR_ARG;
   for (int r = 0; r < N; ++r) bytes[r] = (uint8_t)w13_row_byte(W + (size_t)r * K, K);
diff --git a/detikzify_amd/csrc/gemv_inl.h b/detikzify_amd/csrc/gemv_inl.h
--- a/detikzify_amd/csrc/gemv_inl.h
+++ b/detikzify_amd/csrc/gemv_inl.h
@@ -131,7 +131,7 @@
   return c;
 }
 
-template <int NR, int U>
+template <int NR, int U, bool SP = true, bool LN = true>
 __device__ __forceinline__ void gemv_load_w13(u32x4 (&wl)[NR][U / 2], u32x2 (&wn)[NR][U / 2], uint32_t (&ws)[NR][U / 4],
                                               const u32x4* (&rows)[NR], int g, int lane, int J2, int n_off, int s_off) {
   static_assert(U % 4 == 0, "a stage is whole sign blocks");
@@ -144,10 +144,10 @@
         const unsigned char* p = reinterpret_cast<const unsigned char*>(rows[r]);
 #pragma unroll
         for (int h = 0; h < 2; ++h) {
-          wl[r][2 * ub + h] = ld_nt(rows[r] + ((2 * b + h) * 64 + lane));
-          wn[r][2 * ub + h] = __builtin_nontemporal_load(reinterpret_cast<const u32x2*>(p + n_off) + ((2 * b + h) * 64 + lane));
+          if (LN) wl[r][2 * ub + h] = ld_nt(rows[r] + ((2 * b + h) * 64 + lane));
+          if (LN) wn[r][2 * ub + h] = __builtin_nontemporal_load(reinterpret_cast<const u32x2*>(p + n_off) + ((2 * b + h) * 64 + lane));
         }
-        ws[r][ub] = __builtin_nontemporal_load(reinterpret_cast<const uint32_t*>(p + s_off) + (b * 64 + lane));
+        if (SP) ws[r][ub] = __builtin_nontemporal_load(reinterpret_cast<const uint32_t*>(p + s_off) + (b * 64 + lane));
       }
     }
     return;
@@ -163,10 +163,10 @@
         const bool ok = 2 * b + h < J2;
         const u32x4 zl = {0u, 0u, 0u, 0u};
         const u32x2 zn = {0u, 0u};
-        wl[r][2 * ub + h] = ok ? ld_nt(rows[r] + ((2 * b + h) * 64 + lane)) : zl;
-        wn[r][2 * ub + h] = ok ? __builtin_nontemporal_load(reinterpret_cast<const u32x2*>(p + n_off) + ((2 * b + h) * 64 + lane)) : zn;
+        if (LN) wl[r][2 * ub + h] = ok ? ld_nt(rows[r] + ((2 * b + h) * 64 + lane)) : zl;
+        if (LN) wn[r][2 * ub + h] = ok ? __builtin_nontemporal_load(reinterpret_cast<const u32x2*>(p + n_off) + ((2 * b + h) * 64 + lane)) : zn;
       }
-      ws[r][ub] = (2 * b < J2) ? __builtin_nontemporal_load(reinterpret_cast<const uint32_t*>(p + s_off) + (b * 64 + lane)) : 0u;
+      if (SP) ws[r][ub] = (2 * b < J2) ? __builtin_nontemporal_load(reinterpret_cast<const uint32_t*>(p + s_off) + (b * 64 + lane)) : 0u;
     }
   }
 }
@@ -188,3 +188,30 @@
     }
   }
 }
+
+__device__ __forceinline__ float dot8_w13n(uint32_t la, uint32_t lb, uint32_t n, uint32_t b4, const u32x4& x, float c) {
+  const uint32_t he = ((n & 0x07070707u) + b4) | ((n << 4) & 0x80808080u);
+  const uint32_t ho = (((n >> 4) & 0x07070707u) + b4) | (n & 0x80808080u);
+  c = dot2(__builtin_amdgcn_perm(he, la, 0x05010400u), x[0], c);
+  c = dot2(__builtin_amdgcn_perm(he, la, 0x07030602u), x[1], c);
+  c = dot2(__builtin_amdgcn_perm(ho, lb, 0x05010400u), x[2], c);
+  c = dot2(__builtin_amdgcn_perm(ho, lb, 0x07030602u), x[3], c);
+  return c;
+}
+
+template <int NR, int U>
+__device__ __forceinline__ void gemv_fma_w13n(float (&acc)[NR], const u32x4 (&wl)[NR][U / 2], const u32x2 (&wn)[NR][U / 2],
+                                              const uint32_t (&lo4)[NR], const u32x4* xs, int g, int lane, int K8) {
+  const bool full = 64 * (g * U + U) <= K8;
+#pragma unroll
+  for (int u = 0; u < U; ++u) {
+    const int c = lane + 64 * (g * U + u);
+    u32x4 xv = {0u, 0u, 0u, 0u};
+    if (full || c < K8) xv = xs[c];
+#pragma unroll
+    for (int r = 0; r < NR; ++r) {
+      const u32x4& l = wl[r][u >> 1];
+      acc[r] = dot8_w13n((u & 1) ? l[2] : l[0], (u & 1) ? l[3] : l[1], wn[r][u >> 1][u & 1], lo4[r] + 0x08080808u, xv, acc[r]);
+    }
+  }
+}
diff --git a/detikzify_amd/csrc/kernels.h b/detikzify_amd/csrc/kernels.h
--- a/detikzify_amd/csrc/kernels.h
+++ b/detikzify_amd/csrc/kernels.h
@@ -34,7 +34,10 @@
   int KVH;
   int hd = 128;
   const uint8_t* W4 = nullptr;
-  const uint8_t* S4 = nullptr;
+  union {
+    const uint8_t* S4 = nullptr;
+    const uint8_t* Wn;
+  };
   const uint8_t* Wp = nullptr;
   const uint8_t* Wh = nullptr;
 };
@@ -45,7 +48,9 @@
 void launch_gemv_w13_variant(int pro, int epi, int variant, const GemvArgs& a, hipStream_t s);
 bool gemv_w13_has(int pro, int epi, int variant);
 bool gemv_w13_takes(int pro, int epi, const GemvArgs& a);
-void launch_pack_w13_rows(const bf16_t* W, uint8_t* Wp, uint8_t* Wh, unsigned* bad_rows, int N, int K, bool zflag_all, hipStream_t s);
+struct W13Group { int mode = 0; int R = 1; int p = 0; };
+W13Group gemv_w13_group(int pro, int epi, int v13, const GemvArgs& a, bool any_k);
+void launch_pack_w13_rows(const bf16_t* W, uint8_t* Wp, uint8_t* Wh, unsigned* bad_rows, int N, int K, bool zflag_all, W13Group grp, hipStream_t s);
 void launch_gemv_f8(int pro, int epi, const GemvArgs& a, hipStream_t s);
 void launch_gemv_f8_variant(int pro, int epi, int variant, const GemvArgs& a, hipStream_t s);
 void set_gemv_default_variant(int epi, int variant);
diff --git a/detikzify_amd/csrc/kernels_decode.hip b/detikzify_amd/csrc/kernels_decode.hip
--- a/detikzify_amd/csrc/kernels_decode.hip
+++ b/detikzify_amd/csrc/kernels_decode.hip
@@ -94,8 +94,13 @@
   const uint8_t* srows[NR];
   uint32_t lo4[NR];
   bool zrow = false;
+  constexpr bool W13N = W13 && PRO != PRO_ATTN && EPI != EPI_QKV;
+  bool narrow = false;
+  unsigned nflag = 0;
+  const uint8_t* flags = W13N ? a.Wn : nullptr;
   auto set_rows = [&](int u0) {
     unsigned zb = 0;
+    unsigned nb = 1;
 #pragma unroll
     for (int j = 0; j < R; ++j) {
       int u = u0 + j;
@@ -125,9 +130,11 @@
         if (PAIRED) { lo4[2 * j] = (uint32_t)w13_lo(b0) * 0x01010101u; lo4[2 * j + 1] = (uint32_t)w13_lo(b1) * 0x01010101u; }
         else lo4[j] = (uint32_t)w13_lo(b0) * 0x01010101u;
         zb |= b0 | b1;
+        if (W13N && flags) nb &= (unsigned)flags[r0] & (PAIRED ? (unsigned)flags[r1] : 1u);
       }
     }
     if (W13 && PRO == PRO_RMSNORM) zrow = (__builtin_amdgcn_readfirstlane((int)zb) & W13_ZROW) != 0;
+    if (W13N) nflag = flags ? nb : 0u;
   };
   set_rows(unit0);
 
@@ -142,10 +149,15 @@
   u32x2 nwa[NR][UW / 2], nwb[NR][UW / 2];
   uint32_t zwa[NR][UW / 4], zwb[NR][UW / 4];
   float acc[NR];
-#define GLOAD(w, sc, g) do { if (W13) gemv_load_w13<NR, UW>(l##w, n##w, z##w, rows, (g), lane, J2, n13, s13); else if (F4) gemv_load_f4<NR, U>(w, sc, rows, srows, (g), lane, KC); else gemv_load<NR, U>(w, rows, (g), lane, KC); } while (0)
-#define GFMA(w, sc, g) do { if (W13) gemv_fma_w13<NR, UW, NZ>(acc, l##w, n##w, z##w, lo4, xs, (g), lane, K8); else if (F4) gemv_fma_f4<NR, U>(acc, w, sc, xs, (g), lane, KC); else if (F8) gemv_fma_f8<NR, U>(acc, w, xs, (g), lane, KC); else gemv_fma<NR, U>(acc, w, xs, (g), lane, KC); } while (0)
-
-  if (G > 0) GLOAD(wa, sa, GIDX(0));
+#define GLOAD_(w, sc, g, SP) do { if (W13) gemv_load_w13<NR, UW, SP>(l##w, n##w, z##w, rows, (g), lane, J2, n13, s13); else if (F4) gemv_load_f4<NR, U>(w, sc, rows, srows, (g), lane, KC); else gemv_load<NR, U>(w, rows, (g), lane, KC); } while (0)
+#define GLOAD(w, sc, g) GLOAD_(w, sc, g, (DEC != 2))
+#define GLOAD0(w, sc, g) do { if constexpr (W13N) { gemv_load_w13<NR, UW, false, true>(l##w, n##w, z##w, rows, (g), lane, J2, n13, s13); \
+      narrow = (__builtin_amdgcn_readfirstlane((int)nflag) & 1) != 0;                                                                  \
+      if (!narrow) gemv_load_w13<NR, UW, true, false>(l##w, n##w, z##w, rows, (g), lane, J2, n13, s13); }                           \
+    else GLOAD_(w, sc, g, true); } while (0)
+#define GFMA(w, sc, g) do { if constexpr (W13 && DEC == 2) gemv_fma_w13n<NR, UW>(acc, l##w, n##w, lo4, xs, (g), lane, K8); else if (W13) gemv_fma_w13<NR, UW, DEC == 1>(acc, l##w, n##w, z##w, lo4, xs, (g), lane, K8); else if (F4) gemv_fma_f4<NR, U>(acc, w, sc, xs, (g), lane, KC); else if (F8) gemv_fma_f8<NR, U>(acc, w, xs, (g), lane, KC); else gemv_fma<NR, U>(acc, w, xs, (g), lane, KC); } while (0)
+
+  if (G > 0) GLOAD0(wa, sa, GIDX(0));
 
   float pre0[R], pre1[R];
   int pos = 0;
@@ -299,8 +311,8 @@
     const bool active = unit0 < n_units;
 #pragma unroll
     for (int r = 0; r < NR; ++r) acc[r] = 0.f;
-#define MAIN_LOOP(NZV) do {                                   \
-      constexpr bool NZ = NZV;                                 \
+#define MAIN_LOOP(DECV) do {                                  \
+      constexpr int DEC = DECV;                                \
       for (int g = 0; g < G; g += 2) {                         \
         if (g + 1 < G) GLOAD(wb, sb, GIDX(g + 1));             \
         GFMA(wa, sa, GIDX(g));                                 \
@@ -310,11 +322,18 @@
         }                                                      \
       }                                                        \
     } while (0)
-    if constexpr (W13 && PRO == PRO_RMSNORM) {
-      if (zrow) MAIN_LOOP(false);
-      else MAIN_LOOP(true);
+    if constexpr (W13N && PRO == PRO_RMSNORM) {
+      if (narrow) MAIN_LOOP(2);
+      else if (zrow) MAIN_LOOP(0);
+      else MAIN_LOOP(1);
+    } else if constexpr (W13N) {
+      if (narrow) MAIN_LOOP(2);
+      else MAIN_LOOP(0);
+    } else if constexpr (W13 && PRO == PRO_RMSNORM) {
+      if (zrow) MAIN_LOOP(0);
+      else MAIN_LOOP(1);
     } else {
-      MAIN_LOOP(false);
+      MAIN_LOOP(0);
     }
 #undef MAIN_LOOP
     const int cur = unit0;
@@ -326,7 +345,7 @@
       unit0 = chunk * R;
       if (unit0 < n_units) {
         set_rows(unit0);
-        GLOAD(wa, sa, 0);
+        GLOAD0(wa, sa, 0);
         if (EPI == EPI_RESID || EPI == EPI_QKV) prefetch_epilogue(unit0);
       }
     }
@@ -362,6 +381,8 @@
   }
 #undef GIDX
 #undef GLOAD
+#undef GLOAD0
+#undef GLOAD_
 #undef GFMA
 #undef XI
 }
@@ -585,10 +606,10 @@
   }
   hipLaunchKernelGGL((k_gemv<PRO, EPI, R, U, WAVES, PERSIST, false, KS, 128, false, true, FW>), dim3(grid), dim3(WAVES * 64), lds, s, a);
 }
-#define WV(PRO, EPI, R, U, W) return launch_gemv_w13_t<PRO, EPI, R, U, W>(a, s)
-#define WVP(PRO, EPI, R, U, W, BPC) return launch_gemv_w13_t<PRO, EPI, R, U, W, true, 1, BPC>(a, s)
-#define WVK(PRO, EPI, R, U, W, KS) return launch_gemv_w13_t<PRO, EPI, R, U, W, false, KS>(a, s)
-#define WVF(PRO, EPI, R, U, W, BPC, FW) return launch_gemv_w13_t<PRO, EPI, R, U, W, true, 1, BPC, FW>(a, s)
+#define WV(PRO, EPI, R, U, W) do { if (qR) { *qR = R; return; } return launch_gemv_w13_t<PRO, EPI, R, U, W>(a, s); } while (0)
+#define WVP(PRO, EPI, R, U, W, BPC) do { if (qR) { *qR = R; return; } return launch_gemv_w13_t<PRO, EPI, R, U, W, true, 1, BPC>(a, s); } while (0)
+#define WVK(PRO, EPI, R, U, W, KS) do { if (qR) { *qR = R; return; } return launch_gemv_w13_t<PRO, EPI, R, U, W, false, KS>(a, s); } while (0)
+#define WVF(PRO, EPI, R, U, W, BPC, FW) do { if (qR) { *qR = R; return; } return launch_gemv_w13_t<PRO, EPI, R, U, W, true, 1, BPC, FW>(a, s); } while (0)
 bool gemv_w13_has(int pro, int epi, int v) {
   if (pro == PRO_RMSNORM && (epi == EPI_QKV || epi == EPI_SWIGLU)) return v >= 0 && v <= 7;
   if (pro == PRO_COPY && epi == EPI_RESID) return v >= 0 && v <= 6;
@@ -598,7 +619,7 @@
   if (pro == PRO_COPY && epi == EPI_STORE) return v == 0;
   return false;
 }
-void launch_gemv_w13_variant(int pro, int epi, int v, const GemvArgs& a, hipStream_t s) {
+static void w13_variant_row(int pro, int epi, int v, const GemvArgs& a, hipStream_t s, int* qR) {
   if (pro == PRO_RMSNORM && epi == EPI_QKV) {
     switch (v) { default: WV(PRO_RMSNORM, EPI_QKV, 1, 4, 4); case 1: WV(PRO_RMSNORM, EPI_QKV, 2, 4, 4); case 2: WV(PRO_RMSNORM, EPI_QKV, 1, 4, 8);
                  case 3: WVP(PRO_RMSNORM, EPI_QKV, 1, 4, 8, 2); case 4: WV(PRO_RMSNORM, EPI_QKV, 1, 8, 4);
@@ -630,6 +651,7 @@
   fprintf(stderr, "launch_gemv_w13: no 13-bit kernel for prologue %d, epilogue %d\n", pro, epi);
   abort();
 }
+void launch_gemv_w13_variant(int pro, int epi, int v, const GemvArgs& a, hipStream_t s) { w13_variant_row(pro, epi, v, a, s, nullptr); }
 #undef WV
 #undef WVP
 #undef WVK
@@ -651,32 +673,58 @@
   return -1;
 }
 
-__global__ __launch_bounds__(256) void k_pack_w13_rows(const bf16_t* W, uint8_t* Wp, uint8_t* Wh, unsigned* bad_rows, int N, int K, int zflag_all) {
+__device__ __forceinline__ void w13_row_range(const bf16_t* W, int row, int K, int* red, int* redq, int& hb, int& qmin) {
+  const int tid = threadIdx.x, K8 = K >> 3;
+  const u32x4* w4 = reinterpret_cast<const u32x4*>(W + (size_t)row * K);
+  hb = 0; qmin = 127;
+  for (int c = tid; c < K8; c += 256) {
+    const u32x4 v = w4[c];
+#pragma unroll
+    for (int e = 0; e < 4; ++e) {
+      const int q0 = (int)((v[e] >> 8) & 0x7fu), q1 = (int)((v[e] >> 24) & 0x7fu);
+      hb = max(hb, max(q0, q1));
+      qmin = min(qmin, min(q0, q1));
+    }
+  }
+#pragma unroll
+  for (int off = 32; off >= 1; off >>= 1) { hb = max(hb, __shfl_xor(hb, off)); qmin = min(qmin, __shfl_xor(qmin, off)); }
+  __syncthreads();
+  if ((tid & 63) == 0) { red[tid >> 6] = hb; redq[tid >> 6] = qmin; }
+  __syncthreads();
+  hb = max(max(red[0], red[1]), max(red[2], red[3]));
+  qmin = min(min(redq[0], redq[1]), min(redq[2], redq[3]));
+}
+__global__ __launch_bounds__(256) void k_pack_w13_rows(const bf16_t* W, uint8_t* Wp, uint8_t* Wh, unsigned* bad_rows, int N, int K, int zflag_all, W13Group grp) {
   const int row = blockIdx.x, tid = threadIdx.x;
   const u32x4* w4 = reinterpret_cast<const u32x4*>(W + (size_t)row * K);
   unsigned char* out = Wp + (size_t)row * w13_row_bytes(K);
   __shared__ int red[4], redq[4];
   __shared__ int any_bad;
   const int K8 = K >> 3, J2 = w13_units(K), J4 = w13_blocks(K);
-  int hb = 0, qmin = 127;
-  for (int c = tid; c < K8; c += 256) {
-    const u32x4 v = w4[c];
-#pragma unroll
-    for (int e = 0; e < 4; ++e) {
-      const int q0 = (int)((v[e] >> 8) & 0x7fu), q1 = (int)((v[e] >> 24) & 0x7fu);
-      hb = max(hb, max(q0, q1));
-      qmin = min(qmin, min(q0, q1));
-    }
-  }
-#pragma unroll
-  for (int off = 32; off >= 1; off >>= 1) { hb = max(hb, __shfl_xor(hb, off)); qmin = min(qmin, __shfl_xor(qmin, off)); }
-  if ((tid & 63) == 0) { red[tid >> 6] = hb; redq[tid >> 6] = qmin; }
+  int hb, qmin;
+  w13_row_range(W, row, K, red, redq, hb, qmin);
   if (tid == 0) any_bad = 0;
-  __syncthreads();
-  hb = max(max(red[0], red[1]), max(red[2], red[3]));
-  qmin = min(min(redq[0], redq[1]), min(redq[2], redq[3]));
   if (tid == 0) Wh[row] = (uint8_t)(hb | ((qmin == 0 || zflag_all) ? W13_ZROW : 0));
   const int lo = w13_lo(hb);
+  bool narrow = grp.mode != 0 && qmin >= lo + W13_NARROW_MIN;
+  if (narrow) {
+    const int u = grp.mode == 3 ? row % grp.p : row;
+    const int n_units = grp.mode == 1 ? N : grp.p;
+    const int u0 = (u / grp.R) * grp.R;
+    for (int j = 0; j < grp.R && u0 + j < n_units && narrow; ++j) {
+      const int uu = u0 + j;
+      const int r0 = uu, r1 = grp.mode == 3 ? grp.p + uu : r0;
+      for (int h = 0; h < 2 && narrow; ++h) {
+        const int r = h ? r1 : r0;
+        if (r == row || (h && r1 == r0)) continue;
+        int hb2, q2;
+        w13_row_range(W, r, K, red, redq, hb2, q2);
+        narrow = q2 >= w13_lo(hb2) + W13_NARROW_MIN;
+      }
+    }
+  }
+  if (tid == 0) Wh[N + row] = narrow ? 1 : 0;
+  __syncthreads();
   int bad = 0;
   for (int t = tid; t < J4 * 64; t += 256) {
     const int b = t >> 6, l = t & 63;
@@ -700,8 +748,12 @@
           if (code < 0) { ++bad; code = 0; wk = 0; }
           const int kb = 8 * (k & 3);
           if (k < 4) la |= (wk & 0xffu) << kb; else lb |= (wk & 0xffu) << kb;
-          n |= (uint32_t)code << (kb + 4 * (k >> 2));
-          sg |= (wk >> 15) << (kb + 2 * i + (k >> 2));
+          if (narrow) {
+            if (c < K8) n |= (uint32_t)w13_nibble_narrow((int)(wk >> 15), code) << (kb + 4 * (k >> 2));
+          } else {
+            n |= (uint32_t)code << (kb + 4 * (k >> 2));
+            sg |= (wk >> 15) << (kb + 2 * i + (k >> 2));
+          }
         }
         lv[2 * i2] = la; lv[2 * i2 + 1] = lb; nv[i2] = n;
       }
@@ -714,8 +766,8 @@
   __syncthreads();
   if (tid == 0 && any_bad) atomicAdd(bad_rows, 1u);
 }
-void launch_pack_w13_rows(const bf16_t* W, uint8_t* Wp, uint8_t* Wh, unsigned* bad_rows, int N, int K, bool zflag_all, hipStream_t s) {
-  hipLaunchKernelGGL(k_pack_w13_rows, dim3(N), dim3(256), 0, s, W, Wp, Wh, bad_rows, N, K, zflag_all ? 1 : 0);
+void launch_pack_w13_rows(const bf16_t* W, uint8_t* Wp, uint8_t* Wh, unsigned* bad_rows, int N, int K, bool zflag_all, W13Group grp, hipStream_t s) {
+  hipLaunchKernelGGL(k_pack_w13_rows, dim3(N), dim3(256), 0, s, W, Wp, Wh, bad_rows, N, K, zflag_all ? 1 : 0, grp);
 }
 
 static int g_variant[8] = {0, 0, 0, 0, 0, -1, 0, 0};
@@ -746,6 +798,16 @@
   launch_gemv_variant(pro, epi, v, a, s);
 }
 bool gemv_w13_takes(int pro, int epi, const GemvArgs& a) { return w13_shape_for(pro, epi, gemv_chosen_variant(pro, epi, a), a) >= 0; }
+W13Group gemv_w13_group(int pro, int epi, int v13, const GemvArgs& a, bool any_k) {
+  W13Group g;
+  if (!any_k && a.K < 4096) return g;
+  if (v13 < 0) v13 = w13_shape_for(pro, epi, gemv_chosen_variant(pro, epi, a), a);
+  if (v13 < 0 || pro == PRO_ATTN || epi == EPI_QKV || !gemv_w13_has(pro, epi, v13)) return g;
+  w13_variant_row(pro, epi, v13, a, nullptr, &g.R);
+  g.mode = epi == EPI_SWIGLU ? 3 : 1;
+  g.p = epi == EPI_SWIGLU ? a.ff : 0;
+  return g;
+}
 
 __global__ __launch_bounds__(256) void k_attn_decode(AttnDecArgs a) {
   const int h = blockIdx.x, sp = blockIdx.y;
diff --git a/detikzify_amd/csrc/w13.h b/detikzify_amd/csrc/w13.h
--- a/detikzify_amd/csrc/w13.h
+++ b/detikzify_amd/csrc/w13.h
@@ -69,6 +69,39 @@
     w[k] = (uint16_t)((sign << 15) | (w13_high(code, lo) << 8) | row[p.l]);
   }
 }
+#define W13_NARROW_MIN 8
+W13_HD static inline int w13_nibble_narrow(int sign, int code) { return (sign << 3) | (code - W13_NARROW_MIN); }
+W13_HD static inline int w13_high_narrow(int nibble, int lo) { return ((nibble & 8) << 4) | (lo + W13_NARROW_MIN + (nibble & 7)); }
+W13_HD static inline int w13_pos_nsign(const W13Pos& p) { return p.nshift + 3; }
+static inline int w13_row_narrow(const uint16_t* w, int K) {
+  const int lo = w13_lo(w13_row_hb(w, K));
+  for (int k = 0; k < K; ++k) if (w13_code(w[k], lo) < W13_NARROW_MIN) return 0;
+  return 1;
+}
+static inline int w13_pack_row_n(const uint16_t* w, int K, uint8_t* row, uint8_t* hb_out, uint8_t* narrow) {
+  *narrow = (uint8_t)w13_row_narrow(w, K);
+  if (!*narrow) return w13_pack_row(w, K, row, hb_out);
+  const int hb = w13_row_hb(w, K), lo = w13_lo(hb);
+  const size_t nb = w13_row_bytes(K);
+  for (size_t i = 0; i < nb; ++i) row[i] = 0;
+  for (int k = 0; k < K; ++k) {
+    const W13Pos p = w13_pos(K, k);
+    row[p.l] = (uint8_t)(w[k] & 0xff);
+    row[p.n] = (uint8_t)(row[p.n] | (w13_nibble_narrow((w[k] >> 15) & 1, w13_code(w[k], lo)) << p.nshift));
+  }
+  *hb_out = (uint8_t)hb;
+  return 0;
+}
+static inline void w13_unpack_row_n(const uint8_t* row, int hb, int narrow, int K, uint16_t* w) {
+  if (!narrow) { w13_unpack_row(row, hb, K, w); return; }
+  const int lo = w13_lo(hb);
+  for (int k = 0; k < K; ++k) {
+    const W13Pos p = w13_pos(K, k);
+    w[k] = (uint16_t)((w13_high_narrow((row[p.n] >> p.nshift) & 15, lo) << 8) | row[p.l]);
+  }
+}
+W13_HD static inline size_t w13_row_bytes_streamed(int K, int narrow) { return narrow ? w13_s_off(K) : w13_row_bytes(K); }
+
 static inline void w13_unpack_row_nz(const uint8_t* row, int hb, int K, uint16_t* w) {
   const int lo = w13_lo(hb);
   for (int k = 0; k < K; ++k) {
diff --git a/include/dtk.h b/include/dtk.h
--- a/include/dtk.h
+++ b/include/dtk.h
@@ -334,6 +334,10 @@
 int  dtk_w13_op_bad_rows(dtk_ctx* ctx);
 int  dtk_w13_row_bytes_host(const uint16_t* W, int N, int K, uint8_t* bytes);
 int  dtk_w13_flagged_rows(dtk_ctx* ctx, int role);
+int  dtk_w13_narrow_rows(dtk_ctx* ctx, int role);
+int  dtk_w13_op_narrow_rows(dtk_ctx* ctx);
+int  dtk_w13_pack_narrow_host(const uint16_t* W, int N, int K, uint8_t* planes, uint8_t* hb, uint8_t* narrow, int32_t* bad);
+int  dtk_w13_unpack_narrow_host(const uint8_t* planes, const uint8_t* hb, const uint8_t* narrow, int N, int K, uint16_t* W);
 int  dtk_op_layernorm(dtk_ctx* ctx, const uint16_t* X, const uint16_t* w, const uint16_t* b,
                       int M, int D, float eps, uint16_t* Y);
 int  dtk_op_sample(dtk_ctx* ctx, const float* logits, int V, int step, int64_t* token_out,
```

Result: no change. 416.5 tokens/s (-0.0%).
